# Astropianist/LumFuncMCMC

Hardware: AMD Instinct MI355X
Metric: walker-lnprob evals/sec (10^6 sources, 256 walkers) (higher is better)
Workload: dtype f64; 1 GPU; free completeness, single Schechter: 1000000 synthetic sources, 256 walkers in all (256 per GPU), 2 half-ensemble calls of 128 theta rows per step; walkers_per_gpu=256, walkers_total=256, variant=free, parallelism=1 GPU

## Files before the change

### lumfuncmcmc_amd/csrc/lf_free.h

```cpp
#pragma once
#include "lf_kernels.h"

namespace lf {

constexpr int PB = 512;
constexpr int PTW = 8;
constexpr int QSTRIDE = 9;
constexpr int VF = 32;
constexpr int DEAL_BINS = VF + 1, DEAL_LIST = 2 * (VF + 1), DEAL_MAX = 512;
constexpr unsigned long long PART_EMPTY = 0x7ff8dead7ff8deadull;
constexpr int PART_POLLS = 1 << 19;

template <bool THROUGH = false>
__device__ __forceinline__ void reduce_store512(const double* __restrict__ red, int wlo, int whi, double* __restrict__ out,
                                                size_t stride, int w0, int chunk, int tid) {
    const int w = tid >> 6, lane = tid & 63;
    if (w >= wlo && w < whi) {
        const double* row = red + w * PB + lane;
        double s0 = (row[0] + row[64]) + (row[128] + row[192]);
        double s1 = (row[256] + row[320]) + (row[384] + row[448]);
        const double s = wave_sum_dpp(s0 + s1);
        if (lane == 63) {
            if (THROUGH) __hip_atomic_store(out + (size_t)(w0 + w) * stride + chunk, s, __ATOMIC_RELAXED, __HIP_MEMORY_SCOPE_AGENT);
            else out[(size_t)(w0 + w) * stride + chunk] = s;
        }
    }
}

struct FreeArgs {
    int B, ntiles;
    int nchA, nchB;
    int nslot;
    int tile_stride;
    int skip_grid;
    int* queues;
    double* partA;
    double* partB;
    const double* cells;
    const double* nodes8;
    const int* deal;
    const int* cc_len;
    const int* cc_field;
    int nchC;
    double* partC;
    const int* wstat;
    const double* theta;
    double* out;
    double* wrec_w;
    int* wmode_w;
    int* wstat_w;
    double* wbase_w;
    const double* gq_rec;
    const double* gq_omega;
    const int* gq_rows;
    int nbq;
    int poll;
    int* err;
};

template <int ST, bool CENSUS, bool FUSED, bool STEP>
__device__ __forceinline__ void lf_free_body(const KConst& kc, const SrcArrays& sa, const NodeArrays& na, const double* __restrict__ wrec_arg,
                                             const int* __restrict__ wmode_arg, const FreeArgs& fa, const StepArgs& sp, const AcceptArgs& ap,
                                             unsigned long long t_pre = 0) {
    const double* wrec = FUSED ? fa.wrec_w : wrec_arg;
    const int* wmode = FUSED ? fa.wmode_w : wmode_arg;
    auto pstore = [](double* p, double v) {
        if (FUSED) __hip_atomic_store(p, v == v ? v : __builtin_nan(""), __ATOMIC_RELAXED, __HIP_MEMORY_SCOPE_AGENT);
        else *p = v;
    };
    __shared__ MathTables tab;
    __shared__ TermTables tt;
    __shared__ __attribute__((aligned(16))) double red[PTW * PB];
    __shared__ __attribute__((aligned(16))) double wfc[PTW * MAXF * 8];
    __shared__ __attribute__((aligned(16))) double wsc[PTW * 8];
    __shared__ int sitem[2];
    __shared__ int sdeal[DEAL_MAX];
    __shared__ int scell;
    __shared__ int snosrc;
    const int tid = threadIdx.x;
    __shared__ int sstat[PTW];
    __shared__ double sbase[PTW];
    __shared__ double wlf[PTW * MAXF];
    __shared__ double sprop[PTW * 16];
    __shared__ double szz[PTW];
    __shared__ double spre[PTW * 2];
    if (!FUSED) {
        for (int i = tid; i < 256; i += PB) {
            tab.logt[i] = *reinterpret_cast<const double2*>(LOG_TABLE + 2 * i);
            tab.expt[i] = EXP_TABLE[i];
        }
        load_term_tables<PB>(&tt);
        if (fa.deal && tid < DEAL_LIST + fa.nchC + fa.nbq) sdeal[tid] = fa.deal[tid];
    }
    bool tables_loaded = !FUSED;
    const int wave_base = __builtin_amdgcn_readfirstlane(tid & ~63);
    auto fresh_tid = [&]() -> int {
        int m = -1;
        asm volatile("" : "+s"(m));
        return wave_base + __builtin_amdgcn_mbcnt_hi(m, __builtin_amdgcn_mbcnt_lo(m, 0));
    };
    unsigned xcc;
    asm volatile("s_getreg_b32 %0, hwreg(HW_REG_XCC_ID)" : "=s"(xcc));
    const int myq = (int)(xcc & 7u);
#ifdef LF_STAMPS
    __shared__ unsigned long long s_targs;
    unsigned long long* stamp = kc.stamps ? kc.stamps + (size_t)blockIdx.x * 8 : nullptr;
    if (stamp && tid == 0) {
        stamp[0] = t_pre ? t_pre : __builtin_amdgcn_s_memtime();
        stamp[5] = __builtin_amdgcn_s_memrealtime();
        s_targs = __builtin_amdgcn_s_memtime();
    }
    int nitems_done = 0;
    unsigned long long t_first = 0, t_sw = 0, t_loop = 0, t_red = 0;
    unsigned long long t_prep = 0, t_cells = 0, t_grid = 0;
    __shared__ unsigned long long s_ttab;
    __shared__ unsigned long long s_tp0;
    __shared__ unsigned long long s_tprep[8];
#endif

#pragma unroll 1
    for (int tile = ((int)blockIdx.x >> 3) % fa.ntiles; tile < fa.ntiles; tile += fa.tile_stride) {
        const int w0 = tile * PTW;
        const int nw = min(PTW, fa.B - w0);
        __builtin_assume(nw >= 1 && nw <= PTW);
        int* __restrict__ q = fa.queues + tile * QSTRIDE;
        int fgroup = 8, frank = (int)blockIdx.x & 7;
        if (fa.ntiles <= fa.tile_stride) {
            const int k = (int)blockIdx.x >> 3;
            fgroup = 8 * ((fa.tile_stride - tile + fa.ntiles - 1) / fa.ntiles);
            frank += 8 * ((k - tile) / fa.ntiles);
        }
        bool no_src = false;
        auto grab = [&]() -> int {
            if (no_src) return -1;
            for (int d = 0; d < 8; ++d) {
                const int qq = (myq + d) & 7;
                const int lo = (int)(((long long)qq * fa.nchA) >> 3), hi = (int)(((long long)(qq + 1) * fa.nchA) >> 3);
                if (hi <= lo) continue;
                const int i = atomicAdd(q + 1 + qq, 1);
                if (i < hi - lo) return lo + i;
            }
            return -1;
        };
        int ticket = 0;
        auto take_ticket = [&]() {
            if (!no_src) ticket = atomicAdd(q + 1 + myq, 1);
        };
        auto redeem = [&]() -> int {
            if (no_src) return -1;
            const int lo = (int)(((long long)myq * fa.nchA) >> 3), hi = (int)(((long long)(myq + 1) * fa.nchA) >> 3);
            if (ticket < hi - lo) return lo + ticket;
            return grab();
        };
        if (tile != ((int)blockIdx.x >> 3) % fa.ntiles) __syncthreads();
        const int u = fresh_tid();
        if (FUSED) {
            const int pw = (int)(blockIdx.x >> 8) & 1;
            const int up = u - 64 * pw;
            if (up >= 0 && up < 64) {
                prepare_lane<false, true, STEP, LF_FREE>(kc, sp, fa.theta, fa.B, nullptr, nullptr, nullptr, nullptr, nullptr, 1,
                                          w0 + (up >> 3), up & 7, up >> 3, reinterpret_cast<double(*)[16]>(red), wfc, wsc, sstat, sbase, wlf,
#ifdef LF_STAMPS
                                          s_tprep,
#else
                                          nullptr,
#endif
                                          sprop, szz);
#ifdef LF_STAMPS
                if (up == 0) s_tp0 = __builtin_amdgcn_s_memtime();
#endif
            } else if (!tables_loaded) {
                const int t7 = u < 64 * pw ? u : u - 64;
                double2 lt = *reinterpret_cast<const double2*>(LOG_TABLE + 2 * min(t7, 255));
                double et = EXP_TABLE[min(t7, 255)];
                const int ndeal = fa.deal ? DEAL_LIST + fa.nchC + fa.nbq : 0;
                int d0 = ndeal ? fa.deal[min(t7, ndeal - 1)] : 0, d1 = ndeal ? fa.deal[min(t7 + 256, ndeal - 1)] : 0;
                asm volatile("" : "+v"(lt.x), "+v"(lt.y), "+v"(et), "+v"(d0), "+v"(d1));
                load_term_tables<PB - 64>(&tt, t7);
                if (t7 < 256) {
                    tab.logt[t7] = lt;
                    tab.expt[t7] = et;
                    if (t7 < ndeal) sdeal[t7] = d0;
                    if (t7 + 256 < ndeal) sdeal[t7 + 256] = d1;
                }
#ifdef LF_STAMPS
                if (t7 == 0) s_ttab = __builtin_amdgcn_s_memtime();
#endif
            }
            if (STEP && u >= PB - 64 && u < PB - 64 + nw) {
                const int wl = u - (PB - 64);
                unsigned int rr[4];
                sampler_draw(sp.step, sp.half, w0 + wl, 0, sp.seed, rr);
                accept_terms(ap, w0 + wl, stretch_z(sp.a, u53(rr[0], rr[1])), spre[2 * wl], spre[2 * wl + 1]);
            }
            tables_loaded = true;
            __syncthreads();
        }
        if (u < 64) {
            const int st = FUSED ? sstat[min(u, nw - 1)] : fa.wstat[w0 + min(u, nw - 1)];
            const bool on = fa.nchC > 0 && u < nw && (st & STAT_CELLS);
            const bool need = u < nw && !on && (st & STAT_PRIOR_OK) && !(st & STAT_NEGINF);
            const int m = (int)__ballot(on);
            const unsigned long long mneed = __ballot(need);
            if (u == 0) {
                scell = m;
                no_src = mneed == 0ull;
                snosrc = no_src ? 1 : 0;
                sitem[0] = grab();
            }
        }
        if (!FUSED && u < nw * MAXF) {
            const int w = u / MAXF, f = u - w * MAXF;
            double* d = wfc + u * 8;
            int* di = reinterpret_cast<int*>(d + 4);
            if (f < kc.nf) {
                const double* __restrict__ r = wrec + (size_t)(w0 + w) * REC;
                const int* __restrict__ km = wmode + ((size_t)(w0 + w) * MAXF + f) * WM;
                d[0] = r[R_ALPHAC];
                d[F_V] = r[RF(f, F_V)];
                d[F_CA] = r[RF(f, F_CA)];
                d[F_CY] = r[RF(f, F_CY)] - H_LO - 0.5 / H_INV;
                d[7] = r[RF(f, F_CY)] - H_LO;
#pragma unroll
                for (int i = 0; i < 5; ++i) di[i] = km[i];
            }
        }
        if (!FUSED && u >= PB - PTW * 8) {
            const int t = u - (PB - PTW * 8), w = t >> 3, j = t & 7;
            if (w < nw) wsc[t] = wrec[(size_t)(w0 + w) * REC + j];
        }
        __syncthreads();
#ifdef LF_STAMPS
        t_prep = __builtin_amdgcn_s_memtime();
#endif
        const int cellmask = __builtin_amdgcn_readfirstlane(scell);
        auto fetch = [&](int w, int fld) {
            const double2* __restrict__ p = reinterpret_cast<const double2*>(wfc + (w * MAXF + fld) * 8);
            const double2 a = p[0], b = p[1], c = p[3];
            if (FUSED) {
                const int* __restrict__ ki = reinterpret_cast<const int*>(wfc + (w * MAXF + fld) * 8 + 4);
                return WalkerK{a.x, b.x, b.y, c.y, uni(ki[M_MODE]), uni(ki[M_KLO]), uni(ki[M_KHI]), uni(ki[M_KNE]), uni(ki[M_KAC])};
            }
            const int* __restrict__ km = wmode + ((size_t)(w0 + w) * MAXF + fld) * WM;
            return WalkerK{a.x, b.x, b.y, c.y, km[M_MODE], km[M_KLO], km[M_KHI], km[M_KNE], km[M_KAC]};
        };

        {
            const int v = wave_base >> 6;
#pragma unroll 1
            for (int vr = frank; vr < VF; vr += fgroup) {
            double acc = 0.0;
            const bool dealt = fa.deal != nullptr;
            const int cfirst = (vr - VF / 2 + VF) % VF;
            const int cb = dealt ? DEAL_LIST + uni(sdeal[vr]) : cfirst;
            const int cn = dealt ? uni(sdeal[vr + 1]) - uni(sdeal[vr]) : (cfirst < fa.nchC ? (fa.nchC - cfirst + VF - 1) / VF : 0);
            auto chunk_at = [&](int i) { return dealt ? uni(sdeal[cb + i]) : cb + i * VF; };
            if (fa.nchC > 0 && v < nw && ((cellmask >> v) & 1) && cn > 0) {
                auto load_cells = [&](double (&d)[CELL_REC], int cc) {
                    const int lane = fresh_tid() & 63;
                    const double2* __restrict__ src = reinterpret_cast<const double2*>(fa.cells + ((size_t)cc * 64 + lane) * CELL_REC);
                    static_assert(CELL_REC % 2 == 0, "16-byte loads");
#pragma unroll
                    for (int k = 0; k < CELL_REC / 2; ++k) {
                        const double2 a = src[k];
                        d[2 * k] = a.x;
                        d[2 * k + 1] = a.y;
                    }
                };
                auto field_of = [&](int cc) {
                    int f = 0;
#pragma unroll
                    for (int k = 1; k < MAXF; ++k) f += cc >= kc.cc_fstart[k] ? 1 : 0;
                    return f;
                };
                double nx[CELL_REC];
                load_cells(nx, chunk_at(0));
#pragma unroll 1
                for (int ci = 0; ci < cn; ++ci) {
                    const int cc = chunk_at(ci);
                    double cd[CELL_REC];
#pragma unroll
                    for (int k = 0; k < CELL_REC; ++k) cd[k] = nx[k];
                    if (ci + 1 < cn) load_cells(nx, chunk_at(ci + 1));
                    const WalkerK p = fetch(v, field_of(cc));
                    asm volatile("; LF_BEGIN cell items=1");
                    acc += cell_sum(cd, p, &tt);
                    asm volatile("; LF_END cell");
                    if (CENSUS && kc.forms && (fresh_tid() & 63) == 0) atomicAdd(kc.forms + FORM_CELL, (unsigned long long)uni(fa.cc_len[cc]));
                }
            }
            if (fa.nchC > 0 && v < nw) {
                acc = wave_sum_dpp(acc);
                const int ln = fresh_tid() & 63;
                double* __restrict__ row = fa.partC + (size_t)(w0 + v) * fa.nslot;
                if (ln == 63) pstore(row + vr, acc);
            }
            }
        }
#ifdef LF_STAMPS
        t_cells = __builtin_amdgcn_s_memtime();
#endif
        if (fa.nbq > 0) {
            const int v = wave_base >> 6;
            const int nq = fa.nbq;
#pragma unroll 1
            for (int vr = frank; vr < VF; vr += fgroup) {
            double bsum = 0.0;
            const bool dealt = fa.deal != nullptr;
            const int qb = dealt ? DEAL_LIST + fa.nchC + uni(sdeal[DEAL_BINS + vr]) : vr;
            const int qn = dealt ? uni(sdeal[DEAL_BINS + vr + 1]) - uni(sdeal[DEAL_BINS + vr]) : (vr < nq ? (nq - vr + VF - 1) / VF : 0);
            auto bin_at = [&](int i) { return dealt ? uni(sdeal[qb + i]) : qb + i * VF; };
            if (v < nw && qn > 0) {
                const double* __restrict__ sc = wsc + v * 8;
                const int mode = __builtin_amdgcn_readfirstlane(*reinterpret_cast<const int*>(wfc + (v * MAXF) * 8 + 4));
                const double* __restrict__ r = wfc + v * MAXF * 8 - 8;
                double vmin = r[RF(0, F_V)];
                for (int f = 1; f < kc.nf; ++f) vmin = fmin(vmin, r[RF(f, F_V)]);
                vmin = uni(vmin);
                const double alphaC = uni(sc[R_ALPHAC]);
                auto mine = [&](int c) { return mode != MODE_SKIP && !(kc.grid_parts > 1 && c % kc.grid_parts != kc.grid_part); };
                struct QRec {
                    double x, a4, L, PGL;
                };
                auto load_rec = [&](int c) -> QRec {
                    const int lane = fresh_tid() & 63;
                    const double2* __restrict__ src = reinterpret_cast<const double2*>(fa.gq_rec + ((size_t)c * 64 + lane) * 4);
                    const double2 a = src[0], b = src[1];
                    return QRec{a.x, a.y, b.x, b.y};
                };
                double* __restrict__ Tl = red + v * 64;
                QRec nx = load_rec(bin_at(0));
#pragma unroll 1
                for (int qi = 0; qi < qn; ++qi) {
                    const int c = bin_at(qi);
                    const QRec nd = nx;
                    const int nr = uni(fa.gq_rows[4 * c + 1]), off = uni(fa.gq_rows[4 * c + 2]);
                    if (qi + 1 < qn) nx = load_rec(bin_at(qi + 1));
                    if (mine(c)) {
                        const int lane = fresh_tid() & 63;
                        const double* __restrict__ om = fa.gq_omega + off + lane;
                        double o[8];
#pragma unroll
                        for (int i = 0; i < 8; ++i) o[i] = i < nr ? om[i * 64] : 0.0;
                        asm volatile("; LF_BEGIN qT items=1");
                        Tl[lane] = fexp_c(fma(uni(sc[R_C1]), nd.L - uni(sc[R_LSTAR]), uni(sc[R_C0])) - nd.PGL * uni(sc[R_Q]), &tab);
                        asm volatile("; LF_END qT");
                        const double a4min = __hiloint2double(__builtin_amdgcn_readlane(__double2hiint(nd.a4), 63),
                                                              __builtin_amdgcn_readlane(__double2loint(nd.a4), 63));
                        const bool bright = kc.specialise && alphaC > 0.0 && a4min * vmin > 37.5;
                        if (CENSUS && kc.forms && lane == 0)
                            atomicAdd(kc.forms + (bright ? FORM_NODE_BRIGHT : FORM_NODE_GENERAL), (unsigned long long)(64 * kc.nf));
                        const double s = field_sum_nf(kc, r, alphaC, nd.x, nd.a4, &tab, bright);
                        __builtin_amdgcn_wave_barrier();
                        asm volatile("; LF_BEGIN qdot items=1");
                        double R = 0.0;
#pragma unroll 1
                        for (int k0 = 0; k0 < nr; k0 += 8) {
                            double on[8];
#pragma unroll
                            for (int i = 0; i < 8; ++i) on[i] = k0 + 8 + i < nr ? om[(k0 + 8 + i) * 64] : 0.0;
#pragma unroll
                            for (int i = 0; i < 8; ++i) R = fma(Tl[min(k0 + i, 63)], o[i], R);
#pragma unroll
                            for (int i = 0; i < 8; ++i) o[i] = on[i];
                        }
                        asm volatile("; LF_END qdot");
                        bsum = fma(R, s, bsum);
                        __builtin_amdgcn_wave_barrier();
                    }
                }
            }
            if (v < nw) {
                bsum = wave_sum_dpp(bsum);
                const int ln = fresh_tid() & 63;
                double* __restrict__ row = fa.partB + (size_t)(w0 + v) * fa.nslot;
                if (ln == 63) pstore(row + vr, bsum);
            }
            }
        } else
        {
            const int v = wave_base >> 6;
            const int nch64 = fa.nchB;
#pragma unroll 1
            for (int vr = frank; vr < VF; vr += fgroup) {
            double bsum = 0.0;
            if (v < nw && vr < nch64) {
                const double* __restrict__ sc = wsc + v * 8;
                const int mode = __builtin_amdgcn_readfirstlane(*reinterpret_cast<const int*>(wfc + (v * MAXF) * 8 + 4));
                const double* __restrict__ r = wfc + v * MAXF * 8 - 8;
                double vmin = r[RF(0, F_V)];
                for (int f = 1; f < kc.nf; ++f) vmin = fmin(vmin, r[RF(f, F_V)]);
                vmin = uni(vmin);
                const double alphaC = uni(sc[R_ALPHAC]);
                auto mine = [&](int c) { return mode != MODE_SKIP && !(kc.grid_parts > 1 && c % kc.grid_parts != kc.grid_part); };
                struct Node {
                    double G, PG, W, a3, a4, a4min;
                };
                auto load_nodes = [&](int c) -> Node {
                    const int lane = fresh_tid() & 63;
                    const double2* __restrict__ src = reinterpret_cast<const double2*>(fa.nodes8 + ((size_t)c * 64 + lane) * 8);
                    const double2 a = src[0], b = src[1], d = src[2];
                    return Node{a.x, a.y, b.x, b.y, d.x, d.y};
                };
                Node nx = load_nodes(vr);
#pragma unroll 1
                for (int c = vr; c < nch64; c += VF) {
                    const Node nd = nx;
                    if (c + VF < nch64) nx = load_nodes(c + VF);
                    if (mine(c)) {
                        const double a4min = uni(nd.a4min);
                        const double T = fexp_c(fma(uni(sc[R_C1]), nd.G - uni(sc[R_LSTAR]), uni(sc[R_C0])) - nd.PG * uni(sc[R_Q]), &tab);
                        const bool bright = kc.specialise && alphaC > 0.0 && a4min * vmin > 37.5;
                        if (CENSUS && kc.forms && (fresh_tid() & 63) == 0)
                            atomicAdd(kc.forms + (bright ? FORM_NODE_BRIGHT : FORM_NODE_GENERAL),
                                      (unsigned long long)(min(64, na.nnodes - c * 64) * kc.nf));
                        const double s = field_sum_nf(kc, r, alphaC, nd.a3, nd.a4, &tab, bright);
                        bsum = fma(nd.W * T, s, bsum);
                    }
                }
            }
            if (nch64 > 0 && v < nw) {
                bsum = wave_sum_dpp(bsum);
                const int ln = fresh_tid() & 63;
                double* __restrict__ row = fa.partB + (size_t)(w0 + v) * fa.nslot;
                if (ln == 63) pstore(row + vr, bsum);
            }
            }
        }
#ifdef LF_STAMPS
        t_grid = __builtin_amdgcn_s_memtime();
#endif
        int item = sitem[0];
#pragma unroll 1
        while (item >= 0) {
#ifdef LF_STAMPS
            const unsigned long long ta = __builtin_amdgcn_s_memtime();
            if (t_first == 0) t_first = ta;
            unsigned long long tb = ta, tc = ta;
#endif
            __syncthreads();
            int t = fresh_tid();
            {
                const int c = item;
                const int s0 = uni(sa.chunk_start[c]), n = uni(sa.chunk_len[c]), fld = uni(sa.chunk_field[c]);
                const int kfirst = uni(sa.chunk_keys[KEY_STRIDE * c]), klast = uni(sa.chunk_keys[KEY_STRIDE * c + 1]),
                          kamax = uni(sa.chunk_keys[KEY_STRIDE * c + 4 + (wave_base >> 6)]);
                double x[ST];
                if (t == 0) take_ticket();
                if (n == PB * ST) {
                    typedef double __attribute__((ext_vector_type(2), aligned(8))) double2_a8;
                    const double2_a8* __restrict__ src = reinterpret_cast<const double2_a8*>(sa.a1 + s0 + t * ST);
#pragma unroll
                    for (int k = 0; k < ST / 2; ++k) {
                        const double2_a8 a = src[k];
                        x[2 * k] = a.x;
                        x[2 * k + 1] = a.y;
                    }
                } else {
                    const double* __restrict__ src = sa.a1 + s0;
#pragma unroll
                    for (int k = 0; k < ST; ++k) x[k] = src[min(t * ST + k, n - 1)];
                }
                if (t == 0) {
                    asm volatile("" ::"v"(x[ST - 1]));
                    sitem[0] = redeem();
                }
#ifdef LF_STAMPS
                tb = __builtin_amdgcn_s_memtime();
#endif
                const int npad = ST - min(max(n - t * ST, 0), ST);
                const int nwave = min(max(n - wave_base * ST, 0), 64 * ST);
                int rest = 0;
                WalkerK pn = fetch(0, fld);
#pragma unroll 1
                for (int w = 0; w < nw; ++w) {
                    const WalkerK p = pn;
                    pn = fetch(min(w + 1, nw - 1), fld);
                    double acc = 0.0;
                    if ((cellmask >> w) & 1) {
                    } else if (p.mode < MODE_SKIP && p.mode != MODE_SLOW && kc.tables && kfirst >= p.klo && klast <= p.khi && p.kac <= kamax) {
                        TabCoef C;
                        if (kc.specialise && kfirst >= p.kne) {
                            asm volatile("; LF_BEGIN table_noexp items=%0" ::"n"(ST));
                            table_lookup<ST>(C, x, p, true, &tt);
                            acc = table_terms<ST, true>(C, x, npad);
                            asm volatile("; LF_END table_noexp");
                            if (CENSUS && kc.forms && (t & 63) == 0) atomicAdd(kc.forms + FORM_TABLE_NOEXP, (unsigned long long)nwave);
                        } else {
                            asm volatile("; LF_BEGIN table items=%0" ::"n"(ST));
                            table_lookup<ST>(C, x, p, false, &tt);
                            acc = table_terms<ST, false>(C, x, npad);
                            asm volatile("; LF_END table");
                            if (CENSUS && kc.forms && (t & 63) == 0) atomicAdd(kc.forms + FORM_TABLE, (unsigned long long)nwave);
                        }
                    } else if (p.mode < MODE_SKIP) {
                        rest |= 1 << w;
                    } else if (CENSUS && kc.forms && (t & 63) == 0) {
                        atomicAdd(kc.forms + FORM_SKIPPED, (unsigned long long)nwave);
                    }
                    red[w * PB + t] = acc;
                }
                if (rest) {
                    t = fresh_tid();
                    double u[ST];
                    {
                        const double* __restrict__ up = sa.U + s0;
#pragma unroll
                        for (int k = 0; k < ST; ++k) u[k] = up[min(t * ST + k, n - 1)];
                    }
                    const double a1_first = uni(x[0]), u_first = uni(u[0]);
                    const int nmine = ST - npad;
#pragma unroll 1
                    for (int w = 0; w < nw; ++w) {
                        if (!((rest >> w) & 1)) continue;
                        const double* __restrict__ r = FUSED ? wsc + w * 8 : wrec + (size_t)(w0 + w) * REC;
                        const double* __restrict__ rf = wfc + (w * MAXF + fld) * 8;
                        const int mode = FUSED ? uni(*reinterpret_cast<const int*>(rf + 4)) : wmode[((size_t)(w0 + w) * MAXF + fld) * WM];
                        const double r_lf = FUSED ? wlf[w * MAXF + fld] : r[RF(fld, F_LF)];
                        const double r_v = FUSED ? rf[F_V] : r[RF(fld, F_V)], r_ca = FUSED ? rf[F_CA] : r[RF(fld, F_CA)];
                        double acc = 0.0;
                        int form;
                        if (mode == MODE_SLOW) {
                            form = FORM_CAREFUL;
                            const WFree wf{r[R_LSTAR], r[R_C0] + kc.lnom0_src[fld], r[R_C1], r[R_Q], r[R_ALPHAC],
                                           r_lf, r_v, kc.lnom0_src[fld], 0.0};
#pragma unroll 1
                            for (int i = t; i < n; i += PB) {
                                const size_t g = (size_t)s0 + i;
                                acc += term_free_careful(wf, sa.lum[g], sa.a1[g], sa.P[g], sa.U[g]);
                            }
                        } else {
                            WFree wf{};
                            wf.alphaC = r[R_ALPHAC];
                            wf.cA = r_ca;
                            wf.V = r_v;
                            const bool upper = kc.specialise && wf.alphaC > 0.0 && fma(wf.alphaC, a1_first, wf.cA) >= 0.0;
                            if (upper && u_first * wf.V > 37.5) {
                                form = FORM_GENERAL_NOEXP;
#pragma unroll
                                for (int k = 0; k < ST; ++k) {
                                    asm volatile("; LF_BEGIN general_noexp items=1");
                                    const double term = term_free_noexp(wf, x[k], &tab);
                                    asm volatile("; LF_END general_noexp");
                                    acc += k < nmine ? term : 0.0;
                                    __builtin_amdgcn_sched_barrier(0);
                                }
                            } else {
                                form = FORM_GENERAL;
#pragma unroll
                                for (int k = 0; k < ST; ++k) {
                                    asm volatile("; LF_BEGIN general items=1");
                                    const double term = term_free_fast(wf, x[k], u[k], &tab);
                                    asm volatile("; LF_END general");
                                    acc += k < nmine ? term : 0.0;
                                    __builtin_amdgcn_sched_barrier(0);
                                }
                            }
                        }
                        if (CENSUS && kc.forms && (t & 63) == 0) atomicAdd(kc.forms + form, (unsigned long long)nwave);
                        red[w * PB + t] = acc;
                    }
                }
#ifdef LF_STAMPS
                tc = __builtin_amdgcn_s_memtime();
#endif
                __syncthreads();
                t = fresh_tid();
                reduce_store512<FUSED>(red, 0, nw, fa.partA, (size_t)fa.nchA, w0, c, t);
                item = sitem[0];
            }
#ifdef LF_STAMPS
            ++nitems_done;
            if (tb != ta) {
                t_sw += tb - ta;
                t_loop += tc - tb;
                t_red += __builtin_amdgcn_s_memtime() - tc;
            }
#endif
        }
        if (FUSED && fa.poll && uni(snosrc)) {
            if (frank == fgroup - 1) {
                const int t = fresh_tid(), v = t >> 6, ln = t & 63;
                const int nB = fa.nchB > 0 ? fa.nslot : 0, nC = fa.nchC > 0 ? fa.nslot : 0;
                if (v < nw) {
                    double* __restrict__ pb = fa.partB + (size_t)(w0 + v) * fa.nslot;
                    double* __restrict__ pc = fa.partC + (size_t)(w0 + v) * fa.nslot;
                    double pre[2] = {0.0, 0.0};
                    int tries = 0;
                    bool have;
                    do {
                        if (ln < nC) pre[0] = __hip_atomic_load(pc + ln, __ATOMIC_RELAXED, __HIP_MEMORY_SCOPE_AGENT);
                        if (ln < nB) pre[1] = __hip_atomic_load(pb + ln, __ATOMIC_RELAXED, __HIP_MEMORY_SCOPE_AGENT);
                        have = !((ln < nC && (unsigned long long)__double_as_longlong(pre[0]) == PART_EMPTY) ||
                                 (ln < nB && (unsigned long long)__double_as_longlong(pre[1]) == PART_EMPTY));
                    } while (!__all(have) && ++tries < PART_POLLS);
                    if (tries >= PART_POLLS) {
                        pre[0] = pre[1] = __builtin_nan("");
                        if (ln == 0) atomicExch(fa.err, 1);
                    }
                    if (ln < nC) __hip_atomic_store(pc + ln, __longlong_as_double((long long)PART_EMPTY), __ATOMIC_RELAXED, __HIP_MEMORY_SCOPE_AGENT);
                    if (ln < nB) __hip_atomic_store(pb + ln, __longlong_as_double((long long)PART_EMPTY), __ATOMIC_RELAXED, __HIP_MEMORY_SCOPE_AGENT);
                    finalize_wave<true>(fa.partA, 0, fa.nchA, fa.partB, nB, nB, nC > 0 ? fa.partC : nullptr, nC, (int)STAT_CELLS,
                                        sstat - w0, sbase - w0, w0 + v, ln, ap, fa.out, nullptr, nullptr, 0,
                                        STEP ? sprop + v * 16 : nullptr, STEP ? szz + v : nullptr, STEP ? spre + 2 * v : nullptr, pre);
                }
            }
        } else if (FUSED) {
            asm volatile("s_waitcnt vmcnt(0)" ::: "memory");
            __threadfence_block();
            __syncthreads();
            if (fresh_tid() == 0) sitem[1] = atomicAdd(q, 1);
            __syncthreads();
            if (sitem[1] == fgroup - 1) {
                __builtin_amdgcn_fence(__ATOMIC_ACQUIRE, "workgroup");
                const int t = fresh_tid(), v = t >> 6;
                const int nB = fa.nchB > 0 ? fa.nslot : 0, nC = fa.nchC > 0 ? fa.nslot : 0;
                if (v < nw) {
                    finalize_wave<true>(fa.partA, fa.nchA, fa.nchA, fa.partB, nB, nB, nC > 0 ? fa.partC : nullptr, nC, (int)STAT_CELLS,
                                        sstat - w0, sbase - w0, w0 + v, t & 63, ap, fa.out, nullptr, nullptr, 0,
                                        STEP ? sprop + v * 16 : nullptr, STEP ? szz + v : nullptr, STEP ? spre + 2 * v : nullptr);
                    if (fa.poll) {
                        const int ln = t & 63;
                        if (ln < nC) __hip_atomic_store(fa.partC + (size_t)(w0 + v) * fa.nslot + ln, __longlong_as_double((long long)PART_EMPTY), __ATOMIC_RELAXED, __HIP_MEMORY_SCOPE_AGENT);
                        if (ln < nB) __hip_atomic_store(fa.partB + (size_t)(w0 + v) * fa.nslot + ln, __longlong_as_double((long long)PART_EMPTY), __ATOMIC_RELAXED, __HIP_MEMORY_SCOPE_AGENT);
                    }
                }
                if (t < QSTRIDE) q[t] = 0;
            }
        }
    }
#ifdef LF_STAMPS
    if (stamp && tid == 0) {
        stamp[1] = __builtin_amdgcn_s_memtime();
        const bool noitems = nitems_done == 0;
        stamp[2] = (unsigned long long)nitems_done;
        if (noitems) {
            stamp[3] = t_prep - stamp[0];
            stamp[4] = t_cells - stamp[0];
            stamp[7] = t_grid - stamp[0];
            unsigned long long pk = 0;
            pk = ((s_targs - stamp[0]) >> 4) & 0xfffull;
            for (int i = 0; i < 4; ++i) pk |= (((s_tprep[i] - stamp[0]) >> 4) & 0xfffull) << (12 * (i + 1));
            stamp[2] = pk;
        } else {
            stamp[3] = t_first ? t_first - stamp[0] : 0;
            stamp[4] = t_sw;
            stamp[7] = t_loop;
        }
        stamp[6] = __builtin_amdgcn_s_memrealtime();
        kc.stamps[(size_t)gridDim.x * 8 + blockIdx.x] =
            !noitems ? t_red : (((s_ttab - stamp[0]) << 32) | ((s_tp0 - stamp[0]) & 0xffffffffull));
    }
#endif
}

template <int ST, bool CENSUS, bool FUSED = false>
__global__ __launch_bounds__(PB, 4) void lf_free(KConst kc, SrcArrays sa, NodeArrays na, const double* __restrict__ wrec_arg,
                                                 const int* __restrict__ wmode_arg, FreeArgs fa) {
#ifdef LF_STAMPS
    const unsigned long long t_pre = __builtin_amdgcn_s_memtime();
#else
    const unsigned long long t_pre = 0;
#endif
    warm_kernarg<sizeof(KConst) + sizeof(SrcArrays) + sizeof(NodeArrays) + 2 * 8 + sizeof(FreeArgs)>();
    lf_free_body<ST, CENSUS, FUSED, false>(kc, sa, na, wrec_arg, wmode_arg, fa, StepArgs{}, AcceptArgs{}, t_pre);
}

template <int ST>
__global__ __launch_bounds__(PB, 4) void lf_free_step(KConst kc, SrcArrays sa, NodeArrays na, FreeArgs fa, StepArgs sp, AcceptArgs ap) {
    warm_kernarg<sizeof(KConst) + sizeof(SrcArrays) + sizeof(NodeArrays) + sizeof(FreeArgs) + sizeof(StepArgs) + sizeof(AcceptArgs)>();
    lf_free_body<ST, false, true, true>(kc, sa, na, nullptr, nullptr, fa, sp, ap);
}

}
```

### lumfuncmcmc_amd/csrc/lf_math.h

```cpp
#pragma once
#include <hip/hip_runtime.h>

#include "lf_tables.h"

#define LF_LN10 2.302585092994045684
#define LF_LNLN10 0.834032445247955959
#define LF_LN2 0.693147180559945309
#define LF_UNDERFLOW 745.13321910194122
#define LF_LREF 42.0
#define LF_FREF (-17.0)
#define LF_SQARCSEC 42545170296.152206
#define LF_MPC_CM 3.086e24

namespace lf {

__device__ __forceinline__ double dexp(double x) { return exp(x); }
__device__ __forceinline__ double dlog(double x) { return log(x); }
__device__ __forceinline__ double drsqrt(double x) { return rsqrt(x); }
__device__ __forceinline__ double ddiv(double a, double b) { return a / b; }

struct MathTables {
    double2 logt[256];
    double expt[256];
};

__device__ __forceinline__ double fexp_t(double x, const MathTables* __restrict__ mt) {
    const double MAGIC = 6755399441055744.0;
    const double t = fma(x, 369.32993046757463, MAGIC);
    const double kd = t - MAGIC;
    double r = fma(kd, -0.00270760617331689, x);
    r = fma(kd, -7.453964567463233e-13, r);
    const int k = __double2loint(t);
    const double T = mt->expt[k & 255];
    double q = fma(r, 4.16666666666666666667e-02, 1.66666666666666666667e-01);
    q = fma(q, r, 0.5);
    const double p = fma(r * r, q, r);
    return ldexp(fma(T, p, T), k >> 8);
}

__device__ __forceinline__ double fexp_neg(double u, const MathTables* __restrict__ mt) {
    const double MAGIC = 6755399441055744.0;
    const double t = fma(u, -369.32993046757463, MAGIC);
    const double kd = t - MAGIC;
    const double r = fma(kd, -0.0027076061740622863, -u);
    const int k = __double2loint(t);
    const double T = mt->expt[k & 255];
    double q = fma(r, 4.16666666666666666667e-02, 1.66666666666666666667e-01);
    q = fma(q, r, 0.5);
    const double p = fma(r * r, q, r);
    return ldexp(fma(T, p, T), k >> 8);
}

__device__ __forceinline__ double fexp_c(double x, const MathTables* __restrict__ mt) {
    return fexp_t(fmin(fmax(x, -750.0), 709.0), mt);
}

__device__ __forceinline__ double flog_half(double w, const MathTables* __restrict__ mt) {
    const int hi = __double2hiint(w), lo = __double2loint(w);
    const int e = ((hi >> 20) & 0x7ff) - 1024;
    const int j = (hi >> 12) & 0xff;
    const double m = __hiloint2double((hi & 0x000fffff) | 0x3ff00000, lo);
    const double2 t = mt->logt[j];
    const double r = fma(m, t.x, -1.0);
    double p = fma(r, 0.2, -0.25);
    double third = 1.0 / 3.0;
    asm volatile("" : "+s"(third));
    p = fma(p, r, third);
    p = fma(p, r, -0.5);
    const double r2 = r * r;
    const double hi_part = fma((double)e, LF_LN2, t.y);
    return hi_part + fma(p, r2, r);
}

__device__ __forceinline__ double flog_half_upper(double w, const MathTables* __restrict__ mt) {
    const double m = fmin(w, 1.9999999999999998);
    const int j = (__double2hiint(m) >> 12) & 0xff;
    const double2 t = mt->logt[j];
    const double r = fma(m, t.x, -1.0);
    double p = fma(r, 0.2, -0.25);
    p = fma(p, r, 1.0 / 3.0);
    p = fma(p, r, -0.5);
    const double r2 = r * r;
    return (t.y - LF_LN2) + fma(p, r2, r);
}

__device__ __forceinline__ double frsqrt(double s) {
    const double z0 = __builtin_amdgcn_rsq(s);
    const double e = fma(-(s * z0), z0, 1.0);
    const double p = fma(0.375, e, 0.5);
    return fma(z0, p * e, z0);
}

__device__ __forceinline__ double frcp(double d) {
    const double y0 = __builtin_amdgcn_rcp(d);
    const double e = fma(-d, y0, 1.0);
    return fma(y0, fma(e, e, e), y0);
}

struct TermTables {
    double g[G_N * 8];
    double h[H_N * 8];
};
template <int NT>
__device__ __forceinline__ void load_term_tables(TermTables* tt, int t = -1) {
    double2* g2 = reinterpret_cast<double2*>(tt->g);
    double2* h2 = reinterpret_cast<double2*>(tt->h);
    const double2* G2 = reinterpret_cast<const double2*>(G_TABLE);
    const double2* H2 = reinterpret_cast<const double2*>(H_TABLE);
    constexpr int NG = (G_N * 4 + NT - 1) / NT, NH = (H_N * 4 + NT - 1) / NT;
    double2 vg[NG], vh[NH];
    if (t < 0) t = threadIdx.x;
#pragma unroll
    for (int q = 0; q < NG; ++q) vg[q] = G2[min(t + q * NT, G_N * 4 - 1)];
#pragma unroll
    for (int q = 0; q < NH; ++q) vh[q] = H2[min(t + q * NT, H_N * 4 - 1)];
#pragma unroll
    for (int q = 0; q < NG; ++q) asm volatile("" : "+v"(vg[q].x), "+v"(vg[q].y));
#pragma unroll
    for (int q = 0; q < NH; ++q) asm volatile("" : "+v"(vh[q].x), "+v"(vh[q].y));
#pragma unroll
    for (int q = 0; q < NG; ++q)
        if (t + q * NT < G_N * 4) g2[t + q * NT] = vg[q];
#pragma unroll
    for (int q = 0; q < NH; ++q)
        if (t + q * NT < H_N * 4) h2[t + q * NT] = vh[q];
}

__device__ __forceinline__ double horner7(const double (&c)[8], double t) {
    double p = fma(c[7], t, c[6]);
    p = fma(p, t, c[5]);
    p = fma(p, t, c[4]);
    p = fma(p, t, c[3]);
    p = fma(p, t, c[2]);
    p = fma(p, t, c[1]);
    return fma(p, t, c[0]);
}

__device__ __forceinline__ void load_tables(MathTables* mt) {
    for (int i = threadIdx.x; i < 256; i += blockDim.x) {
        mt->logt[i] = make_double2(LOG_TABLE[2 * i], LOG_TABLE[2 * i + 1]);
        mt->expt[i] = EXP_TABLE[i];
    }
}
__device__ __forceinline__ void load_tables_256(MathTables* mt) {
    const int i = threadIdx.x;
    const double2 l = *reinterpret_cast<const double2*>(LOG_TABLE + 2 * i);
    const double e = EXP_TABLE[i];
    mt->logt[i] = l;
    mt->expt[i] = e;
}

template <int CTRL, int ROW_MASK>
__device__ __forceinline__ double dpp_shift_add(double v) {
    const int lo = __builtin_amdgcn_update_dpp(0, __double2loint(v), CTRL, ROW_MASK, 0xf, false);
    const int hi = __builtin_amdgcn_update_dpp(0, __double2hiint(v), CTRL, ROW_MASK, 0xf, false);
    return v + __hiloint2double(hi, lo);
}
__device__ __forceinline__ double wave_sum_dpp(double v) {
    v = dpp_shift_add<0x111, 0xf>(v);
    v = dpp_shift_add<0x112, 0xf>(v);
    v = dpp_shift_add<0x114, 0xf>(v);
    v = dpp_shift_add<0x118, 0xf>(v);
    v = dpp_shift_add<0x142, 0xa>(v);
    v = dpp_shift_add<0x143, 0xc>(v);
    return v;
}

__device__ __forceinline__ double wave_sum(double v) {
#pragma unroll
    for (int off = 32; off > 0; off >>= 1) v += __shfl_down(v, off, 64);
    return v;
}

#define LF_KW1(o) "s_load_dword %0, %1, " #o "\n\t"
#define LF_KW4(b) LF_KW1(b + 0x00) LF_KW1(b + 0x40) LF_KW1(b + 0x80) LF_KW1(b + 0xc0)
template <int BYTES>
__device__ __forceinline__ void warm_kernarg() {
    constexpr int N4 = (BYTES + 255) / 256;
    static_assert(N4 >= 1 && N4 <= 10, "extend the ladder");
    auto p = __builtin_amdgcn_kernarg_segment_ptr();
    int t;
    if constexpr (N4 == 1) asm volatile(LF_KW4(0x000) "s_waitcnt lgkmcnt(0)" : "=&s"(t) : "s"(p) : "memory");
    if constexpr (N4 == 2) asm volatile(LF_KW4(0x000) LF_KW4(0x100) "s_waitcnt lgkmcnt(0)" : "=&s"(t) : "s"(p) : "memory");
    if constexpr (N4 == 3) asm volatile(LF_KW4(0x000) LF_KW4(0x100) LF_KW4(0x200) "s_waitcnt lgkmcnt(0)" : "=&s"(t) : "s"(p) : "memory");
    if constexpr (N4 == 4)
        asm volatile(LF_KW4(0x000) LF_KW4(0x100) LF_KW4(0x200) LF_KW4(0x300) "s_waitcnt lgkmcnt(0)" : "=&s"(t) : "s"(p) : "memory");
    if constexpr (N4 == 5)
        asm volatile(LF_KW4(0x000) LF_KW4(0x100) LF_KW4(0x200) LF_KW4(0x300) LF_KW4(0x400) "s_waitcnt lgkmcnt(0)" : "=&s"(t) : "s"(p) : "memory");
    if constexpr (N4 == 6)
        asm volatile(LF_KW4(0x000) LF_KW4(0x100) LF_KW4(0x200) LF_KW4(0x300) LF_KW4(0x400) LF_KW4(0x500) "s_waitcnt lgkmcnt(0)"
                     : "=&s"(t) : "s"(p) : "memory");
    if constexpr (N4 == 7)
        asm volatile(LF_KW4(0x000) LF_KW4(0x100) LF_KW4(0x200) LF_KW4(0x300) LF_KW4(0x400) LF_KW4(0x500) LF_KW4(0x600) "s_waitcnt lgkmcnt(0)"
                     : "=&s"(t) : "s"(p) : "memory");
    if constexpr (N4 == 8)
        asm volatile(LF_KW4(0x000) LF_KW4(0x100) LF_KW4(0x200) LF_KW4(0x300) LF_KW4(0x400) LF_KW4(0x500) LF_KW4(0x600) LF_KW4(0x700)
                     "s_waitcnt lgkmcnt(0)" : "=&s"(t) : "s"(p) : "memory");
    if constexpr (N4 == 9)
        asm volatile(LF_KW4(0x000) LF_KW4(0x100) LF_KW4(0x200) LF_KW4(0x300) LF_KW4(0x400) LF_KW4(0x500) LF_KW4(0x600) LF_KW4(0x700)
                     LF_KW4(0x800) "s_waitcnt lgkmcnt(0)" : "=&s"(t) : "s"(p) : "memory");
    if constexpr (N4 == 10)
        asm volatile(LF_KW4(0x000) LF_KW4(0x100) LF_KW4(0x200) LF_KW4(0x300) LF_KW4(0x400) LF_KW4(0x500) LF_KW4(0x600) LF_KW4(0x700)
                     LF_KW4(0x800) LF_KW4(0x900) "s_waitcnt lgkmcnt(0)" : "=&s"(t) : "s"(p) : "memory");
}

}
```

### lumfuncmcmc_amd/csrc/lf_pers.h

```cpp
#pragma once
#include "lf_free.h"

namespace lf {

constexpr int PERS_MAXS = 256;

struct PersArgs {
    int B, ntiles;
    int nchB;
    int nchC, ncell;
    int nslot;
    int tile_stride;
    int* queues;
    double* partA;
    double* partB;
    double* partC;
    const double* nodes4;
    const double* zcol;
    const double* cells;
    const double* lum;
    const double* a1;
    const double* P;
    const double* U;
    const double* theta;
    double* out;
    const double* wrec;
    const int* wmode;
    const int* wstat;
    int poll;
    int* err;
};

template <int VARIANT, bool FUSED, bool STEP>
__device__ __forceinline__ void lf_pers_body(const KConst& kc, const PersArgs& pa, const StepArgs& sp, const AcceptArgs& ap) {
    static_assert(VARIANT == LF_ZEVOL || VARIANT == LF_FIXCOMP, "the free variant has lf_free");
    auto pstore = [](double* p, double v) {
        if (FUSED) __hip_atomic_store(p, v == v ? v : __builtin_nan(""), __ATOMIC_RELAXED, __HIP_MEMORY_SCOPE_AGENT);
        else *p = v;
    };
    __shared__ MathTables tab;
    __shared__ __attribute__((aligned(16))) double wsc[PTW * 8];
    __shared__ __attribute__((aligned(16))) double wfc[PTW * MAXF * 8];
    __shared__ __attribute__((aligned(16))) double qe[VARIANT == LF_ZEVOL ? PTW * PERS_MAXS * 2 : 2];
    __shared__ __attribute__((aligned(16))) double red[PB];
    __shared__ __attribute__((aligned(16))) double zcl[VARIANT == LF_ZEVOL ? PERS_MAXS * 2 : 2];
    __shared__ int sstat[PTW];
    __shared__ double sbase[PTW];
    __shared__ double sprop[PTW * 16];
    __shared__ double szz[PTW];
    __shared__ double spre[PTW * 2];
    __shared__ int smask[4];
    __shared__ int sdone;
    const int tid = threadIdx.x;
    const int wave_base = __builtin_amdgcn_readfirstlane(tid & ~63);
    const int lane = tid & 63, v = wave_base >> 6;
    bool tables_loaded = false;
#ifdef LF_STAMPS
    unsigned long long* stamp = kc.stamps ? kc.stamps + (size_t)blockIdx.x * 8 : nullptr;
    unsigned long long t_prep = 0, t_cols = 0, t_cells = 0, t_grid = 0;
    if (stamp && tid == 0) {
        stamp[0] = __builtin_amdgcn_s_memtime();
        stamp[5] = __builtin_amdgcn_s_memrealtime();
    }
#endif

#pragma unroll 1
    for (int tile = ((int)blockIdx.x >> 3) % pa.ntiles; tile < pa.ntiles; tile += pa.tile_stride) {
        const int w0 = tile * PTW;
        const int nw = min(PTW, pa.B - w0);
        __builtin_assume(nw >= 1 && nw <= PTW);
        int* __restrict__ q = pa.queues + tile * QSTRIDE;
        int fgroup = 8, frank = (int)blockIdx.x & 7;
        if (pa.ntiles <= pa.tile_stride) {
            const int k = (int)blockIdx.x >> 3;
            fgroup = 8 * ((pa.tile_stride - tile + pa.ntiles - 1) / pa.ntiles);
            frank += 8 * ((k - tile) / pa.ntiles);
        }
        __syncthreads();
        if (FUSED) {
            const int pw = (int)(blockIdx.x >> 8) & 1;
            const int up = tid - 64 * pw;
            if (up >= 0 && up < 64) {
                prepare_lane<false, true, STEP, VARIANT>(kc, sp, pa.theta, pa.B, nullptr, nullptr, nullptr, nullptr, nullptr, 0, w0 + (up >> 3), up & 7,
                                                up >> 3, reinterpret_cast<double(*)[16]>(red), wfc, wsc, sstat, sbase, nullptr, nullptr, sprop, szz);
            } else if (!tables_loaded && tid >= 128 && tid < 128 + 256) {
                int fm = -1;
                asm volatile("" : "+s"(fm));
                const int t = wave_base + __builtin_amdgcn_mbcnt_hi(fm, __builtin_amdgcn_mbcnt_lo(fm, 0)) - 128;
                double2 lt = *reinterpret_cast<const double2*>(LOG_TABLE + 2 * t);
                double et = EXP_TABLE[t];
                double2 zz = VARIANT == LF_ZEVOL ? *reinterpret_cast<const double2*>(pa.zcol + 2 * min(t, kc.S - 1)) : double2{0.0, 0.0};
                asm volatile("" : "+v"(lt.x), "+v"(lt.y), "+v"(et), "+v"(zz.x), "+v"(zz.y));
                tab.logt[t] = lt;
                tab.expt[t] = et;
                if (VARIANT == LF_ZEVOL) *reinterpret_cast<double2*>(zcl + 2 * t) = zz;
            }
        } else {
            if (!tables_loaded && tid >= 256) {
                const int t = tid - 256;
                double2 lt = *reinterpret_cast<const double2*>(LOG_TABLE + 2 * t);
                double et = EXP_TABLE[t];
                double2 zz = VARIANT == LF_ZEVOL ? *reinterpret_cast<const double2*>(pa.zcol + 2 * min(t, kc.S - 1)) : double2{0.0, 0.0};
                asm volatile("" : "+v"(lt.x), "+v"(lt.y), "+v"(et), "+v"(zz.x), "+v"(zz.y));
                tab.logt[t] = lt;
                tab.expt[t] = et;
                if (VARIANT == LF_ZEVOL) *reinterpret_cast<double2*>(zcl + 2 * t) = zz;
            }
            if (tid < nw * MAXF) {
                const int w = tid / MAXF, f = tid - w * MAXF;
                wfc[tid * 8] = pa.wrec[(size_t)(w0 + w) * REC + RF(f, 0)];
                reinterpret_cast<int*>(wfc + tid * 8 + 4)[M_MODE] = pa.wmode[((size_t)(w0 + w) * MAXF + f) * WM + M_MODE];
            }
            if (tid >= 64 && tid < 128) {
                const int t = tid - 64, w = t >> 3, j = t & 7;
                if (w < nw) wsc[t] = pa.wrec[(size_t)(w0 + w) * REC + j];
            }
            if (tid >= 128 && tid < 128 + nw) sstat[tid - 128] = pa.wstat[w0 + tid - 128];
        }
        if (FUSED && STEP && tid >= PB - 64 && tid < PB - 64 + nw) {
            const int wl = tid - (PB - 64);
            unsigned int rr[4];
            sampler_draw(sp.step, sp.half, w0 + wl, 0, sp.seed, rr);
            accept_terms(ap, w0 + wl, stretch_z(sp.a, u53(rr[0], rr[1])), spre[2 * wl], spre[2 * wl + 1]);
        }
        tables_loaded = true;
        __syncthreads();
        if (tid < 64) {
            const int st = sstat[min(tid, nw - 1)];
            const bool in = tid < nw;
            const bool live = in && (st & STAT_PRIOR_OK) && !(st & STAT_NEGINF);
            const bool on = VARIANT == LF_ZEVOL && pa.nchC > 0 && in && (st & STAT_CELLS);
            const bool need = live && (VARIANT == LF_FIXCOMP ? (st & STAT_SLOW) != 0 : !on);
            const int mc = (int)__ballot(on), mn = (int)__ballot(need), mo = (int)__ballot(in && !(st & STAT_PRIOR_OK));
            if (tid == 0) {
                smask[0] = mc;
                smask[1] = mn;
                smask[2] = mo;
            }
        }
        __syncthreads();
#ifdef LF_STAMPS
        t_prep = __builtin_amdgcn_s_memtime();
#endif
        const int cellmask = uni(smask[0]), needmask = uni(smask[1]), outmask = uni(smask[2]);
        const bool mine_w = v < nw;
        const bool grid_w = mine_w && !((outmask >> v) & 1);
        const double* __restrict__ sc = wsc + v * 8;

#ifdef LF_STAMPS
        t_cols = __builtin_amdgcn_s_memtime();
#endif
        if (VARIANT == LF_ZEVOL && pa.nchC > 0 && mine_w) {
#pragma unroll 1
            for (int vr = frank; vr < VF; vr += fgroup) {
            double acc = 0.0;
            const int cfirst = (vr - VF / 2 + VF) % VF;
            if ((cellmask >> v) & 1) {
                const double aL = uni(sc[Z_AL]), bL = uni(sc[Z_BL]), cL = uni(sc[Z_CL]);
                auto load_cell = [&](double (&d)[8], int cc) {
                    const int i = cc * 64 + lane;
                    const double2* __restrict__ src = reinterpret_cast<const double2*>(pa.cells + (size_t)min(i, pa.ncell - 1) * 8);
#pragma unroll
                    for (int k = 0; k < 4; ++k) {
                        const double2 a = src[k];
                        d[2 * k] = i < pa.ncell || k == 0 ? a.x : 0.0;
                        d[2 * k + 1] = i < pa.ncell ? a.y : 0.0;
                    }
                };
                double nx[8];
                if (cfirst < pa.nchC) load_cell(nx, cfirst);
#pragma unroll 1
                for (int cc = cfirst; cc < pa.nchC; cc += VF) {
                    double cd[8];
#pragma unroll
                    for (int k = 0; k < 8; ++k) cd[k] = nx[k];
                    if (cc + VF < pa.nchC) load_cell(nx, cc + VF);
                    asm volatile("; LF_BEGIN pzcell items=1");
                    const double zc2 = cd[0] * cd[0];
                    const double Lc = quad_nofma(aL, bL, cL, cd[0], zc2);
                    const double Hc = fexp_c(LF_LN10 * (LF_LREF - Lc), &tab);
                    const double b2 = -2.0 * LF_LN10 * aL;
                    const double a = fma(b2, cd[0], -LF_LN10 * bL);
                    double cm2 = 1.0, cm1 = a, tail = 0.0;
                    const double head = fma(cm1, cd[2], cd[1]);
#pragma unroll
                    for (int j = 2; j <= ZCELL_M; ++j) {
                        const double cj = fma(a, cm1, b2 * cm2) * (1.0 / j);
                        tail = fma(cj, cd[1 + j], tail);
                        cm2 = cm1;
                        cm1 = cj;
                    }
                    acc = fma(-Hc, head + tail, acc);
                    asm volatile("; LF_END pzcell");
                }
            }
            acc = wave_sum_dpp(acc);
            double* __restrict__ row = pa.partC + (size_t)(w0 + v) * pa.nslot;
            if (lane == 63) pstore(row + vr, acc);
            }
        }
#ifdef LF_STAMPS
        t_cells = __builtin_amdgcn_s_memtime();
#endif
        if (mine_w) {
            const int cpr = (pa.nchB + VF - 1) / VF;
#pragma unroll 1
            for (int vr = frank; vr < VF; vr += fgroup) {
            double bsum = 0.0;
            const int clo = vr * cpr, chi = min(clo + cpr, pa.nchB);
            if (VARIANT == LF_ZEVOL && grid_w && clo < chi) {
                const double aL = uni(sc[Z_AL]), bL = uni(sc[Z_BL]), cL = uni(sc[Z_CL]);
                const double aP = uni(sc[Z_AP]), bP = uni(sc[Z_BP]), cP = uni(sc[Z_CP]), c1z = uni(sc[Z_C1]);
                const int k_lo = (clo * 64) / kc.S, k_hi = min((chi * 64 - 1) / kc.S, kc.S - 1);
                for (int k = k_lo + lane; k <= k_hi; k += 64) {
                    const double2 zz = *reinterpret_cast<const double2*>(zcl + 2 * k);
                    const double Lsz = quad_nofma(aL, bL, cL, zz.x, zz.y);
                    const double ph = quad_nofma(aP, bP, cP, zz.x, zz.y);
                    double2 o;
                    o.x = fexp_c(LF_LN10 * (LF_LREF - Lsz), &tab);
                    o.y = fma(-c1z, Lsz - LF_LREF, fma(LF_LN10, ph, LF_LNLN10));
                    *reinterpret_cast<double2*>(qe + (v * PERS_MAXS + k) * 2) = o;
                }
                __builtin_amdgcn_wave_barrier();
            }
            if (grid_w && clo < chi) {
                struct Node {
                    double G, PG, W, col;
                };
                auto load_nodes = [&](int c) -> Node {
                    const double2* __restrict__ src = reinterpret_cast<const double2*>(pa.nodes4 + ((size_t)c * 64 + lane) * 4);
                    const double2 a = src[0], b = src[1];
                    return Node{a.x, a.y, b.x, b.y};
                };
                auto mine = [&](int c) { return !(kc.grid_parts > 1 && c % kc.grid_parts != kc.grid_part); };
                const double c1 = uni(sc[VARIANT == LF_ZEVOL ? Z_C1 : R_C1]);
                const double Ls = uni(sc[R_LSTAR]), c0 = uni(sc[R_C0]), Qf = uni(sc[R_Q]);
                auto node = [&](const Node& nd, int c) {
                    if (!mine(c)) return;
                    asm volatile("; LF_BEGIN pznode items=1");
                    double e;
                    if (VARIANT == LF_ZEVOL) {
                        const int k = min((int)nd.col, PERS_MAXS - 1);
                        const double2 QE = *reinterpret_cast<const double2*>(qe + (v * PERS_MAXS + k) * 2);
                        e = fma(c1, nd.G - LF_LREF, QE.y) - nd.PG * QE.x;
                    } else {
                        e = fma(c1, nd.G - Ls, c0) - nd.PG * Qf;
                    }
                    if (__ballot(e > -750.0) != 0ull) bsum = fma(nd.W, fexp_c(e, &tab), bsum);
                    asm volatile("; LF_END pznode");
                };
                Node na = load_nodes(clo), nb;
#pragma unroll 1
                for (int c = clo; c < chi; c += 2) {
                    nb = load_nodes(min(c + 1, chi - 1));
                    node(na, c);
                    na = load_nodes(min(c + 2, chi - 1));
                    if (c + 1 < chi) node(nb, c + 1);
                }
            }
            bsum = wave_sum_dpp(bsum);
            double* __restrict__ row = pa.partB + (size_t)(w0 + v) * pa.nslot;
            if (lane == 63) pstore(row + vr, bsum);
            }
        }
#ifdef LF_STAMPS
        t_grid = __builtin_amdgcn_s_memtime();
#endif
        if (needmask) {
            const double NEG_INF = -__builtin_huge_val();
#pragma unroll 1
            for (int w = 0; w < nw; ++w) {
                if (!((needmask >> w) & 1)) continue;
                const double* __restrict__ r = wsc + w * 8;
#pragma unroll 1
                for (int vr = frank; vr < VF; vr += fgroup) {
                double acc = 0.0;
                long long start = 0;
#pragma unroll 1
                for (int f = 0; f < kc.nf; ++f) {
                    const int n = kc.nsrc[f];
                    const int mode = uni(reinterpret_cast<const int*>(wfc + (w * MAXF + f) * 8 + 4)[M_MODE]);
                    if (VARIANT == LF_FIXCOMP ? mode == MODE_SLOW : mode <= MODE_SLOW) {
#pragma unroll 1
                        for (int i = vr * PB + tid; i < n; i += VF * PB) {
                            const size_t g = (size_t)(start + i);
                            const double clum = pa.lum[g], ca1 = pa.a1[g], cpp = pa.P[g];
                            double term;
                            if (VARIANT == LF_FIXCOMP) {
                                const double vv = cpp * r[R_Q];
                                const double lnT = fma(r[R_C1], clum - r[R_LSTAR], r[R_C0]) - vv;
                                term = lnT + ca1;
                                const bool bad = (vv > LF_UNDERFLOW) | (lnT < -LF_UNDERFLOW) | (term < -LF_UNDERFLOW) | (term != term);
                                term = bad ? NEG_INF : 0.0;
                            } else {
                                const WZ wz{r[Z_AL], r[Z_BL], r[Z_CL], r[Z_AP], r[Z_BP], r[Z_CP], r[Z_C1], 0.0};
                                double vv;
                                if (mode == MODE_SLOW) {
                                    const double lnT = lnT_zevol<false>(wz, clum, ca1, pa.U[g], vv, &tab);
                                    term = lnT + cpp;
                                    const bool bad = (vv > LF_UNDERFLOW) | (lnT < -LF_UNDERFLOW) | (term < -LF_UNDERFLOW) | (term != term);
                                    term = bad ? NEG_INF : -vv;
                                } else {
                                    const double Lsz = quad_nofma(wz.aL, wz.bL, wz.cL, ca1, pa.U[g]);
                                    term = -fexp_t(LF_LN10 * (clum - Lsz), &tab);
                                }
                            }
                            acc += term;
                        }
                    }
                    start += n;
                }
                __syncthreads();
                red[tid] = acc;
                __syncthreads();
                if (tid < 64) {
                    double s = 0.0;
#pragma unroll
                    for (int k = 0; k < PB / 64; ++k) s += red[tid + 64 * k];
                    s = wave_sum_dpp(s);
                    double* __restrict__ row = pa.partA + (size_t)(w0 + w) * pa.nslot;
                    if (tid == 63) pstore(row + vr, s);
                }
                }
            }
        }
        if (FUSED && pa.poll && needmask == 0) {
            if (frank == fgroup - 1 && v < nw) {
                const int nB = pa.nchB > 0 ? pa.nslot : 0, nC = VARIANT == LF_ZEVOL && pa.nchC > 0 ? pa.nslot : 0;
                double* __restrict__ pb = pa.partB + (size_t)(w0 + v) * pa.nslot;
                double* __restrict__ pc = pa.partC + (size_t)(w0 + v) * pa.nslot;
                double pre[2] = {0.0, 0.0};
                int tries = 0;
                bool have;
                do {
                    if (lane < nC) pre[0] = __hip_atomic_load(pc + lane, __ATOMIC_RELAXED, __HIP_MEMORY_SCOPE_AGENT);
                    if (lane < nB) pre[1] = __hip_atomic_load(pb + lane, __ATOMIC_RELAXED, __HIP_MEMORY_SCOPE_AGENT);
                    have = !((lane < nC && (unsigned long long)__double_as_longlong(pre[0]) == PART_EMPTY) ||
                             (lane < nB && (unsigned long long)__double_as_longlong(pre[1]) == PART_EMPTY));
                } while (!__all(have) && ++tries < PART_POLLS);
                if (tries >= PART_POLLS) {
                    pre[0] = pre[1] = __builtin_nan("");
                    if (lane == 0) atomicExch(pa.err, 1);
                }
                if (lane < nC) __hip_atomic_store(pc + lane, __longlong_as_double((long long)PART_EMPTY), __ATOMIC_RELAXED, __HIP_MEMORY_SCOPE_AGENT);
                if (lane < nB) __hip_atomic_store(pb + lane, __longlong_as_double((long long)PART_EMPTY), __ATOMIC_RELAXED, __HIP_MEMORY_SCOPE_AGENT);
                finalize_wave<true>(pa.partA, 0, pa.nslot, pa.partB, nB, pa.nslot, nC > 0 ? pa.partC : nullptr, nC, (int)STAT_CELLS,
                                    sstat - w0, sbase - w0, w0 + v, lane, ap, pa.out, nullptr, nullptr,
                                    VARIANT == LF_FIXCOMP ? (int)STAT_SLOW : 0,
                                    STEP ? sprop + v * 16 : nullptr, STEP ? szz + v : nullptr, STEP ? spre + 2 * v : nullptr, pre);
            }
        } else if (FUSED) {
            asm volatile("s_waitcnt vmcnt(0)" ::: "memory");
            __threadfence_block();
            __syncthreads();
            if (tid == 0) sdone = atomicAdd(q, 1);
            __syncthreads();
            if (sdone == fgroup - 1) {
                __builtin_amdgcn_fence(__ATOMIC_ACQUIRE, "workgroup");
                const int nC = VARIANT == LF_ZEVOL && pa.nchC > 0 ? pa.nslot : 0;
                if (v < nw) {
                    finalize_wave<true>(pa.partA, pa.nslot, pa.nslot, pa.partB, pa.nslot, pa.nslot, nC > 0 ? pa.partC : nullptr, nC, (int)STAT_CELLS,
                                        sstat - w0, sbase - w0, w0 + v, lane, ap, pa.out, nullptr, nullptr,
                                        VARIANT == LF_FIXCOMP ? (int)STAT_SLOW : 0,
                                        STEP ? sprop + v * 16 : nullptr, STEP ? szz + v : nullptr, STEP ? spre + 2 * v : nullptr);
                    if (pa.poll) {
                        if (lane < nC) __hip_atomic_store(pa.partC + (size_t)(w0 + v) * pa.nslot + lane, __longlong_as_double((long long)PART_EMPTY), __ATOMIC_RELAXED, __HIP_MEMORY_SCOPE_AGENT);
                        if (lane < pa.nslot) __hip_atomic_store(pa.partB + (size_t)(w0 + v) * pa.nslot + lane, __longlong_as_double((long long)PART_EMPTY), __ATOMIC_RELAXED, __HIP_MEMORY_SCOPE_AGENT);
                    }
                }
                if (tid < QSTRIDE) q[tid] = 0;
            }
        }
    }
#ifdef LF_STAMPS
    if (stamp && tid == 0) {
        stamp[1] = __builtin_amdgcn_s_memtime();
        stamp[2] = 0;
        stamp[3] = t_prep - stamp[0];
        stamp[4] = t_cells - stamp[0];
        stamp[7] = t_grid - stamp[0];
        stamp[6] = __builtin_amdgcn_s_memrealtime();
        kc.stamps[(size_t)gridDim.x * 8 + blockIdx.x] = ((t_cols - stamp[0]) << 32) | ((t_prep - stamp[0]) & 0xffffffffull);
    }
#endif
}

template <int VARIANT, bool FUSED>
__global__ __launch_bounds__(PB, 4) void lf_pers(KConst kc, PersArgs pa) {
    warm_kernarg<sizeof(KConst) + sizeof(PersArgs)>();
    lf_pers_body<VARIANT, FUSED, false>(kc, pa, StepArgs{}, AcceptArgs{});
}

template <int VARIANT>
__global__ __launch_bounds__(PB, 4) void lf_pers_step(KConst kc, PersArgs pa, StepArgs sp, AcceptArgs ap) {
    warm_kernarg<sizeof(KConst) + sizeof(PersArgs) + sizeof(StepArgs) + sizeof(AcceptArgs)>();
    lf_pers_body<VARIANT, true, true>(kc, pa, sp, ap);
}

}
```

### lumfuncmcmc_amd/csrc/lfmcmc.hip

```cpp
#include "../../include/lfmcmc.h"

#include <hip/hip_runtime.h>

#include <algorithm>
#include <cmath>
#include <cstdio>
#include <cstdlib>
#include <cstring>
#include <map>
#include <string>
#include <vector>

#include "lf_bands.h"
#include "lf_compress.h"
#include "lf_gridbound.h"
#include "lf_kernels.h"
#include "lf_free.h"
#include "lf_pers.h"

namespace {

thread_local std::string g_create_error = "";

struct ChunkTable {
    int n = 0;
    int* d_start = nullptr;
    int* d_len = nullptr;
    int* d_field = nullptr;
    int* d_keys = nullptr;
};

struct EventPair {
    hipEvent_t a, b;
    int kind;
    int count = 1;
};

struct CompressedCat {
    bool built = false;
    int64_t n = 0;
    std::vector<int64_t> field_ind;
    double *d_lum = nullptr, *d_a1 = nullptr, *d_U = nullptr, *d_W = nullptr;
    std::map<int, ChunkTable> chunks;
    int nbins = 0;
    double bound = 0.0;
};

}

struct lf_ctx {
    lf::KConst kc{};
    int device = 0;
    int64_t N = 0;
    int nnodes = 0;
    std::vector<int64_t> field_ind;
    std::vector<double> h_x;
    unsigned long long* d_forms = nullptr;
    int last_launch[8] = {0, 0, 0, 0, 0, 0, 0, 0};
    int* d_queue = nullptr;
    double* d_cells = nullptr;
    int* d_cc_start = nullptr;
    int* d_deal = nullptr;
    int64_t deal_key = -1;
    int* d_cc_len = nullptr;
    int* d_cc_field = nullptr;
    int ncell = 0, ncchunk = 0;
    int64_t opt_cells = 1;
    int cap_queue = 0;
    int slots_free[3] = {0, 0, 0};
    int num_cu = 0;
    double *d_lum = nullptr, *d_a1 = nullptr, *d_P = nullptr, *d_U = nullptr;
    double *d_G = nullptr, *d_PG = nullptr, *d_W = nullptr, *d_a3 = nullptr, *d_a4 = nullptr, *d_a4min = nullptr, *d_nodes8 = nullptr;
    std::map<int, ChunkTable> chunks;
    std::map<int, ChunkTable> chunks_free;
    int64_t opt_persistent = 1;
    int64_t opt_fuse = 1;
    int64_t opt_fuse_step = 1;
    bool queue_zero = false;
    bool parts_empty = false;
    int* d_err = nullptr;
    int64_t opt_poll = 1;
    int64_t opt_free_st = 0;
    int64_t opt_geometry = -1;
    int64_t opt_walker_tile = 0;
    int64_t opt_taper = 0;
    int64_t opt_skip_grid = 0;
    int64_t opt_compress = 0;
    int64_t opt_compress_grid = 1;
    CompressedCat cmp;
    std::vector<double> h_L, h_wL, h_ck, h_Dk;
    struct {
        bool built = false;
        int nb = 0;
        double bound = 0.0;
        double *d_U = nullptr, *d_A4 = nullptr, *d_omega = nullptr, *d_L = nullptr, *d_PGL = nullptr;
        int *d_row0 = nullptr, *d_nrows = nullptr, *d_off = nullptr;
    } gridc;
    struct {
        bool built = false;
        int nb = 0;
        double margin = 0.0;
        double *d_rec = nullptr, *d_omega = nullptr;
        int* d_rows = nullptr;
    } gridq;
    int64_t opt_grid_shortcut = 1;
    double *d_nodes4 = nullptr, *d_zcol = nullptr;
    int nch4 = 0;
    int slots_pers = 0;
    double* d_partR = nullptr;
    int* d_slow = nullptr;
    int cap_slow = 0;
    size_t cap_partR = 0;
    int cap_B = 0;
    size_t cap_partA = 0, cap_partB = 0;
    double *d_theta = nullptr, *d_out = nullptr, *d_outA = nullptr, *d_outB = nullptr;
    double *d_wrec = nullptr, *d_partA = nullptr, *d_partB = nullptr;
    int *d_wstat = nullptr, *d_wmode = nullptr;
    double* d_wbase = nullptr;
    double *h_theta = nullptr, *h_out = nullptr;
    hipStream_t stream = nullptr;
    hipStream_t last_stream = nullptr;
    bool any_enqueued = false;
    int profiling = 0;
    lf::ZCells zcells{};
    int64_t opt_profile_every = 1;
    int64_t prof_tick = 0;
    int64_t opt_profile_span = 1;
    int64_t prof_pos = 0;
    bool prof_span_ok = false;
    bool span_open = false;
    EventPair span_ep{};
    bool prof_this = true;
    std::vector<EventPair> events;
    double acc_ms[4] = {0, 0, 0, 0};
    int64_t acc_n[4] = {0, 0, 0, 0};
    std::string err;
};

namespace {

#define LF_HIP(ctx, call)                                                                  \
    do {                                                                                   \
        hipError_t e_ = (call);                                                            \
        if (e_ != hipSuccess) {                                                            \
            (ctx)->err = std::string(#call) + ": " + hipGetErrorString(e_);                \
            return LF_ERR_HIP;                                                             \
        }                                                                                  \
    } while (0)

template <typename T>
int upload(lf_ctx* c, T** dst, const T* src, size_t n) {
    LF_HIP(c, hipMalloc((void**)dst, std::max<size_t>(n, 1) * sizeof(T)));
    if (n) LF_HIP(c, hipMemcpy(*dst, src, n * sizeof(T), hipMemcpyHostToDevice));
    return LF_OK;
}

double zcell_rho_for_box(const lf::KConst& kc, int nf) {
    using namespace lf;
    const double lo = kc.lims[LF_LIM_LSTAR][0], hi = kc.lims[LF_LIM_LSTAR][1];
    double zmin = HUGE_VAL, zmax = -HUGE_VAL;
    for (int f = 0; f < nf; ++f)
        if (kc.nsrc[f] > 0) {
            zmin = std::fmin(zmin, kc.z_lo[f]);
            zmax = std::fmax(zmax, kc.z_hi[f]);
        }
    if (!(std::isfinite(lo) && std::isfinite(hi) && std::isfinite(zmin) && std::isfinite(zmax))) return 0.0;
    const double z1 = kc.pivots[0], z2 = kc.pivots[1], z3 = kc.pivots[2];
    if (!(z1 != z2 && z2 != z3 && z1 != z3)) return 0.0;
    double smax = 0.0, amax = 0.0;
    for (int corner = 0; corner < 8; ++corner) {
        const double L1 = corner & 1 ? hi : lo, L2 = corner & 2 ? hi : lo, L3 = corner & 4 ? hi : lo;
        const double d12 = (L2 - L1) / (z2 - z1), d23 = (L3 - L2) / (z3 - z2);
        const double a = (d23 - d12) / (z3 - z1);
        for (double z : {zmin, zmax}) smax = std::fmax(smax, std::fabs(d12 + a * (2.0 * z - z1 - z2)));
        amax = std::fmax(amax, std::fabs(a));
    }
    double rho = ZCELL_RHO;
    if (smax > 0.0) rho = std::fmin(rho, 0.98 * ZCELL_X1 / (LF_LN10 * smax));
    if (amax > 0.0) rho = std::fmin(rho, std::sqrt(0.98 * ZCELL_X2 / (LF_LN10 * amax)));
    return std::isfinite(rho) ? rho : 0.0;
}

int build_cells(lf_ctx* c, lf::KConst& kc, const std::vector<double>& x, int nf, const double* wts = nullptr) {
    using namespace lf;
    const double ahi = kc.lims[LF_LIM_ALPHA][1];
    if (!wts && (!(ahi > 0.0) || !std::isfinite(ahi))) return LF_OK;
    const double rho = wts ? kc.zcell_rho : std::fmin(CELL_RHO_H, CELL_RHO_G / ahi);
    if (!(rho > 0.0)) return LF_OK;
    const size_t per_chunk = wts ? (size_t)BLOCK : 64;
    const int M = wts ? ZCELL_M : CELL_M;
    const size_t rec = (size_t)M + 2;
    std::vector<double> cd;
    std::vector<int> cst, cln, cfl;
    size_t nreal = 0;
    for (int f = 0; f < nf; ++f) {
        const int64_t lo = c->field_ind[f], hi = c->field_ind[f + 1];
        if (hi <= lo) continue;
        for (int64_t i = lo; i < hi; ++i)
            if (!std::isfinite(x[(size_t)i]) || (wts && !(std::isfinite(wts[(size_t)i]) && wts[(size_t)i] > 0.0))) return LF_OK;
        if (!wts) {
            const double k0 = std::floor((x[(size_t)lo] - kc.key_x0) * KEY_SCALE), k1 = std::ceil((x[(size_t)hi - 1] - kc.key_x0) * KEY_SCALE);
            if (!(k0 >= 0.0 && k1 < (double)KEY_MAX)) return LF_OK;
            kc.kf_first[f] = (int)k0;
            kc.kf_last[f] = (int)k1;
        }
        const size_t first_cell = cd.size() / rec;
        for (int64_t i = lo; i < hi;) {
            int64_t j = i + 1;
            while (j < hi && x[(size_t)j] - x[(size_t)i] <= 2.0 * rho) ++j;
            const double xc = 0.5 * (x[(size_t)i] + x[(size_t)j - 1]);
            long double S[CELL_M + 1] = {0};
            static_assert(ZCELL_M <= CELL_M, "S is sized for the larger");
            for (int64_t k = i; k < j; ++k) {
                const long double dlt = (long double)x[(size_t)k] - (long double)xc;
                long double pw = wts ? (long double)wts[(size_t)k] : 1.0L;
                for (int m = 0; m <= M; ++m) {
                    S[m] += pw;
                    pw *= dlt;
                }
            }
            cd.push_back(xc);
            for (int m = 0; m <= M; ++m) cd.push_back((double)S[m]);
            i = j;
        }
        size_t ncf = cd.size() / rec - first_cell;
        nreal += ncf;
        if (!wts) {
            kc.cc_fstart[f] = (int)cst.size();
            const double xlast = cd[cd.size() - rec];
            while (ncf % 64) {
                cd.push_back(xlast);
                for (int m = 0; m <= M; ++m) cd.push_back(0.0);
                ++ncf;
            }
        }
        for (size_t s0 = 0; s0 < ncf; s0 += per_chunk) {
            cst.push_back((int)(first_cell + s0));
            cln.push_back((int)std::min<size_t>(per_chunk, ncf - s0));
            cfl.push_back(f);
        }
    }
    const size_t ncell = cd.size() / rec;
    if (!wts) {
        for (int f = nf; f <= MAXF; ++f) kc.cc_fstart[f] = (int)cst.size();
        for (int f = nf - 1; f >= 0; --f)
            if (c->field_ind[f + 1] <= c->field_ind[f]) kc.cc_fstart[f] = kc.cc_fstart[f + 1];
    }
    if (nreal == 0 || ((size_t)c->N < 4 * nreal && c->N > 65536)) return LF_OK;
    int rc;
    if ((rc = upload(c, &c->d_cells, cd.data(), cd.size())) != LF_OK) return rc;
    if ((rc = upload(c, &c->d_cc_start, cst.data(), cst.size())) != LF_OK) return rc;
    if ((rc = upload(c, &c->d_cc_len, cln.data(), cln.size())) != LF_OK) return rc;
    if ((rc = upload(c, &c->d_cc_field, cfl.data(), cfl.size())) != LF_OK) return rc;
    c->ncell = (int)ncell;
    c->ncchunk = (int)cst.size();
    kc.cells = c->opt_cells ? 1 : 0;
    return LF_OK;
}

int get_chunks(lf_ctx* c, std::map<int, ChunkTable>& tables, const std::vector<int64_t>& field_ind, int ch,
               ChunkTable** out, const double* hx = nullptr, int lane_w = 0) {
    auto it = tables.find(ch);
    if (it != tables.end()) {
        *out = &it->second;
        return LF_OK;
    }
    std::vector<int> st, ln, fl;
    for (int f = 0; f < c->kc.nf; ++f) {
        for (int64_t s = field_ind[f]; s < field_ind[f + 1]; s += ch) {
            st.push_back((int)s);
            ln.push_back((int)std::min<int64_t>(ch, field_ind[f + 1] - s));
            fl.push_back(f);
        }
    }
    constexpr int KS = lf::KEY_STRIDE;
    std::vector<int> keys((size_t)KS * st.size(), 0);
// ... 171 lines not shown
            c->span_open = true;
        }
    }
    ~Prof() {
        if (on) {
            hipEventRecord(ep.b, s);
            c->events.push_back(ep);
        }
        if (span && c->span_open) {
            ++c->span_ep.count;
            if (c->span_ep.count >= std::min(c->opt_profile_span, c->opt_profile_every)) {
                hipEventRecord(c->span_ep.b, s);
                c->events.push_back(c->span_ep);
                c->span_open = false;
            }
        }
    }
};

template <int VARIANT, int GI, bool CMP = false>
void launch_geo(lf_ctx* c, dim3 grid, lf::Tiling tl, int ntilesB, int twb, int nblkB, hipStream_t s,
                const lf::SrcArrays& sa, const lf::NodeArrays& na, int B, int nchA, int nchB,
                const lf::Rescue& rs = lf::Rescue{}, const lf::GridC& gc = lf::GridC{}) {
    using namespace lf;
    if (std::getenv("LF_DEBUG_OCC")) {
        int nb = -1;
        hipFuncAttributes fa{};
        hipOccupancyMaxActiveBlocksPerMultiprocessor(&nb, lf_main<VARIANT, GEOS[GI].st, GEOS[GI].tw, GEOS[GI].twb, CMP>, BLOCK, 0);
        hipFuncGetAttributes(&fa, reinterpret_cast<const void*>(&lf_main<VARIANT, GEOS[GI].st, GEOS[GI].tw, GEOS[GI].twb, CMP>));
        std::fprintf(stderr, "lf_main<%d,%d,%d,%d,%d>: %d workgroups per CU (occupancy API), %d VGPRs, %zu B LDS, grid %u\n", VARIANT,
                     GEOS[GI].st, GEOS[GI].tw, GEOS[GI].twb, (int)CMP, nb, fa.numRegs, fa.sharedSizeBytes, grid.x);
    }
    ZCells zc{};
    if (!CMP && ((VARIANT == LF_ZEVOL && c->zcells.nchC > 0) || VARIANT == LF_FIXCOMP)) {
        zc = c->zcells;
        const int nsrc_wg = nchA * (tl.ntiles + tl.ntiles_s);
        zc.nwork = std::min(nsrc_wg, std::max(c->num_cu, 1));
        if (zc.nwork > 0) {
            grid.x = (unsigned)(nblkB + zc.nwork + zc.nchC * ((B + GEOS[GI].tw - 1) / GEOS[GI].tw));
            c->last_launch[4] = (int)grid.x;
        }
    }
    hipLaunchKernelGGL((lf_main<VARIANT, GEOS[GI].st, GEOS[GI].tw, GEOS[GI].twb, CMP>), grid, dim3(BLOCK), 0, s, c->kc, sa,
                       na, c->d_wrec, c->d_wmode, B, tl, nchA, ntilesB, twb, nblkB, c->d_partA, nchA, c->d_partB, nchB, rs, gc, zc);
}

constexpr int CMP_GEOS[] = {8, 1, 4, 2};
template <int VARIANT>
void launch_main_cmp(lf_ctx* c, int gi, dim3 grid, lf::Tiling tl, int ntilesB, int twb, int nblkB, hipStream_t s,
                     const lf::SrcArrays& sa, const lf::NodeArrays& na, int B, int nchA, int nchB, const lf::Rescue& rs,
                     const lf::GridC& gc) {
    switch (gi) {
        case 1: launch_geo<VARIANT, 1, true>(c, grid, tl, ntilesB, twb, nblkB, s, sa, na, B, nchA, nchB, rs, gc); break;
        case 4: launch_geo<VARIANT, 4, true>(c, grid, tl, ntilesB, twb, nblkB, s, sa, na, B, nchA, nchB, rs, gc); break;
        case 2: launch_geo<VARIANT, 2, true>(c, grid, tl, ntilesB, twb, nblkB, s, sa, na, B, nchA, nchB, rs, gc); break;
        default: launch_geo<VARIANT, 8, true>(c, grid, tl, ntilesB, twb, nblkB, s, sa, na, B, nchA, nchB, rs, gc);
    }
}

template <int VARIANT>
void launch_main(lf_ctx* c, int gi, dim3 grid, lf::Tiling tl, int ntilesB, int twb, int nblkB, hipStream_t s,
                 const lf::SrcArrays& sa, const lf::NodeArrays& na, int B, int nchA, int nchB, const lf::Rescue& rs) {
    switch (gi) {
        case 0: launch_geo<VARIANT, 0>(c, grid, tl, ntilesB, twb, nblkB, s, sa, na, B, nchA, nchB, rs); break;
        case 1: launch_geo<VARIANT, 1>(c, grid, tl, ntilesB, twb, nblkB, s, sa, na, B, nchA, nchB, rs); break;
        case 2: launch_geo<VARIANT, 2>(c, grid, tl, ntilesB, twb, nblkB, s, sa, na, B, nchA, nchB, rs); break;
        case 3: launch_geo<VARIANT, 3>(c, grid, tl, ntilesB, twb, nblkB, s, sa, na, B, nchA, nchB, rs); break;
        case 4: launch_geo<VARIANT, 4>(c, grid, tl, ntilesB, twb, nblkB, s, sa, na, B, nchA, nchB, rs); break;
        case 5: launch_geo<VARIANT, 5>(c, grid, tl, ntilesB, twb, nblkB, s, sa, na, B, nchA, nchB, rs); break;
        case 6: launch_geo<VARIANT, 6>(c, grid, tl, ntilesB, twb, nblkB, s, sa, na, B, nchA, nchB, rs); break;
        case 7: launch_geo<VARIANT, 7>(c, grid, tl, ntilesB, twb, nblkB, s, sa, na, B, nchA, nchB, rs); break;
        default: launch_geo<VARIANT, 8>(c, grid, tl, ntilesB, twb, nblkB, s, sa, na, B, nchA, nchB, rs);
    }
}

struct FreeShape {
    int st;
    int64_t items_per_tile;
};
FreeShape free_shape(const lf_ctx* c) {
    using namespace lf;
    FreeShape fs;
    const int64_t chunks8 = (c->N + 8 * (int64_t)PB - 1) / (8 * (int64_t)PB);
    fs.st = c->opt_free_st ? (int)c->opt_free_st : (chunks8 >= 74 ? 8 : 4);
    const int64_t nchB = c->opt_skip_grid ? 0 : (c->nnodes + PB - 1) / PB;
    fs.items_per_tile = (c->N + (int64_t)PB * fs.st - 1) / ((int64_t)PB * fs.st) + nchB * 2;
    return fs;
}

template <int ST>
int free_groups(lf_ctx* c, int slot, int ntiles, int nchA, int nchB, int nchC) {
    using namespace lf;
    if (c->slots_free[slot] == 0) {
        int nb = 0;
        if (hipOccupancyMaxActiveBlocksPerMultiprocessor(&nb, lf_free<ST, false>, PB, 0) != hipSuccess || nb < 1) nb = 1;
        c->slots_free[slot] = nb * std::max(c->num_cu, 1);
        if (std::getenv("LF_DEBUG_OCC")) {
            hipFuncAttributes at{};
            hipFuncGetAttributes(&at, reinterpret_cast<const void*>(&lf_free<ST, false>));
            std::fprintf(stderr, "lf_free<%d>: %d workgroups per CU (occupancy API), %d VGPRs, %zu B LDS\n", ST, nb, at.numRegs, at.sharedSizeBytes);
        }
    }
    const int64_t per_tile = std::min<int64_t>(VF / 8, ((int64_t)nchA + nchB + nchC + 7) / 8);
    return (int)std::max<int64_t>(1, std::min<int64_t>(c->slots_free[slot] / 8, (int64_t)ntiles * std::max<int64_t>(per_tile, 1)));
}

static std::vector<int> make_deal(int nchC, int nbq, int grid_part, int grid_parts) {
    using namespace lf;
    std::vector<int> load(VF), cnt_c(VF, 0), cnt_b(VF, 0), own_c(nchC), own_b(nbq);
    const int cost_h = std::getenv("LF_DEAL_H") ? std::atoi(std::getenv("LF_DEAL_H")) : 8;
    const int cost_b = std::getenv("LF_DEAL_B") ? std::atoi(std::getenv("LF_DEAL_B")) : 8;
    for (int v = 0; v < VF; ++v) load[v] = v >= VF / 2 ? cost_h : 0;
    auto next = [&]() { return (int)(std::min_element(load.begin(), load.end()) - load.begin()); };
    for (int b = 0; b < nbq; ++b) {
        const int v = next();
        own_b[b] = v;
        ++cnt_b[v];
        load[v] += grid_parts > 1 && b % grid_parts != grid_part ? 0 : cost_b;
    }
    for (int i = 0; i < nchC; ++i) {
        const int v = next();
        own_c[i] = v;
        ++cnt_c[v];
        load[v] += 3;
    }
    std::vector<int> t(DEAL_LIST + nchC + nbq);
    t[0] = 0;
    t[DEAL_BINS] = 0;
    for (int v = 0; v < VF; ++v) {
        t[v + 1] = t[v] + cnt_c[v];
        t[DEAL_BINS + v + 1] = t[DEAL_BINS + v] + cnt_b[v];
    }
    std::vector<int> at_c(t.begin(), t.begin() + VF), at_b(t.begin() + DEAL_BINS, t.begin() + DEAL_BINS + VF);
    for (int i = 0; i < nchC; ++i) t[DEAL_LIST + at_c[own_c[i]]++] = i;
    for (int b = 0; b < nbq; ++b) t[DEAL_LIST + nchC + at_b[own_b[b]]++] = b;
    return t;
}

int ensure_deal(lf_ctx* c, int nchC, int nbq, hipStream_t s) {
    using namespace lf;
    const int64_t key = nbq <= 0 || DEAL_LIST + nchC + nbq > DEAL_MAX || std::getenv("LF_NO_DEAL")
                            ? 0 : 1 + nchC + 4096ll * nbq + (4096ll * 4096) * (c->kc.grid_part + 4096ll * c->kc.grid_parts);
    if (key == c->deal_key) return LF_OK;
    if (key > 0) {
        const std::vector<int> t = make_deal(nchC, nbq, c->kc.grid_part, c->kc.grid_parts);
        if (!c->d_deal) LF_HIP(c, hipMalloc((void**)&c->d_deal, (size_t)DEAL_MAX * sizeof(int)));
        if (c->any_enqueued) LF_HIP(c, hipStreamSynchronize(c->last_stream));
        LF_HIP(c, hipMemcpy(c->d_deal, t.data(), t.size() * sizeof(int), hipMemcpyHostToDevice));
    }
    c->deal_key = key;
    return LF_OK;
}

template <int ST>
void launch_free(lf_ctx* c, int slot, int B, int ntiles, const lf::SrcArrays& sa, const lf::NodeArrays& na, lf::FreeArgs fa, hipStream_t s,
                 bool fused, const lf::StepArgs* sp = nullptr, const lf::AcceptArgs* ap = nullptr) {
    using namespace lf;
    const dim3 grid((unsigned)(8 * fa.tile_stride));
    const int info[8] = {ST, PTW, PTW, fused ? 3 : 2, (int)grid.x, fa.nchA, fa.nchB, B};
    std::memcpy(c->last_launch, info, sizeof(info));
    if (fused && sp) hipLaunchKernelGGL((lf_free_step<ST>), grid, dim3(PB), 0, s, c->kc, sa, na, fa, *sp, *ap);
    else if (fused) hipLaunchKernelGGL((lf_free<ST, false, true>), grid, dim3(PB), 0, s, c->kc, sa, na, c->d_wrec, c->d_wmode, fa);
    else if (c->kc.forms) hipLaunchKernelGGL((lf_free<ST, true>), grid, dim3(PB), 0, s, c->kc, sa, na, c->d_wrec, c->d_wmode, fa);
    else hipLaunchKernelGGL((lf_free<ST, false>), grid, dim3(PB), 0, s, c->kc, sa, na, c->d_wrec, c->d_wmode, fa);
}

int enqueue_free(lf_ctx* c, const double* d_theta, int B, double* d_out, double* d_outA, double* d_outB, hipStream_t s,
                 const lf::StepArgs& sp, const lf::AcceptArgs& ap) {
    using namespace lf;
    const int ntiles = (B + PTW - 1) / PTW;
    const FreeShape fs = free_shape(c);
    const int st = fs.st, slot = fs.st == 8 ? 2 : (fs.st == 4 ? 1 : 0);
    ChunkTable* ct = nullptr;
    int rc = get_chunks(c, c->chunks_free, c->field_ind, PB * st, &ct, c->h_x.data(), st);
    if (rc != LF_OK) return rc;
    const int nchA = ct->n;
    const bool gq = c->gridq.built && c->opt_grid_shortcut && !c->opt_skip_grid;
    const int nchB = c->opt_skip_grid ? 0 : (gq ? c->gridq.nb : (c->nnodes + 63) / 64);
    const int nchC = c->kc.cells ? c->ncchunk : 0;
    const int g8 = st == 8 ? free_groups<8>(c, slot, ntiles, nchA, nchB, nchC)
                 : st == 4 ? free_groups<4>(c, slot, ntiles, nchA, nchB, nchC) : free_groups<2>(c, slot, ntiles, nchA, nchB, nchC);
    const int nslot = VF;
    rc = ensure_workspace(c, B, (size_t)B * std::max(nchA, 1), (size_t)B * nslot, (size_t)B * nslot);
    if (rc != LF_OK) return rc;
    if ((rc = ensure_deal(c, nchC, gq ? c->gridq.nb : 0, s)) != LF_OK) return rc;
    if (ntiles * QSTRIDE > c->cap_queue) {
        LF_HIP(c, hipDeviceSynchronize());
        release(c->d_queue);
        c->cap_queue = 0;
        const int cap = std::max(2 * ntiles * QSTRIDE, 1024);
        LF_HIP(c, hipMalloc((void**)&c->d_queue, (size_t)cap * sizeof(int)));
        c->cap_queue = cap;
        c->queue_zero = false;
    }
    const bool stepf = sp.enabled && ap.enabled && c->opt_fuse_step;
    const bool fused = c->opt_fuse && (stepf || (!sp.enabled && !ap.enabled)) && !d_outA && !d_outB && d_out && !c->kc.forms && c->profiling < 2 &&
                       nchA + nchB > 0;
    if (c->any_enqueued && c->last_stream != s) LF_HIP(c, hipStreamSynchronize(c->last_stream));
    c->last_stream = s;
    c->any_enqueued = true;
    c->prof_pos = c->prof_tick++ % c->opt_profile_every;
    c->prof_this = c->profiling > 0 && c->prof_pos == 0;
    c->prof_span_ok = fused;
    if (fused && !c->queue_zero) {
        LF_HIP(c, hipMemsetAsync(c->d_queue, 0, (size_t)c->cap_queue * sizeof(int), s));
        c->queue_zero = true;
    }
    const bool poll = fused && c->opt_poll && nslot <= 64;
    if (poll && !c->parts_empty) {
        static_assert((PART_EMPTY >> 32) == (PART_EMPTY & 0xffffffffull), "filled by 32-bit words");
        LF_HIP(c, hipMemsetD32Async((hipDeviceptr_t)c->d_partB, (int)(PART_EMPTY & 0xffffffffull), c->cap_partB * 2, s));
        LF_HIP(c, hipMemsetD32Async((hipDeviceptr_t)c->d_partR, (int)(PART_EMPTY & 0xffffffffull), c->cap_partR * 2, s));
        if (!c->d_err) {
            LF_HIP(c, hipMalloc((void**)&c->d_err, sizeof(int)));
            LF_HIP(c, hipMemsetAsync(c->d_err, 0, sizeof(int), s));
        }
        c->parts_empty = true;
    }
    if (!poll) c->parts_empty = false;
    if (!fused) {
        c->queue_zero = false;
        Prof p(c, s, 0);
        hipLaunchKernelGGL(lf_prepare, dim3((B + 7) / 8), dim3(64), 0, s, c->kc, sp, d_theta, B, c->d_wrec,
                           c->d_wstat, c->d_wmode, c->d_wbase, (int*)nullptr, c->d_queue, ntiles * QSTRIDE);
    }
    const SrcArrays sa{c->d_lum, c->d_a1, c->d_P, c->d_U, nullptr, ct->d_start, ct->d_len, ct->d_field, ct->d_keys, nullptr};
    const NodeArrays na{c->d_G, c->d_PG, c->d_W, c->d_a3, c->d_a4, c->d_a4min, c->nnodes};
    FreeArgs fa{B, ntiles, nchA, nchB, nslot, g8, (int)c->opt_skip_grid, c->d_queue, c->d_partA, c->d_partB,
                c->d_cells, c->d_nodes8, c->deal_key > 0 ? c->d_deal : nullptr, c->d_cc_len, c->d_cc_field, nchC, c->d_partR, c->d_wstat,
                d_theta, d_out, c->d_wrec, c->d_wmode, c->d_wstat, c->d_wbase,
                gq ? c->gridq.d_rec : nullptr, gq ? c->gridq.d_omega : nullptr, gq ? c->gridq.d_rows : nullptr, gq ? c->gridq.nb : 0,
                poll ? 1 : 0, c->d_err};
    {
        Prof p(c, s, 1);
        if (nchA + nchB > 0) {
            const StepArgs* psp = fused && stepf ? &sp : nullptr;
            if (st == 8) launch_free<8>(c, slot, B, ntiles, sa, na, fa, s, fused, psp, &ap);
            else if (st == 4) launch_free<4>(c, slot, B, ntiles, sa, na, fa, s, fused, psp, &ap);
            else launch_free<2>(c, slot, B, ntiles, sa, na, fa, s, fused, psp, &ap);
        }
    }
    if (!fused) {
        Prof p(c, s, 3);
        const int nB = nchB > 0 ? nslot : 0, nC = nchC > 0 ? nslot : 0;
        hipLaunchKernelGGL(lf_finalize, dim3(B), dim3(64), 0, s, c->d_partA, nchA, nchA, c->d_partB, nB, nB,
                           nC > 0 ? (const double*)c->d_partR : (const double*)nullptr, nC, (int)STAT_CELLS, c->d_wstat, c->d_wbase, B, ap,
                           d_out, d_outA, d_outB, (int*)nullptr, 0);
    }
    LF_HIP(c, hipGetLastError());
    return LF_OK;
}

template <int VARIANT>
int enqueue_pers_v(lf_ctx* c, const double* d_theta, int B, double* d_out, double* d_outA, double* d_outB, hipStream_t s,
                   const lf::StepArgs& sp, const lf::AcceptArgs& ap) {
    using namespace lf;
    const int ntiles = (B + PTW - 1) / PTW;
    if (c->slots_pers == 0) {
        int nb = 0;
        if (hipOccupancyMaxActiveBlocksPerMultiprocessor(&nb, lf_pers<VARIANT, true>, PB, 0) != hipSuccess || nb < 1) nb = 1;
        c->slots_pers = std::min(nb, 2) * std::max(c->num_cu, 1);
    }
    const int nchB = c->opt_skip_grid ? 0 : c->nch4;
    const int nchC = VARIANT == LF_ZEVOL && c->kc.cells ? (c->ncell + 63) / 64 : 0;
    const int64_t per_tile = std::max<int64_t>(1, std::min<int64_t>(VF / 8, ((int64_t)nchB + nchC + 7) / 8));
    const int g8 = (int)std::max<int64_t>(1, std::min<int64_t>(c->slots_pers / 8, (int64_t)ntiles * per_tile));
    const int nslot = VF;
    int rc = ensure_workspace(c, B, (size_t)B * nslot, (size_t)B * nslot, (size_t)B * nslot);
    if (rc != LF_OK) return rc;
    if (ntiles * QSTRIDE > c->cap_queue) {
        LF_HIP(c, hipDeviceSynchronize());
        release(c->d_queue);
        c->cap_queue = 0;
        const int cap = std::max(2 * ntiles * QSTRIDE, 1024);
        LF_HIP(c, hipMalloc((void**)&c->d_queue, (size_t)cap * sizeof(int)));
        c->cap_queue = cap;
        c->queue_zero = false;
    }
    const bool stepf = sp.enabled && ap.enabled && c->opt_fuse_step;
    const bool fused = c->opt_fuse && (stepf || (!sp.enabled && !ap.enabled)) && !d_outA && !d_outB && d_out && c->profiling < 2;
    if (c->any_enqueued && c->last_stream != s) LF_HIP(c, hipStreamSynchronize(c->last_stream));
    c->last_stream = s;
    c->any_enqueued = true;
    c->prof_pos = c->prof_tick++ % c->opt_profile_every;
    c->prof_this = c->profiling > 0 && c->prof_pos == 0;
    c->prof_span_ok = fused;
    if (fused && !c->queue_zero) {
        LF_HIP(c, hipMemsetAsync(c->d_queue, 0, (size_t)c->cap_queue * sizeof(int), s));
        c->queue_zero = true;
    }
    const bool poll = fused && c->opt_poll;
    if (poll && !c->parts_empty) {
        LF_HIP(c, hipMemsetD32Async((hipDeviceptr_t)c->d_partB, (int)(PART_EMPTY & 0xffffffffull), c->cap_partB * 2, s));
        LF_HIP(c, hipMemsetD32Async((hipDeviceptr_t)c->d_partR, (int)(PART_EMPTY & 0xffffffffull), c->cap_partR * 2, s));
        if (!c->d_err) {
            LF_HIP(c, hipMalloc((void**)&c->d_err, sizeof(int)));
            LF_HIP(c, hipMemsetAsync(c->d_err, 0, sizeof(int), s));
        }
        c->parts_empty = true;
    }
    if (!poll) c->parts_empty = false;
    if (!fused) {
        Prof p(c, s, 0);
        hipLaunchKernelGGL(lf_prepare, dim3((B + 7) / 8), dim3(64), 0, s, c->kc, sp, d_theta, B, c->d_wrec,
                           c->d_wstat, c->d_wmode, c->d_wbase, (int*)nullptr, c->d_queue, 0);
    }
    const PersArgs pa{B, ntiles, nchB, nchC, c->ncell, nslot, g8, c->d_queue, c->d_partA, c->d_partB, c->d_partR, c->d_nodes4, c->d_zcol,
                      c->d_cells, c->d_lum, c->d_a1, c->d_P, c->d_U, d_theta, d_out, c->d_wrec, c->d_wmode, c->d_wstat, poll ? 1 : 0, c->d_err};
    {
        Prof p(c, s, 1);
        const dim3 grid((unsigned)(8 * g8));
        const int info[8] = {0, PTW, PTW, fused ? 5 : 4, (int)grid.x, nchC, nchB, B};
        std::memcpy(c->last_launch, info, sizeof(info));
        if (fused && stepf) hipLaunchKernelGGL((lf_pers_step<VARIANT>), grid, dim3(PB), 0, s, c->kc, pa, sp, ap);
        else if (fused) hipLaunchKernelGGL((lf_pers<VARIANT, true>), grid, dim3(PB), 0, s, c->kc, pa);
        else hipLaunchKernelGGL((lf_pers<VARIANT, false>), grid, dim3(PB), 0, s, c->kc, pa);
    }
    if (!fused) {
        Prof p(c, s, 3);
        hipLaunchKernelGGL(lf_finalize, dim3(B), dim3(64), 0, s, c->d_partA, nslot, nslot, c->d_partB, nchB > 0 ? nslot : 0, nslot,
                           nchC > 0 ? (const double*)c->d_partR : (const double*)nullptr, nchC > 0 ? nslot : 0, (int)STAT_CELLS, c->d_wstat,
                           c->d_wbase, B, ap, d_out, d_outA, d_outB, (int*)nullptr, VARIANT == LF_FIXCOMP ? (int)STAT_SLOW : 0);
    }
    LF_HIP(c, hipGetLastError());
    return LF_OK;
}

int enqueue(lf_ctx* c, const double* d_theta, int B, double* d_out, double* d_outA, double* d_outB,
            hipStream_t s, const lf::StepArgs* step = nullptr, const lf::AcceptArgs* accept = nullptr) {
    using namespace lf;
    StepArgs sp{};
    AcceptArgs ap{};
    if (step) sp = *step;
    if (accept) ap = *accept;
    const bool shared_bins = c->kc.variant == LF_FREE && c->kc.grid_parts > 1 && c->gridq.built && c->opt_grid_shortcut && !c->opt_skip_grid;
    if (c->kc.variant == LF_FREE && c->opt_persistent && c->opt_geometry < 0 && c->opt_walker_tile == 0 && !c->opt_taper &&
        !(c->opt_compress && c->cmp.built) && (c->N >= 8192 || c->kc.cells || c->opt_persistent == 2 || shared_bins)) {
        const int64_t ntiles = (B + PTW - 1) / PTW;
        const int64_t items = free_shape(c).items_per_tile * ntiles;
        const bool plain = !sp.enabled && !ap.enabled && !d_outA && !d_outB && c->opt_fuse;
        const bool wins = c->kc.cells ? true : items >= 4 * 2 * (int64_t)std::max(c->num_cu, 1);
        (void)plain;
        if (wins || shared_bins || c->opt_persistent == 2 || c->opt_free_st)
            return enqueue_free(c, d_theta, B, d_out, d_outA, d_outB, s, sp, ap);
    }
    if (c->kc.variant != LF_FREE && c->opt_persistent && c->opt_geometry < 0 && c->opt_walker_tile == 0 && !c->opt_taper &&
        !(c->opt_compress && c->cmp.built) && !c->kc.forms && c->d_nodes4 &&
        (c->kc.variant == LF_FIXCOMP || (c->kc.cells && c->kc.zgrid_cols && c->kc.S <= PERS_MAXS))) {
        return c->kc.variant == LF_FIXCOMP ? enqueue_pers_v<LF_FIXCOMP>(c, d_theta, B, d_out, d_outA, d_outB, s, sp, ap)
                                           : enqueue_pers_v<LF_ZEVOL>(c, d_theta, B, d_out, d_outA, d_outB, s, sp, ap);
    }
    c->parts_empty = false;
    const bool cmp = c->opt_compress && c->cmp.built && c->kc.variant != LF_FIXCOMP;
    int gi = pick_geometry(c, B);
    if (cmp) {
        bool ok = false;
        for (int g : CMP_GEOS) ok = ok || g == gi;
        if (!ok || c->opt_geometry < 0) gi = CMP_GEOS[0];
    }
    const Geo geo = GEOS[gi];
    ChunkTable *ct = nullptr, *ctd = nullptr;
    const double* hz = c->kc.variant == LF_ZEVOL && !c->h_x.empty() ? c->h_x.data() : nullptr;
    int rc = cmp ? get_chunks(c, c->cmp.chunks, c->cmp.field_ind, geo.st * BLOCK, &ct)
                 : get_chunks(c, c->chunks, c->field_ind, geo.st * BLOCK, &ct, hz, hz ? geo.st : 0);
    if (rc != LF_OK) return rc;
    if (cmp && (rc = get_chunks(c, c->chunks, c->field_ind, geo.st * BLOCK, &ctd, hz, hz ? geo.st : 0)) != LF_OK) return rc;
    const int nchA = ct->n;
    const int nchD = cmp ? ctd->n : 0;
    const int nresc = cmp ? std::min(nchD, std::min(1024, std::max(128, 2 * B))) : 0;
    const bool cgrid = cmp && c->gridc.built && c->opt_compress_grid && !c->opt_skip_grid && c->kc.grid_parts <= 1;
    const int nchB = c->opt_skip_grid ? 0 : (cgrid ? (c->gridc.nb + 15) / 16 : (c->nnodes + BLOCK - 1) / BLOCK);
    const int nchC = !cmp && c->kc.variant == LF_ZEVOL && c->kc.cells ? c->ncchunk : 0;
    rc = ensure_workspace(c, B, (size_t)B * std::max(nchA, 1), (size_t)B * std::max(nchB, 1), (size_t)B * std::max(nchD, nchC));
    if (rc != LF_OK) return rc;
    c->zcells = ZCells{c->d_cells, c->d_cc_start, c->d_cc_len, c->d_cc_field, nchC, c->d_partR, c->d_wstat, 0};
    if (c->any_enqueued && c->last_stream != s) LF_HIP(c, hipStreamSynchronize(c->last_stream));
    c->last_stream = s;
    c->any_enqueued = true;
    c->prof_pos = c->prof_tick++ % c->opt_profile_every;
    c->prof_this = c->profiling > 0 && c->prof_pos == 0;
    c->prof_span_ok = false;

    {
        Prof p(c, s, 0);
        hipLaunchKernelGGL(lf_prepare, dim3((B + 7) / 8), dim3(64), 0, s, c->kc, sp, d_theta, B, c->d_wrec,
                           c->d_wstat, c->d_wmode, c->d_wbase, cmp ? c->d_slow : nullptr, c->d_queue, 0);
    }
    const SrcArrays sd{c->d_lum, c->d_a1, c->d_P, c->d_U, nullptr, ct->d_start, ct->d_len, ct->d_field, ct->d_keys, c->d_queue};
    SrcArrays sa = sd;
    Rescue rs{};
    GridC gc{};
    if (cgrid) {
        const auto& g = c->gridc;
        gc = GridC{g.d_U, g.d_A4, g.d_row0, g.d_nrows, g.d_off, g.d_omega, g.d_L, g.d_PGL, g.nb, c->kc.S};
    }
    if (cmp) {
        sa = SrcArrays{c->cmp.d_lum, c->cmp.d_a1, c->cmp.d_lum, c->cmp.d_U, c->cmp.d_W, ct->d_start, ct->d_len, ct->d_field, ct->d_keys, nullptr};
        rs.sd = sd;
        rs.sd.chunk_start = ctd->d_start;
        rs.sd.chunk_len = ctd->d_len;
        rs.sd.chunk_field = ctd->d_field;
        rs.sd.chunk_keys = ctd->d_keys;
        rs.slow_count = c->d_slow;
        rs.slow_list = c->d_slow + 1;
        rs.partR = c->d_partR;
        rs.nchD = nchD;
        rs.nresc = nresc;
    }
    NodeArrays na{c->d_G, c->d_PG, c->d_W, c->d_a3, c->d_a4, c->d_a4min, c->nnodes};
    {
        Prof p(c, s, 1);
        int tw = geo.tw, twb = geo.twb;
        if (cmp && nchB > 0) {
            const int64_t want = cgrid ? 768 : 2048;
            int t = 1;
            while (t < geo.twb && (int64_t)nchB * ((B + 2 * t - 1) / (2 * t)) >= want) t *= 2;
            twb = t;
        }
        if (cmp && nchA > 0) {
            int t = 1;
            while (t < geo.tw && (int64_t)nchA * ((B + 2 * t - 1) / (2 * t)) >= 1024) t *= 2;
            tw = t;
        }
        if (c->opt_walker_tile > 0) {
            tw = (int)std::min<int64_t>(c->opt_walker_tile, geo.tw);
            twb = (int)std::min<int64_t>(c->opt_walker_tile, geo.twb);
        }
        Tiling tl{tw, 0, B, std::max(1, tw / 4), 0};
        if (c->opt_taper && !cmp && B >= 2 * tw && tw >= 4) {
            const int tail = std::max(tw, ((B / 8 + tw - 1) / tw) * tw);
            tl.B1 = ((B - tail) / tw) * tw;
        }
        tl.ntiles = (tl.B1 + tw - 1) / tw;
        tl.ntiles_s = (B - tl.B1 + tl.tws - 1) / tl.tws;
        const int ntilesB = (B + twb - 1) / twb;
        const int nblkB = nchB * ntilesB;
        dim3 grid((unsigned)(nblkB + nchA * (tl.ntiles + tl.ntiles_s) + nresc));
        const int info[8] = {geo.st, geo.tw, geo.twb, cmp ? 1 : 0, (int)grid.x, nchA, nchB, B};
        std::memcpy(c->last_launch, info, sizeof(info));
        if (grid.x > 0) {
            if (cmp) {
                if (c->kc.variant == LF_FREE) launch_main_cmp<LF_FREE>(c, gi, grid, tl, ntilesB, twb, nblkB, s, sa, na, B, nchA, nchB, rs, gc);
                else launch_main_cmp<LF_ZEVOL>(c, gi, grid, tl, ntilesB, twb, nblkB, s, sa, na, B, nchA, nchB, rs, gc);
            } else switch (c->kc.variant) {
                case LF_FREE: launch_main<LF_FREE>(c, gi, grid, tl, ntilesB, twb, nblkB, s, sa, na, B, nchA, nchB, rs); break;
                case LF_FIXCOMP: launch_main<LF_FIXCOMP>(c, gi, grid, tl, ntilesB, twb, nblkB, s, sa, na, B, nchA, nchB, rs); break;
                default: launch_main<LF_ZEVOL>(c, gi, grid, tl, ntilesB, twb, nblkB, s, sa, na, B, nchA, nchB, rs);
            }
        }
    }
    {
        Prof p(c, s, 3);
        hipLaunchKernelGGL(lf_finalize, dim3(B), dim3(64), 0, s, c->d_partA, nchA, nchA, c->d_partB, nchB, nchB,
                           cmp || nchC > 0 ? c->d_partR : nullptr, cmp ? nchD : nchC, (int)(cmp ? STAT_SLOW : STAT_CELLS), c->d_wstat,
                           c->d_wbase, B, ap, d_out, d_outA, d_outB, cmp ? c->d_slow : nullptr,
                           !cmp && c->kc.variant == LF_FIXCOMP && nchA > 0 ? (int)STAT_SLOW : 0);
    }
    LF_HIP(c, hipGetLastError());
    return LF_OK;
}

void free_cmp(CompressedCat& cc) {
    for (auto& kv : cc.chunks) {
        hipFree(kv.second.d_start);
        hipFree(kv.second.d_len);
        hipFree(kv.second.d_field);
        hipFree(kv.second.d_keys);
    }
    cc.chunks.clear();
// ... 38 lines not shown
    const lfc::Bins bins = lfc::shared_bins(m, klo, khi);
    for (int f = 0; f < c->kc.nf; ++f) {
        const int64_t lo = c->field_ind[f], hi = c->field_ind[f + 1];
        if (!lfc::compress_field(m, key.data() + lo, wt.empty() ? nullptr : wt.data() + lo, hi - lo, out, &bins)) {
            c->err = "compress: the catalogue of field " + std::to_string(f) + " cannot be compressed to the error bound "
                     "(non-finite coordinate, or a prior box the bins cannot resolve)";
            return LF_ERR_ARG;
        }
        {
            const size_t a = (size_t)cc.field_ind.back(), b = out.node.size();
            std::vector<size_t> idx(b - a);
            for (size_t i = 0; i < idx.size(); ++i) idx[i] = a + i;
            std::stable_sort(idx.begin(), idx.end(), [&](size_t x, size_t y) { return out.node[x] < out.node[y]; });
            std::vector<double> nn(idx.size()), ww(idx.size());
            for (size_t i = 0; i < idx.size(); ++i) {
                nn[i] = out.node[idx[i]];
                ww[i] = out.weight[idx[i]];
            }
            std::copy(nn.begin(), nn.end(), out.node.begin() + (std::ptrdiff_t)a);
            std::copy(ww.begin(), ww.end(), out.weight.begin() + (std::ptrdiff_t)a);
        }
        cc.field_ind.push_back((int64_t)out.node.size());
    }
    cc.n = (int64_t)out.node.size();
    cc.nbins = out.nbins;
    cc.bound = out.bound;
    std::vector<double> lumc((size_t)cc.n, c->kc.variant == LF_ZEVOL ? LF_LREF : 0.0), U((size_t)cc.n);
    for (int64_t i = 0; i < cc.n; ++i)
        U[(size_t)i] = c->kc.variant == LF_FREE ? std::pow(10.0, out.node[(size_t)i] - LF_FREF) : out.node[(size_t)i] * out.node[(size_t)i];
    int rc;
    if ((rc = upload(c, &cc.d_lum, lumc.data(), (size_t)cc.n)) != LF_OK || (rc = upload(c, &cc.d_a1, out.node.data(), (size_t)cc.n)) != LF_OK ||
        (rc = upload(c, &cc.d_U, U.data(), (size_t)cc.n)) != LF_OK || (rc = upload(c, &cc.d_W, out.weight.data(), (size_t)cc.n)) != LF_OK) {
        free_cmp(cc);
        return rc;
    }
    cc.built = true;
    c->cmp = cc;
    if (c->kc.variant == LF_FREE && !c->h_L.empty() && !c->gridc.built) {
        lfc::Model mg = m;
        mg.kind = 2;
        lfc::GridOut go;
        const int S = c->kc.S;
        if (lfc::compress_grid(mg, S, c->h_L.data(), c->h_wL.data(), c->h_ck.data(), c->h_Dk.data(), go)) {
            std::vector<double> A4(go.u.size()), PGL((size_t)S);
            for (size_t i = 0; i < go.u.size(); ++i) A4[i] = std::pow(10.0, go.u[i] - LF_FREF);
            for (int j = 0; j < S; ++j) PGL[(size_t)j] = std::pow(10.0, c->h_L[(size_t)j] - LF_LREF);
            auto& g = c->gridc;
            if ((rc = upload(c, &g.d_U, go.u.data(), go.u.size())) != LF_OK) return rc;
            if ((rc = upload(c, &g.d_A4, A4.data(), A4.size())) != LF_OK) return rc;
            if ((rc = upload(c, &g.d_omega, go.omega.data(), go.omega.size())) != LF_OK) return rc;
            if ((rc = upload(c, &g.d_L, c->h_L.data(), (size_t)S)) != LF_OK) return rc;
            if ((rc = upload(c, &g.d_PGL, PGL.data(), (size_t)S)) != LF_OK) return rc;
            if ((rc = upload(c, &g.d_row0, go.row0.data(), go.row0.size())) != LF_OK) return rc;
            if ((rc = upload(c, &g.d_nrows, go.nrows.data(), go.nrows.size())) != LF_OK) return rc;
            if ((rc = upload(c, &g.d_off, go.off.data(), go.off.size())) != LF_OK) return rc;
            g.nb = go.nb;
            g.bound = go.bound;
            g.built = true;
        }
    }
    return LF_OK;
}

int compress_selfcheck(lf_ctx* c) {
    using namespace lf;
    const int B = 64, nd = c->kc.ndim, nf = c->kc.nf;
    std::vector<double> th((size_t)B * nd), direct(B), comp(B);
    uint64_t st = 0x9e3779b97f4a7c15ull;
    auto uni = [&]() {
        uint64_t z = (st += 0x9e3779b97f4a7c15ull);
        z = (z ^ (z >> 30)) * 0xbf58476d1ce4e5b9ull;
        z = (z ^ (z >> 27)) * 0x94d049bb133111ebull;
        return (double)((z ^ (z >> 31)) >> 11) * 1.1102230246251565e-16;
    };
    auto in = [&](int lim, double lo_frac) {
        const double lo = c->kc.lims[lim][0], hi = c->kc.lims[lim][1];
        return lo + (hi - lo) * (lo_frac + (1.0 - lo_frac) * uni());
    };
    for (int b = 0; b < B; ++b) {
        double* t = th.data() + (size_t)b * nd;
        int k = 0;
        if (c->kc.variant == LF_ZEVOL) {
            for (int i = 0; i < 3; ++i) t[k++] = in(LF_LIM_LSTAR, 0.3);
            for (int i = 0; i < 3; ++i) t[k++] = in(LF_LIM_PHISTAR, 0.0);
            if (!c->kc.fix_sch_al) t[k++] = in(LF_LIM_SCH_AL, 0.0);
        } else {
            t[k++] = in(LF_LIM_LSTAR, 0.3);
            t[k++] = in(LF_LIM_PHISTAR, 0.0);
            if (!c->kc.fix_sch_al) t[k++] = in(LF_LIM_SCH_AL, 0.0);
            if (c->kc.variant == LF_FREE) {
                for (int f = 0; f < nf; ++f) t[k++] = in(LF_LIM_FLIM, 0.0);
                t[k++] = in(LF_LIM_ALPHA, 0.0);
            }
        }
    }
    const int64_t was = c->opt_compress;
    int rc = ensure_workspace(c, B, 0, 0);
    for (int pass = 0; pass < 2 && rc == LF_OK; ++pass) {
        c->opt_compress = pass;
        LF_HIP(c, hipMemcpy(c->d_theta, th.data(), th.size() * sizeof(double), hipMemcpyHostToDevice));
        rc = enqueue(c, c->d_theta, B, c->d_out, nullptr, nullptr, c->stream);
        if (rc != LF_OK) break;
        LF_HIP(c, hipStreamSynchronize(c->stream));
        LF_HIP(c, hipMemcpy(pass ? comp.data() : direct.data(), c->d_out, B * sizeof(double), hipMemcpyDeviceToHost));
    }
    c->opt_compress = was;
    if (rc != LF_OK) return rc;
    double worst = 0.0;
    int nfin = 0;
    for (int b = 0; b < B; ++b) {
        if (std::isinf(direct[b]) || std::isinf(comp[b])) {
            if (direct[b] != comp[b]) worst = HUGE_VAL;
            continue;
        }
        ++nfin;
        worst = std::fmax(worst, std::fabs(comp[b] - direct[b]) / std::fmax(std::fabs(direct[b]), 1e-300));
    }
    if (!(worst <= 1.0e-12)) {
        char msg[200];
        std::snprintf(msg, sizeof(msg), "compress: the compressed catalogue differs from the direct path by %.3g (relative) on "
                      "%d of 64 self-check walkers of this prior box: option refused", worst, nfin);
        c->err = msg;
        return LF_ERR_ARG;
    }
    return LF_OK;
}

void free_ctx(lf_ctx* c) {
    if (!c) return;
    hipSetDevice(c->device);
    if (c->stream) hipStreamSynchronize(c->stream);
    for (auto& e : c->events) {
        hipEventDestroy(e.a);
        hipEventDestroy(e.b);
    }
    for (auto& kv : c->chunks) {
        hipFree(kv.second.d_start);
        hipFree(kv.second.d_len);
        hipFree(kv.second.d_field);
        hipFree(kv.second.d_keys);
    }
    for (auto& kv : c->chunks_free) {
        hipFree(kv.second.d_start);
        hipFree(kv.second.d_len);
        hipFree(kv.second.d_field);
        hipFree(kv.second.d_keys);
    }
    free_cmp(c->cmp);
    if (c->d_partR) hipFree(c->d_partR);
    if (c->d_cells) hipFree(c->d_cells);
    if (c->d_cc_start) hipFree(c->d_cc_start);
    if (c->d_deal) hipFree(c->d_deal);
    if (c->d_err) hipFree(c->d_err);
    if (c->d_cc_len) hipFree(c->d_cc_len);
    if (c->d_cc_field) hipFree(c->d_cc_field);
    {
        auto& g = c->gridc;
        double* gb[] = {g.d_U, g.d_A4, g.d_omega, g.d_L, g.d_PGL};
        for (double* b : gb)
            if (b) hipFree(b);
        int* gi_[] = {g.d_row0, g.d_nrows, g.d_off};
        for (int* b : gi_)
            if (b) hipFree(b);
        if (c->d_nodes4) hipFree(c->d_nodes4);
        if (c->d_zcol) hipFree(c->d_zcol);
        if (c->gridq.d_rec) hipFree(c->gridq.d_rec);
        if (c->gridq.d_omega) hipFree(c->gridq.d_omega);
        if (c->gridq.d_rows) hipFree(c->gridq.d_rows);
    }
    double* bufs[] = {c->d_lum, c->d_a1, c->d_P, c->d_U, c->d_G, c->d_PG, c->d_W, c->d_a3, c->d_a4, c->d_a4min, c->d_nodes8,
                      c->d_theta, c->d_out, c->d_outA, c->d_outB, c->d_wrec, c->d_partA, c->d_partB};
    for (double* b : bufs)
        if (b) hipFree(b);
    if (c->d_wstat) hipFree(c->d_wstat);
    if (c->d_wmode) hipFree(c->d_wmode);
    if (c->d_wbase) hipFree(c->d_wbase);
    if (c->d_slow) hipFree(c->d_slow);
    if (c->d_forms) hipFree(c->d_forms);
    if (c->d_queue) hipFree(c->d_queue);
    if (c->h_theta) hipHostFree(c->h_theta);
    if (c->h_out) hipHostFree(c->h_out);
    if (c->stream) hipStreamDestroy(c->stream);
    delete c;
}

int build(lf_ctx* c, const lf_desc* d) {
    using namespace lf;
    const int nf = d->nf, S = d->S;
    const int64_t N = d->N;
    KConst& kc = c->kc;
    kc.variant = d->variant;
    kc.fix_sch_al = d->fix_sch_al ? 1 : 0;
    kc.specialise = 1;
    kc.grid_part = 0;
    kc.grid_parts = 1;
    kc.tables = 1;
    kc.key_x0 = 0.0;
    kc.forms = nullptr;
#ifdef LF_STAMPS
    kc.stamps = nullptr;
#endif
    kc.nf = nf;
    kc.S = S;
    if (d->variant == LF_FREE) kc.ndim = 2 + (kc.fix_sch_al ? 0 : 1) + nf + 1;
    else if (d->variant == LF_FIXCOMP) kc.ndim = 2 + (kc.fix_sch_al ? 0 : 1);
    else kc.ndim = 6 + (kc.fix_sch_al ? 0 : 1);
    for (int f = 0; f < MAXF; ++f) {
        kc.lnom0_src[f] = 0.0;
        kc.om0_grid[f] = 0.0;
        kc.flim0[f] = 0.0;
    }
    for (int f = 0; f < nf; ++f) {
        kc.lnom0_src[f] = std::log(std::trunc(d->omega0[f]) / LF_SQARCSEC);
        kc.om0_grid[f] = d->omega0[f] / LF_SQARCSEC;
        if (d->flim0) kc.flim0[f] = d->flim0[f];
    }
    {
        const double a = (2.0 * d->fcmin - 1.0) * (2.0 * d->fcmin - 1.0);
        kc.fc_ratio = std::fabs(a / (1.0 - a));
    }
    std::memcpy(kc.lims, d->lims, sizeof(kc.lims));
    std::memcpy(kc.pivots, d->pivots, sizeof(kc.pivots));
    kc.sch_al0 = d->sch_al0;
    kc.alpha0 = d->alpha0;
    c->N = N;
    c->nnodes = S * S;
    c->field_ind.assign(d->field_ind, d->field_ind + nf + 1);

    std::vector<int64_t> perm((size_t)N);
    for (int64_t i = 0; i < N; ++i) perm[(size_t)i] = i;
    if (d->variant == LF_FREE || d->variant == LF_ZEVOL) {
        const double* key = d->variant == LF_FREE ? d->logf : d->z;
        for (int f = 0; f < nf; ++f)
            std::stable_sort(perm.begin() + d->field_ind[f], perm.begin() + d->field_ind[f + 1], [&](int64_t a, int64_t b) {
                const double x = key[a], y = key[b];
                return std::isnan(y) ? !std::isnan(x) : x < y;
            });
    }
    std::vector<double> lumv(N), a1(N), P(N), U(N);
    for (int64_t i = 0; i < N; ++i) lumv[(size_t)i] = d->lum[perm[(size_t)i]];
    for (int64_t i = 0; i < N; ++i) {
        const double lum = lumv[(size_t)i];
        if (d->variant == LF_FREE) {
            a1[i] = d->logf[perm[(size_t)i]];
            P[i] = std::pow(10.0, lum - LF_LREF);
            U[i] = std::pow(10.0, d->logf[perm[(size_t)i]] - LF_FREF);
        } else if (d->variant == LF_FIXCOMP) {
            a1[i] = std::log(d->om_arr[perm[(size_t)i]]);
            P[i] = std::pow(10.0, lum - LF_LREF);
            U[i] = 0.0;
        } else {
            a1[i] = d->z[perm[(size_t)i]];
            P[i] = std::log(d->om_arr[perm[(size_t)i]]);
            U[i] = d->z[perm[(size_t)i]] * d->z[perm[(size_t)i]];
        }
    }
    for (int f = 0; f < MAXF; ++f) {
        kc.nsrc[f] = 0;
        kc.pmax[f] = kc.lum_min[f] = kc.lum_max[f] = kc.a_min[f] = kc.u_min[f] = kc.u_max[f] = kc.z_lo[f] = kc.z_hi[f] = kc.slc[f] = kc.sp[f] = kc.som[f] = kc.sz[f] = kc.sz2[f] = 0.0;
    }
    for (int f = 0; f < nf; ++f) {
        const int64_t lo = d->field_ind[f], hi = d->field_ind[f + 1];
        kc.nsrc[f] = (int)(hi - lo);
        if (hi <= lo) continue;
        double pmax = -HUGE_VAL, lmin = HUGE_VAL, lmax = -HUGE_VAL, amin = HUGE_VAL, amax = -HUGE_VAL, zlo = HUGE_VAL, zhi = -HUGE_VAL;
        bool nan = false;
        long double slc = 0.0L, sp = 0.0L, som = 0.0L, sz = 0.0L, sz2 = 0.0L;
        for (int64_t i = lo; i < hi; ++i) {
            const double lum = lumv[(size_t)i];
            slc += (long double)(lum - LF_LREF);
            if (d->variant != LF_ZEVOL) sp += (long double)P[i];
            if (d->variant == LF_FIXCOMP) som += (long double)a1[i];
            if (d->variant == LF_ZEVOL) {
                som += (long double)P[i];
                sz += (long double)d->z[perm[(size_t)i]];
                sz2 += (long double)U[i];
            }
            lmin = std::fmin(lmin, lum);
            lmax = std::fmax(lmax, lum);
            nan = nan || std::isnan(lum);
            if (d->variant != LF_ZEVOL) pmax = std::fmax(pmax, P[i]);
            const double a = d->variant == LF_FREE ? a1[i] : (d->variant == LF_FIXCOMP ? a1[i] : P[i]);
            amin = std::fmin(amin, a);
            amax = std::fmax(amax, a);
            nan = nan || std::isnan(a);
            if (d->variant == LF_ZEVOL) {
                zlo = std::fmin(zlo, d->z[perm[(size_t)i]]);
                zhi = std::fmax(zhi, d->z[perm[(size_t)i]]);
                nan = nan || std::isnan(d->z[perm[(size_t)i]]);
            }
        }
        if (nan) amin = -HUGE_VAL;
        kc.pmax[f] = pmax;
        kc.lum_min[f] = lmin;
        kc.lum_max[f] = lmax;
        kc.a_min[f] = amin;
        kc.u_min[f] = d->variant == LF_FREE ? std::pow(10.0, amin - LF_FREF) : 0.0;
        kc.u_max[f] = d->variant == LF_FREE ? (nan ? HUGE_VAL : std::pow(10.0, amax - LF_FREF)) : 0.0;
        kc.z_lo[f] = zlo;
        kc.z_hi[f] = zhi;
        kc.slc[f] = (double)slc;
        kc.sp[f] = (double)sp;
        kc.som[f] = (double)som;
        kc.sz[f] = (double)sz;
        kc.sz2[f] = (double)sz2;
    }
// ... 109 lines not shown
    }
    if (d->variant == LF_FIXCOMP && !std::getenv("LF_NO_COLLAPSE_GRID")) {
        bool sep = true;
        for (int j = 0; j < S && sep; ++j)
            for (int k = 1; k < S; ++k)
                if (d->logL[(size_t)j * S + k] != d->logL[(size_t)j * S]) {
                    sep = false;
                    break;
                }
        if (sep) {
            for (int j = 0; j < S; ++j) {
                long double rs = 0.0L;
                for (int k = 0; k < S; ++k) rs += (long double)W[(size_t)j * S + k];
                G[(size_t)j] = G[(size_t)j * S];
                PG[(size_t)j] = PG[(size_t)j * S];
                W[(size_t)j] = (double)rs;
                a3[(size_t)j] = a4[(size_t)j] = 0.0;
            }
            nn = (size_t)S;
            c->nnodes = S;
        }
    }
    if ((rc = upload(c, &c->d_G, G.data(), nn)) != LF_OK) return rc;
    if ((rc = upload(c, &c->d_PG, PG.data(), nn)) != LF_OK) return rc;
    if ((rc = upload(c, &c->d_W, W.data(), nn)) != LF_OK) return rc;
    if ((rc = upload(c, &c->d_a3, a3.data(), nn)) != LF_OK) return rc;
    if ((rc = upload(c, &c->d_a4, a4.data(), nn)) != LF_OK) return rc;
    if (d->variant != LF_FREE) {
        const size_t nch = (nn + 63) / 64;
        std::vector<double> n4(nch * 64 * 4, 0.0);
        for (size_t g = 0; g < nch * 64; ++g) {
            const size_t gg = std::min(g, nn - 1);
            double* r = &n4[g * 4];
            r[0] = G[gg];
            r[1] = PG[gg];
            r[2] = g < nn ? W[gg] : 0.0;
            r[3] = kc.zgrid_cols ? (double)(gg / (size_t)S) : 0.0;
        }
        if ((rc = upload(c, &c->d_nodes4, n4.data(), n4.size())) != LF_OK) return rc;
        c->nch4 = (int)nch;
        std::vector<double> zc((size_t)S * 2);
        for (int k = 0; k < S; ++k) {
            zc[(size_t)2 * k] = d->zarr[k];
            zc[(size_t)2 * k + 1] = d->zarr[k] * d->zarr[k];
        }
        if ((rc = upload(c, &c->d_zcol, zc.data(), zc.size())) != LF_OK) return rc;
    }
    {
        std::vector<double> a4min((nn + lf::BLOCK - 1) / lf::BLOCK, 0.0);
        for (size_t ch = 0; ch < a4min.size(); ++ch) {
            double m = HUGE_VAL;
            for (size_t g = ch * lf::BLOCK; g < std::min(nn, (ch + 1) * lf::BLOCK); ++g) m = std::isnan(a4[g]) ? 0.0 : std::fmin(m, a4[g]);
            a4min[ch] = d->variant == LF_FREE ? m : 0.0;
        }
        if ((rc = upload(c, &c->d_a4min, a4min.data(), a4min.size())) != LF_OK) return rc;
        if (d->variant == LF_FREE) {
            const size_t nch64 = (nn + 63) / 64;
            std::vector<double> n8(nch64 * 64 * 8, 0.0);
            for (size_t ch = 0; ch < nch64; ++ch) {
                double m = HUGE_VAL;
                for (size_t g = ch * 64; g < std::min(nn, (ch + 1) * 64); ++g) m = std::isnan(a4[g]) ? 0.0 : std::fmin(m, a4[g]);
                for (size_t l = 0; l < 64; ++l) {
                    const size_t g = std::min(ch * 64 + l, nn - 1);
                    double* r = &n8[(ch * 64 + l) * 8];
                    r[0] = G[g];
                    r[1] = PG[g];
                    r[2] = ch * 64 + l < nn ? W[g] : 0.0;
                    r[3] = a3[g];
                    r[4] = a4[g];
                    r[5] = m;
                }
            }
            if ((rc = upload(c, &c->d_nodes8, n8.data(), n8.size())) != LF_OK) return rc;
        }
    }
    {
        hipDeviceProp_t prop;
        LF_HIP(c, hipGetDeviceProperties(&prop, c->device));
        c->num_cu = prop.multiProcessorCount;
        LF_HIP(c, hipMalloc((void**)&c->d_queue, 1024 * sizeof(int)));
        LF_HIP(c, hipMemset(c->d_queue, 0, 1024 * sizeof(int)));
        c->cap_queue = 1024;
    }
    LF_HIP(c, hipStreamCreateWithFlags(&c->stream, hipStreamNonBlocking));
    const int mb = d->max_batch > 0 ? d->max_batch : 1024;
    return ensure_workspace(c, mb, 0, 0);
}

}

extern "C" {

int lf_deal_table(int n_cell_chunks, int n_bins, int grid_part, int grid_parts, int32_t* table, int64_t cap) {
    using namespace lf;
    if (n_cell_chunks < 0 || n_bins < 0 || grid_parts < 0 || grid_part < 0 || (grid_parts > 0 && grid_part >= grid_parts)) return LF_ERR_ARG;
    const int64_t n = (int64_t)DEAL_LIST + n_cell_chunks + n_bins;
    if (!table) return (int)n;
    if (cap < n) return LF_ERR_ARG;
    const std::vector<int> t = make_deal(n_cell_chunks, n_bins, grid_part, grid_parts);
    for (int64_t i = 0; i < n; ++i) table[i] = t[(size_t)i];
    return (int)n;
}

int lf_abi_version(void) { return LF_ABI_VERSION; }

const char* lf_last_error(const lf_ctx* ctx) { return ctx ? ctx->err.c_str() : g_create_error.c_str(); }

lf_ctx* lf_create(const lf_desc* d) {
    g_create_error.clear();
    if (!d) {
        g_create_error = "lf_create: NULL descriptor";
        return nullptr;
    }
    auto bad = [&](const char* m) {
        g_create_error = std::string("lf_create: ") + m;
        return (lf_ctx*)nullptr;
    };
    if (d->variant < LF_FREE || d->variant > LF_ZEVOL) return bad("unknown variant");
    if (d->nf < 1 || d->nf > LF_MAX_FIELDS) return bad("nf out of range (1..LF_MAX_FIELDS)");
    if (d->S < 2 || d->S > 4096) return bad("S out of range");
    if (d->N < 0 || d->N > 2000000000LL) return bad("N out of range");
    if (!d->field_ind || !d->omega0 || !d->logL || !d->zarr) return bad("NULL field_ind/omega0/logL/zarr");
    if (d->N > 0 && !d->lum) return bad("NULL lum");
    if (d->field_ind[0] != 0 || d->field_ind[d->nf] != d->N) return bad("field_ind must span [0, N]");
    for (int f = 0; f < d->nf; ++f)
        if (d->field_ind[f + 1] < d->field_ind[f]) return bad("field_ind must be non-decreasing");
    if (!(d->fcmin > 0.0 && d->fcmin < 1.0) || d->fcmin == 0.5) return bad("fcmin must be in (0,1), != 0.5");
    if (d->variant == LF_FREE) {
        if ((d->N > 0 && !d->logf) || !d->volume_part || !d->dl_zarr) return bad("FREE needs logf, volume_part, dl_zarr");
    } else {
        if ((d->N > 0 && !d->om_arr) || !d->integ_part) return bad("FIXCOMP/ZEVOL need om_arr, integ_part");
        if (d->variant == LF_FIXCOMP && !d->flim0) return bad("FIXCOMP needs flim0");
        if (d->variant == LF_ZEVOL && d->N > 0 && !d->z) return bad("ZEVOL needs z");
        if (d->variant == LF_ZEVOL && (d->pivots[0] == d->pivots[1] || d->pivots[0] == d->pivots[2] ||
                                       d->pivots[1] == d->pivots[2]))
            return bad("ZEVOL pivots must be distinct");
    }
    int ndev = 0;
    if (hipGetDeviceCount(&ndev) != hipSuccess || ndev <= 0) return bad("no HIP device visible");
    if (d->device < 0 || d->device >= ndev) return bad("device ordinal out of range");
    hipDeviceProp_t prop;
    if (hipGetDeviceProperties(&prop, d->device) != hipSuccess) return bad("hipGetDeviceProperties failed");
    if (std::strncmp(prop.gcnArchName, "gfx950", 6) != 0) {
        g_create_error = std::string("lf_create: device is ") + prop.gcnArchName + ", this library is built for gfx950 only";
        return nullptr;
    }
    if (hipSetDevice(d->device) != hipSuccess) return bad("hipSetDevice failed");
    lf_ctx* c = new (std::nothrow) lf_ctx();
    if (!c) return bad("out of host memory");
    c->device = d->device;
    int rc = LF_OK;
    try {
        rc = build(c, d);
    } catch (const std::bad_alloc&) {
        c->err = "out of host memory";
        rc = LF_ERR_NOMEM;
    }
    if (rc != LF_OK) {
        g_create_error = "lf_create: " + c->err;
        free_ctx(c);
        return nullptr;
    }
    return c;
}

void lf_destroy(lf_ctx* ctx) { free_ctx(ctx); }

int lf_ndim(const lf_ctx* ctx) { return ctx ? ctx->kc.ndim : LF_ERR_ARG; }

int lf_lnprob_batch_device(lf_ctx* c, const double* d_theta, int B, double* d_out, void* hip_stream) {
    if (!c) return LF_ERR_ARG;
    if (!d_theta || !d_out || B <= 0) {
        c->err = "lf_lnprob_batch_device: NULL pointer or B <= 0";
        return LF_ERR_ARG;
    }
    LF_HIP(c, hipSetDevice(c->device));
    return enqueue(c, d_theta, B, d_out, nullptr, nullptr, (hipStream_t)hip_stream);
}

int lf_lnprob_batch_device_n(lf_ctx* c, const double* d_theta, int B, int K, double* d_out, void* hip_stream) {
    if (!c) return LF_ERR_ARG;
    if (!d_theta || !d_out || B <= 0 || K <= 0) {
        c->err = "lf_lnprob_batch_device_n: NULL pointer, B <= 0 or K <= 0";
        return LF_ERR_ARG;
    }
    LF_HIP(c, hipSetDevice(c->device));
    const size_t nd = (size_t)c->kc.ndim;
    for (int k = 0; k < K; ++k) {
        const int rc = enqueue(c, d_theta + (size_t)k * B * nd, B, d_out + (size_t)k * B, nullptr, nullptr, (hipStream_t)hip_stream);
        if (rc != LF_OK) return rc;
    }
    return LF_OK;
}

static int host_eval(lf_ctx* c, const double* theta, int B, double* out, double* outA, double* outB) {
    using namespace lf;
    if (!c) return LF_ERR_ARG;
    if (!theta || B <= 0 || (!out && !(outA && outB))) {
        c->err = "lf_lnprob_batch: NULL pointer or B <= 0";
        return LF_ERR_ARG;
    }
    LF_HIP(c, hipSetDevice(c->device));
    int rc = ensure_workspace(c, B, 0, 0);
    if (rc != LF_OK) return rc;
    const size_t tb = (size_t)B * c->kc.ndim * sizeof(double);
    std::memcpy(c->h_theta, theta, tb);
    LF_HIP(c, hipMemcpyAsync(c->d_theta, c->h_theta, tb, hipMemcpyHostToDevice, c->stream));
    rc = enqueue(c, c->d_theta, B, c->d_out, outA ? c->d_outA : nullptr, outB ? c->d_outB : nullptr, c->stream);
    if (rc != LF_OK) return rc;
    const size_t ob = (size_t)B * sizeof(double);
    LF_HIP(c, hipMemcpyAsync(c->h_out, c->d_out, ob, hipMemcpyDeviceToHost, c->stream));
    if (outA) {
        LF_HIP(c, hipMemcpyAsync(c->h_out + B, c->d_outA, ob, hipMemcpyDeviceToHost, c->stream));
        LF_HIP(c, hipMemcpyAsync(c->h_out + 2 * (size_t)B, c->d_outB, ob, hipMemcpyDeviceToHost, c->stream));
    }
    LF_HIP(c, hipStreamSynchronize(c->stream));
    if (out && c->d_err) {
        bool nan = false;
        for (int i = 0; i < B; ++i) nan = nan || c->h_out[i] != c->h_out[i];
        if (nan) {
            int e = 0;
            LF_HIP(c, hipMemcpy(&e, c->d_err, sizeof(int), hipMemcpyDeviceToHost));
            if (e) {
                c->err = "lf_lnprob_batch: a tile's finishing workgroup waited in vain for the tile's partial sums (device stalled?)";
                return LF_ERR_HIP;
            }
        }
    }
    if (out) std::memcpy(out, c->h_out, ob);
    if (outA) {
        std::memcpy(outA, c->h_out + B, ob);
        std::memcpy(outB, c->h_out + 2 * (size_t)B, ob);
    }
    return LF_OK;
}

int lf_lnprob_batch(lf_ctx* c, const double* theta, int B, double* out) {
    if (c && !out) {
        c->err = "lf_lnprob_batch: NULL out";
        return LF_ERR_ARG;
    }
    return host_eval(c, theta, B, out, nullptr, nullptr);
}

int lf_lnprob_pieces(lf_ctx* c, const double* theta, int B, double* outA, double* outB) {
    if (c && (!outA || !outB)) {
        c->err = "lf_lnprob_pieces: NULL output";
        return LF_ERR_ARG;
    }
    return host_eval(c, theta, B, nullptr, outA, outB);
}

int lf_set_profiling(lf_ctx* c, int enabled) {
    if (!c) return LF_ERR_ARG;
    c->profiling = enabled < 0 ? 0 : (enabled > 2 ? 2 : enabled);
    return LF_OK;
}

int lf_kernel_times(lf_ctx* c, double ms[4], int64_t launches[4]) {
    if (!c || !ms || !launches) return LF_ERR_ARG;
    LF_HIP(c, hipSetDevice(c->device));
    if (c->span_open) {
        if (c->span_ep.count > 0) {
            hipEventRecord(c->span_ep.b, c->last_stream);
            c->events.push_back(c->span_ep);
        } else {
            hipEventDestroy(c->span_ep.a);
            hipEventDestroy(c->span_ep.b);
        }
        c->span_open = false;
    }
    for (auto& e : c->events) {
        LF_HIP(c, hipEventSynchronize(e.b));
        float t = 0.f;
        LF_HIP(c, hipEventElapsedTime(&t, e.a, e.b));
        c->acc_ms[e.kind] += t;
        c->acc_n[e.kind] += e.count;
        hipEventDestroy(e.a);
        hipEventDestroy(e.b);
    }
    c->events.clear();
    for (int i = 0; i < 4; ++i) {
        ms[i] = c->acc_ms[i];
        launches[i] = c->acc_n[i];
        c->acc_ms[i] = 0;
        c->acc_n[i] = 0;
    }
    return LF_OK;
}

#ifdef LF_STAMPS
int lf_debug_stamps(lf_ctx* c, uint64_t* out, int64_t nblocks) {
    if (!c) return LF_ERR_ARG;
    LF_HIP(c, hipSetDevice(c->device));
    LF_HIP(c, hipDeviceSynchronize());
    if (!out) {
        if (c->kc.stamps) hipFree(c->kc.stamps);
        c->kc.stamps = nullptr;
        if (nblocks > 0) {
            LF_HIP(c, hipMalloc((void**)&c->kc.stamps, (size_t)nblocks * 8 * sizeof(uint64_t)));
            LF_HIP(c, hipMemset(c->kc.stamps, 0, (size_t)nblocks * 8 * sizeof(uint64_t)));
        }
        return LF_OK;
    }
    if (!c->kc.stamps) return LF_ERR_ARG;
    LF_HIP(c, hipMemcpy(out, c->kc.stamps, (size_t)nblocks * 8 * sizeof(uint64_t), hipMemcpyDeviceToHost));
// ... 533 lines not shown
```

Before: 9.515 million walker-lnprob evals/s.

## Move invariant kernel arguments into a cached device-resident constant block

Splits the large by-value kernel argument structs into a per-launch LaunchArgs (theta, out, sizes) and a FreeCtx/PersCtx block holding the invariant pointers and constants. The block is uploaded once to a device buffer and re-copied only when its bytes change. Kernels receive a pointer to it instead of copying everything into the kernarg segment. This shrinks per-launch argument size and setup cost, at the price of an extra indirection (global/scalar loads) inside the kernel and a device synchronize whenever the block changes.

```diff
diff --git a/lumfuncmcmc_amd/csrc/lf_free.h b/lumfuncmcmc_amd/csrc/lf_free.h
--- a/lumfuncmcmc_amd/csrc/lf_free.h
+++ b/lumfuncmcmc_amd/csrc/lf_free.h
@@ -27,11 +27,17 @@
     }
 }
 
+struct LaunchArgs {
+    const double* theta;
+    double* out;
+    int B, ntiles;
+    int tile_stride;
+    int nslot;
+    int poll;
+};
+
 struct FreeArgs {
-    int B, ntiles;
     int nchA, nchB;
-    int nslot;
-    int tile_stride;
     int skip_grid;
     int* queues;
     double* partA;
@@ -44,8 +50,6 @@
     int nchC;
     double* partC;
     const int* wstat;
-    const double* theta;
-    double* out;
     double* wrec_w;
     int* wmode_w;
     int* wstat_w;
@@ -54,16 +58,22 @@
     const double* gq_omega;
     const int* gq_rows;
     int nbq;
-    int poll;
     int* err;
 };
 
+struct FreeCtx {
+    KConst kc;
+    SrcArrays sa;
+    NodeArrays na;
+    FreeArgs fa;
+};
+
 template <int ST, bool CENSUS, bool FUSED, bool STEP>
 __device__ __forceinline__ void lf_free_body(const KConst& kc, const SrcArrays& sa, const NodeArrays& na, const double* __restrict__ wrec_arg,
-                                             const int* __restrict__ wmode_arg, const FreeArgs& fa, const StepArgs& sp, const AcceptArgs& ap,
-                                             unsigned long long t_pre = 0) {
-    const double* wrec = FUSED ? fa.wrec_w : wrec_arg;
-    const int* wmode = FUSED ? fa.wmode_w : wmode_arg;
+                                             const int* __restrict__ wmode_arg, const FreeArgs& fa, const LaunchArgs& la, const StepArgs& sp,
+                                             const AcceptArgs& ap, unsigned long long t_pre = 0) {
+    const double* wrec = FUSED ? glb(fa.wrec_w) : wrec_arg;
+    const int* wmode = FUSED ? glb(fa.wmode_w) : wmode_arg;
     auto pstore = [](double* p, double v) {
         if (FUSED) __hip_atomic_store(p, v == v ? v : __builtin_nan(""), __ATOMIC_RELAXED, __HIP_MEMORY_SCOPE_AGENT);
         else *p = v;
@@ -90,7 +100,7 @@
             tab.expt[i] = EXP_TABLE[i];
         }
         load_term_tables<PB>(&tt);
-        if (fa.deal && tid < DEAL_LIST + fa.nchC + fa.nbq) sdeal[tid] = fa.deal[tid];
+        if (fa.deal && tid < DEAL_LIST + fa.nchC + fa.nbq) sdeal[tid] = glb(fa.deal)[tid];
     }
     bool tables_loaded = !FUSED;
     const int wave_base = __builtin_amdgcn_readfirstlane(tid & ~63);
@@ -104,7 +114,7 @@
     const int myq = (int)(xcc & 7u);
 #ifdef LF_STAMPS
     __shared__ unsigned long long s_targs;
-    unsigned long long* stamp = kc.stamps ? kc.stamps + (size_t)blockIdx.x * 8 : nullptr;
+    unsigned long long* stamp = kc.stamps ? glb(kc.stamps) + (size_t)blockIdx.x * 8 : nullptr;
     if (stamp && tid == 0) {
         stamp[0] = t_pre ? t_pre : __builtin_amdgcn_s_memtime();
         stamp[5] = __builtin_amdgcn_s_memrealtime();
@@ -119,16 +129,16 @@
 #endif
 
 #pragma unroll 1
-    for (int tile = ((int)blockIdx.x >> 3) % fa.ntiles; tile < fa.ntiles; tile += fa.tile_stride) {
+    for (int tile = ((int)blockIdx.x >> 3) % la.ntiles; tile < la.ntiles; tile += la.tile_stride) {
         const int w0 = tile * PTW;
-        const int nw = min(PTW, fa.B - w0);
+        const int nw = min(PTW, la.B - w0);
         __builtin_assume(nw >= 1 && nw <= PTW);
-        int* __restrict__ q = fa.queues + tile * QSTRIDE;
+        int* __restrict__ q = glb(fa.queues) + tile * QSTRIDE;
         int fgroup = 8, frank = (int)blockIdx.x & 7;
-        if (fa.ntiles <= fa.tile_stride) {
+        if (la.ntiles <= la.tile_stride) {
             const int k = (int)blockIdx.x >> 3;
-            fgroup = 8 * ((fa.tile_stride - tile + fa.ntiles - 1) / fa.ntiles);
-            frank += 8 * ((k - tile) / fa.ntiles);
+            fgroup = 8 * ((la.tile_stride - tile + la.ntiles - 1) / la.ntiles);
+            frank += 8 * ((k - tile) / la.ntiles);
         }
         bool no_src = false;
         auto grab = [&]() -> int {
@@ -152,13 +162,13 @@
             if (ticket < hi - lo) return lo + ticket;
             return grab();
         };
-        if (tile != ((int)blockIdx.x >> 3) % fa.ntiles) __syncthreads();
+        if (tile != ((int)blockIdx.x >> 3) % la.ntiles) __syncthreads();
         const int u = fresh_tid();
         if (FUSED) {
             const int pw = (int)(blockIdx.x >> 8) & 1;
             const int up = u - 64 * pw;
             if (up >= 0 && up < 64) {
-                prepare_lane<false, true, STEP, LF_FREE>(kc, sp, fa.theta, fa.B, nullptr, nullptr, nullptr, nullptr, nullptr, 1,
+                prepare_lane<false, true, STEP, LF_FREE>(kc, sp, la.theta, la.B, nullptr, nullptr, nullptr, nullptr, nullptr, 1,
                                           w0 + (up >> 3), up & 7, up >> 3, reinterpret_cast<double(*)[16]>(red), wfc, wsc, sstat, sbase, wlf,
 #ifdef LF_STAMPS
                                           s_tprep,
@@ -174,7 +184,7 @@
                 double2 lt = *reinterpret_cast<const double2*>(LOG_TABLE + 2 * min(t7, 255));
                 double et = EXP_TABLE[min(t7, 255)];
                 const int ndeal = fa.deal ? DEAL_LIST + fa.nchC + fa.nbq : 0;
-                int d0 = ndeal ? fa.deal[min(t7, ndeal - 1)] : 0, d1 = ndeal ? fa.deal[min(t7 + 256, ndeal - 1)] : 0;
+                int d0 = ndeal ? glb(fa.deal)[min(t7, ndeal - 1)] : 0, d1 = ndeal ? glb(fa.deal)[min(t7 + 256, ndeal - 1)] : 0;
                 asm volatile("" : "+v"(lt.x), "+v"(lt.y), "+v"(et), "+v"(d0), "+v"(d1));
                 load_term_tables<PB - 64>(&tt, t7);
                 if (t7 < 256) {
@@ -197,7 +207,7 @@
             __syncthreads();
         }
         if (u < 64) {
-            const int st = FUSED ? sstat[min(u, nw - 1)] : fa.wstat[w0 + min(u, nw - 1)];
+            const int st = FUSED ? sstat[min(u, nw - 1)] : glb(fa.wstat)[w0 + min(u, nw - 1)];
             const bool on = fa.nchC > 0 && u < nw && (st & STAT_CELLS);
             const bool need = u < nw && !on && (st & STAT_PRIOR_OK) && !(st & STAT_NEGINF);
             const int m = (int)__ballot(on);
@@ -258,7 +268,7 @@
             if (fa.nchC > 0 && v < nw && ((cellmask >> v) & 1) && cn > 0) {
                 auto load_cells = [&](double (&d)[CELL_REC], int cc) {
                     const int lane = fresh_tid() & 63;
-                    const double2* __restrict__ src = reinterpret_cast<const double2*>(fa.cells + ((size_t)cc * 64 + lane) * CELL_REC);
+                    const double2* __restrict__ src = reinterpret_cast<const double2*>(glb(fa.cells) + ((size_t)cc * 64 + lane) * CELL_REC);
                     static_assert(CELL_REC % 2 == 0, "16-byte loads");
 #pragma unroll
                     for (int k = 0; k < CELL_REC / 2; ++k) {
@@ -286,13 +296,13 @@
                     asm volatile("; LF_BEGIN cell items=1");
                     acc += cell_sum(cd, p, &tt);
                     asm volatile("; LF_END cell");
-                    if (CENSUS && kc.forms && (fresh_tid() & 63) == 0) atomicAdd(kc.forms + FORM_CELL, (unsigned long long)uni(fa.cc_len[cc]));
+                    if (CENSUS && kc.forms && (fresh_tid() & 63) == 0) atomicAdd(glb(kc.forms) + FORM_CELL, (unsigned long long)uni(glb(fa.cc_len)[cc]));
                 }
             }
             if (fa.nchC > 0 && v < nw) {
                 acc = wave_sum_dpp(acc);
                 const int ln = fresh_tid() & 63;
-                double* __restrict__ row = fa.partC + (size_t)(w0 + v) * fa.nslot;
+                double* __restrict__ row = glb(fa.partC) + (size_t)(w0 + v) * la.nslot;
                 if (ln == 63) pstore(row + vr, acc);
             }
             }
@@ -324,7 +334,7 @@
                 };
                 auto load_rec = [&](int c) -> QRec {
                     const int lane = fresh_tid() & 63;
-                    const double2* __restrict__ src = reinterpret_cast<const double2*>(fa.gq_rec + ((size_t)c * 64 + lane) * 4);
+                    const double2* __restrict__ src = reinterpret_cast<const double2*>(glb(fa.gq_rec) + ((size_t)c * 64 + lane) * 4);
                     const double2 a = src[0], b = src[1];
                     return QRec{a.x, a.y, b.x, b.y};
                 };
@@ -334,11 +344,11 @@
                 for (int qi = 0; qi < qn; ++qi) {
                     const int c = bin_at(qi);
                     const QRec nd = nx;
-                    const int nr = uni(fa.gq_rows[4 * c + 1]), off = uni(fa.gq_rows[4 * c + 2]);
+                    const int nr = uni(glb(fa.gq_rows)[4 * c + 1]), off = uni(glb(fa.gq_rows)[4 * c + 2]);
                     if (qi + 1 < qn) nx = load_rec(bin_at(qi + 1));
                     if (mine(c)) {
                         const int lane = fresh_tid() & 63;
-                        const double* __restrict__ om = fa.gq_omega + off + lane;
+                        const double* __restrict__ om = glb(fa.gq_omega) + off + lane;
                         double o[8];
 #pragma unroll
                         for (int i = 0; i < 8; ++i) o[i] = i < nr ? om[i * 64] : 0.0;
@@ -349,7 +359,7 @@
                                                               __builtin_amdgcn_readlane(__double2loint(nd.a4), 63));
                         const bool bright = kc.specialise && alphaC > 0.0 && a4min * vmin > 37.5;
                         if (CENSUS && kc.forms && lane == 0)
-                            atomicAdd(kc.forms + (bright ? FORM_NODE_BRIGHT : FORM_NODE_GENERAL), (unsigned long long)(64 * kc.nf));
+                            atomicAdd(glb(kc.forms) + (bright ? FORM_NODE_BRIGHT : FORM_NODE_GENERAL), (unsigned long long)(64 * kc.nf));
                         const double s = field_sum_nf(kc, r, alphaC, nd.x, nd.a4, &tab, bright);
                         __builtin_amdgcn_wave_barrier();
                         asm volatile("; LF_BEGIN qdot items=1");
@@ -373,7 +383,7 @@
             if (v < nw) {
                 bsum = wave_sum_dpp(bsum);
                 const int ln = fresh_tid() & 63;
-                double* __restrict__ row = fa.partB + (size_t)(w0 + v) * fa.nslot;
+                double* __restrict__ row = glb(fa.partB) + (size_t)(w0 + v) * la.nslot;
                 if (ln == 63) pstore(row + vr, bsum);
             }
             }
@@ -398,7 +408,7 @@
                 };
                 auto load_nodes = [&](int c) -> Node {
                     const int lane = fresh_tid() & 63;
-                    const double2* __restrict__ src = reinterpret_cast<const double2*>(fa.nodes8 + ((size_t)c * 64 + lane) * 8);
+                    const double2* __restrict__ src = reinterpret_cast<const double2*>(glb(fa.nodes8) + ((size_t)c * 64 + lane) * 8);
                     const double2 a = src[0], b = src[1], d = src[2];
                     return Node{a.x, a.y, b.x, b.y, d.x, d.y};
                 };
@@ -412,7 +422,7 @@
                         const double T = fexp_c(fma(uni(sc[R_C1]), nd.G - uni(sc[R_LSTAR]), uni(sc[R_C0])) - nd.PG * uni(sc[R_Q]), &tab);
                         const bool bright = kc.specialise && alphaC > 0.0 && a4min * vmin > 37.5;
                         if (CENSUS && kc.forms && (fresh_tid() & 63) == 0)
-                            atomicAdd(kc.forms + (bright ? FORM_NODE_BRIGHT : FORM_NODE_GENERAL),
+                            atomicAdd(glb(kc.forms) + (bright ? FORM_NODE_BRIGHT : FORM_NODE_GENERAL),
                                       (unsigned long long)(min(64, na.nnodes - c * 64) * kc.nf));
                         const double s = field_sum_nf(kc, r, alphaC, nd.a3, nd.a4, &tab, bright);
                         bsum = fma(nd.W * T, s, bsum);
@@ -422,7 +432,7 @@
             if (nch64 > 0 && v < nw) {
                 bsum = wave_sum_dpp(bsum);
                 const int ln = fresh_tid() & 63;
-                double* __restrict__ row = fa.partB + (size_t)(w0 + v) * fa.nslot;
+                double* __restrict__ row = glb(fa.partB) + (size_t)(w0 + v) * la.nslot;
                 if (ln == 63) pstore(row + vr, bsum);
             }
             }
@@ -442,14 +452,14 @@
             int t = fresh_tid();
             {
                 const int c = item;
-                const int s0 = uni(sa.chunk_start[c]), n = uni(sa.chunk_len[c]), fld = uni(sa.chunk_field[c]);
-                const int kfirst = uni(sa.chunk_keys[KEY_STRIDE * c]), klast = uni(sa.chunk_keys[KEY_STRIDE * c + 1]),
-                          kamax = uni(sa.chunk_keys[KEY_STRIDE * c + 4 + (wave_base >> 6)]);
+                const int s0 = uni(glb(sa.chunk_start)[c]), n = uni(glb(sa.chunk_len)[c]), fld = uni(glb(sa.chunk_field)[c]);
+                const int kfirst = uni(glb(sa.chunk_keys)[KEY_STRIDE * c]), klast = uni(glb(sa.chunk_keys)[KEY_STRIDE * c + 1]),
+                          kamax = uni(glb(sa.chunk_keys)[KEY_STRIDE * c + 4 + (wave_base >> 6)]);
                 double x[ST];
                 if (t == 0) take_ticket();
                 if (n == PB * ST) {
                     typedef double __attribute__((ext_vector_type(2), aligned(8))) double2_a8;
-                    const double2_a8* __restrict__ src = reinterpret_cast<const double2_a8*>(sa.a1 + s0 + t * ST);
+                    const double2_a8* __restrict__ src = reinterpret_cast<const double2_a8*>(glb(sa.a1) + s0 + t * ST);
 #pragma unroll
                     for (int k = 0; k < ST / 2; ++k) {
                         const double2_a8 a = src[k];
@@ -457,7 +467,7 @@
                         x[2 * k + 1] = a.y;
                     }
                 } else {
-                    const double* __restrict__ src = sa.a1 + s0;
+                    const double* __restrict__ src = glb(sa.a1) + s0;
 #pragma unroll
                     for (int k = 0; k < ST; ++k) x[k] = src[min(t * ST + k, n - 1)];
                 }
@@ -485,18 +495,18 @@
                             table_lookup<ST>(C, x, p, true, &tt);
                             acc = table_terms<ST, true>(C, x, npad);
                             asm volatile("; LF_END table_noexp");
-                            if (CENSUS && kc.forms && (t & 63) == 0) atomicAdd(kc.forms + FORM_TABLE_NOEXP, (unsigned long long)nwave);
+                            if (CENSUS && kc.forms && (t & 63) == 0) atomicAdd(glb(kc.forms) + FORM_TABLE_NOEXP, (unsigned long long)nwave);
                         } else {
                             asm volatile("; LF_BEGIN table items=%0" ::"n"(ST));
                             table_lookup<ST>(C, x, p, false, &tt);
                             acc = table_terms<ST, false>(C, x, npad);
                             asm volatile("; LF_END table");
-                            if (CENSUS && kc.forms && (t & 63) == 0) atomicAdd(kc.forms + FORM_TABLE, (unsigned long long)nwave);
+                            if (CENSUS && kc.forms && (t & 63) == 0) atomicAdd(glb(kc.forms) + FORM_TABLE, (unsigned long long)nwave);
                         }
                     } else if (p.mode < MODE_SKIP) {
                         rest |= 1 << w;
                     } else if (CENSUS && kc.forms && (t & 63) == 0) {
-                        atomicAdd(kc.forms + FORM_SKIPPED, (unsigned long long)nwave);
+                        atomicAdd(glb(kc.forms) + FORM_SKIPPED, (unsigned long long)nwave);
                     }
                     red[w * PB + t] = acc;
                 }
@@ -504,7 +514,7 @@
                     t = fresh_tid();
                     double u[ST];
                     {
-                        const double* __restrict__ up = sa.U + s0;
+                        const double* __restrict__ up = glb(sa.U) + s0;
 #pragma unroll
                         for (int k = 0; k < ST; ++k) u[k] = up[min(t * ST + k, n - 1)];
                     }
@@ -527,7 +537,7 @@
 #pragma unroll 1
                             for (int i = t; i < n; i += PB) {
                                 const size_t g = (size_t)s0 + i;
-                                acc += term_free_careful(wf, sa.lum[g], sa.a1[g], sa.P[g], sa.U[g]);
+                                acc += term_free_careful(wf, glb(sa.lum)[g], glb(sa.a1)[g], glb(sa.P)[g], glb(sa.U)[g]);
                             }
                         } else {
                             WFree wf{};
@@ -557,7 +567,7 @@
                                 }
                             }
                         }
-                        if (CENSUS && kc.forms && (t & 63) == 0) atomicAdd(kc.forms + form, (unsigned long long)nwave);
+                        if (CENSUS && kc.forms && (t & 63) == 0) atomicAdd(glb(kc.forms) + form, (unsigned long long)nwave);
                         red[w * PB + t] = acc;
                     }
                 }
@@ -566,7 +576,7 @@
 #endif
                 __syncthreads();
                 t = fresh_tid();
-                reduce_store512<FUSED>(red, 0, nw, fa.partA, (size_t)fa.nchA, w0, c, t);
+                reduce_store512<FUSED>(red, 0, nw, glb(fa.partA), (size_t)fa.nchA, w0, c, t);
                 item = sitem[0];
             }
 #ifdef LF_STAMPS
@@ -578,13 +588,13 @@
             }
 #endif
         }
-        if (FUSED && fa.poll && uni(snosrc)) {
+        if (FUSED && la.poll && uni(snosrc)) {
             if (frank == fgroup - 1) {
                 const int t = fresh_tid(), v = t >> 6, ln = t & 63;
-                const int nB = fa.nchB > 0 ? fa.nslot : 0, nC = fa.nchC > 0 ? fa.nslot : 0;
+                const int nB = fa.nchB > 0 ? la.nslot : 0, nC = fa.nchC > 0 ? la.nslot : 0;
                 if (v < nw) {
-                    double* __restrict__ pb = fa.partB + (size_t)(w0 + v) * fa.nslot;
-                    double* __restrict__ pc = fa.partC + (size_t)(w0 + v) * fa.nslot;
+                    double* __restrict__ pb = glb(fa.partB) + (size_t)(w0 + v) * la.nslot;
+                    double* __restrict__ pc = glb(fa.partC) + (size_t)(w0 + v) * la.nslot;
                     double pre[2] = {0.0, 0.0};
                     int tries = 0;
                     bool have;
@@ -596,12 +606,12 @@
                     } while (!__all(have) && ++tries < PART_POLLS);
                     if (tries >= PART_POLLS) {
                         pre[0] = pre[1] = __builtin_nan("");
-                        if (ln == 0) atomicExch(fa.err, 1);
+                        if (ln == 0) atomicExch(glb(fa.err), 1);
                     }
                     if (ln < nC) __hip_atomic_store(pc + ln, __longlong_as_double((long long)PART_EMPTY), __ATOMIC_RELAXED, __HIP_MEMORY_SCOPE_AGENT);
                     if (ln < nB) __hip_atomic_store(pb + ln, __longlong_as_double((long long)PART_EMPTY), __ATOMIC_RELAXED, __HIP_MEMORY_SCOPE_AGENT);
-                    finalize_wave<true>(fa.partA, 0, fa.nchA, fa.partB, nB, nB, nC > 0 ? fa.partC : nullptr, nC, (int)STAT_CELLS,
-                                        sstat - w0, sbase - w0, w0 + v, ln, ap, fa.out, nullptr, nullptr, 0,
+                    finalize_wave<true>(glb(fa.partA), 0, fa.nchA, glb(fa.partB), nB, nB, nC > 0 ? glb(fa.partC) : nullptr, nC, (int)STAT_CELLS,
+                                        sstat - w0, sbase - w0, w0 + v, ln, ap, la.out, nullptr, nullptr, 0,
                                         STEP ? sprop + v * 16 : nullptr, STEP ? szz + v : nullptr, STEP ? spre + 2 * v : nullptr, pre);
                 }
             }
@@ -614,15 +624,15 @@
             if (sitem[1] == fgroup - 1) {
                 __builtin_amdgcn_fence(__ATOMIC_ACQUIRE, "workgroup");
                 const int t = fresh_tid(), v = t >> 6;
-                const int nB = fa.nchB > 0 ? fa.nslot : 0, nC = fa.nchC > 0 ? fa.nslot : 0;
+                const int nB = fa.nchB > 0 ? la.nslot : 0, nC = fa.nchC > 0 ? la.nslot : 0;
                 if (v < nw) {
-                    finalize_wave<true>(fa.partA, fa.nchA, fa.nchA, fa.partB, nB, nB, nC > 0 ? fa.partC : nullptr, nC, (int)STAT_CELLS,
-                                        sstat - w0, sbase - w0, w0 + v, t & 63, ap, fa.out, nullptr, nullptr, 0,
+                    finalize_wave<true>(glb(fa.partA), fa.nchA, fa.nchA, glb(fa.partB), nB, nB, nC > 0 ? glb(fa.partC) : nullptr, nC, (int)STAT_CELLS,
+                                        sstat - w0, sbase - w0, w0 + v, t & 63, ap, la.out, nullptr, nullptr, 0,
                                         STEP ? sprop + v * 16 : nullptr, STEP ? szz + v : nullptr, STEP ? spre + 2 * v : nullptr);
-                    if (fa.poll) {
+                    if (la.poll) {
                         const int ln = t & 63;
-                        if (ln < nC) __hip_atomic_store(fa.partC + (size_t)(w0 + v) * fa.nslot + ln, __longlong_as_double((long long)PART_EMPTY), __ATOMIC_RELAXED, __HIP_MEMORY_SCOPE_AGENT);
-                        if (ln < nB) __hip_atomic_store(fa.partB + (size_t)(w0 + v) * fa.nslot + ln, __longlong_as_double((long long)PART_EMPTY), __ATOMIC_RELAXED, __HIP_MEMORY_SCOPE_AGENT);
+                        if (ln < nC) __hip_atomic_store(glb(fa.partC) + (size_t)(w0 + v) * la.nslot + ln, __longlong_as_double((long long)PART_EMPTY), __ATOMIC_RELAXED, __HIP_MEMORY_SCOPE_AGENT);
+                        if (ln < nB) __hip_atomic_store(glb(fa.partB) + (size_t)(w0 + v) * la.nslot + ln, __longlong_as_double((long long)PART_EMPTY), __ATOMIC_RELAXED, __HIP_MEMORY_SCOPE_AGENT);
                     }
                 }
                 if (t < QSTRIDE) q[t] = 0;
@@ -648,28 +658,30 @@
             stamp[7] = t_loop;
         }
         stamp[6] = __builtin_amdgcn_s_memrealtime();
-        kc.stamps[(size_t)gridDim.x * 8 + blockIdx.x] =
+        glb(kc.stamps)[(size_t)gridDim.x * 8 + blockIdx.x] =
             !noitems ? t_red : (((s_ttab - stamp[0]) << 32) | ((s_tp0 - stamp[0]) & 0xffffffffull));
     }
 #endif
 }
 
 template <int ST, bool CENSUS, bool FUSED = false>
-__global__ __launch_bounds__(PB, 4) void lf_free(KConst kc, SrcArrays sa, NodeArrays na, const double* __restrict__ wrec_arg,
-                                                 const int* __restrict__ wmode_arg, FreeArgs fa) {
+__global__ __launch_bounds__(PB, 4) void lf_free(const FreeCtx* __restrict__ cb, const double* __restrict__ wrec_arg,
+                                                 const int* __restrict__ wmode_arg, LaunchArgs la) {
 #ifdef LF_STAMPS
     const unsigned long long t_pre = __builtin_amdgcn_s_memtime();
 #else
     const unsigned long long t_pre = 0;
 #endif
-    warm_kernarg<sizeof(KConst) + sizeof(SrcArrays) + sizeof(NodeArrays) + 2 * 8 + sizeof(FreeArgs)>();
-    lf_free_body<ST, CENSUS, FUSED, false>(kc, sa, na, wrec_arg, wmode_arg, fa, StepArgs{}, AcceptArgs{}, t_pre);
+    static_assert(sizeof(FreeCtx*) + 2 * 8 + sizeof(LaunchArgs) <= 64, "the kernel arguments fit one line");
+    const FreeCtx& k = const_block(cb);
+    lf_free_body<ST, CENSUS, FUSED, false>(k.kc, k.sa, k.na, wrec_arg, wmode_arg, k.fa, la, StepArgs{}, AcceptArgs{}, t_pre);
 }
 
 template <int ST>
-__global__ __launch_bounds__(PB, 4) void lf_free_step(KConst kc, SrcArrays sa, NodeArrays na, FreeArgs fa, StepArgs sp, AcceptArgs ap) {
-    warm_kernarg<sizeof(KConst) + sizeof(SrcArrays) + sizeof(NodeArrays) + sizeof(FreeArgs) + sizeof(StepArgs) + sizeof(AcceptArgs)>();
-    lf_free_body<ST, false, true, true>(kc, sa, na, nullptr, nullptr, fa, sp, ap);
+__global__ __launch_bounds__(PB, 4) void lf_free_step(const FreeCtx* __restrict__ cb, LaunchArgs la, StepArgs sp, AcceptArgs ap) {
+    warm_kernarg<sizeof(FreeCtx*) + sizeof(LaunchArgs) + sizeof(StepArgs) + sizeof(AcceptArgs)>();
+    const FreeCtx& k = const_block(cb);
+    lf_free_body<ST, false, true, true>(k.kc, k.sa, k.na, nullptr, nullptr, k.fa, la, sp, ap);
 }
 
 }
diff --git a/lumfuncmcmc_amd/csrc/lf_math.h b/lumfuncmcmc_amd/csrc/lf_math.h
--- a/lumfuncmcmc_amd/csrc/lf_math.h
+++ b/lumfuncmcmc_amd/csrc/lf_math.h
@@ -172,36 +172,39 @@
     return v;
 }
 
-#define LF_KW1(o) "s_load_dword %0, %1, " #o "\n\t"
-#define LF_KW4(b) LF_KW1(b + 0x00) LF_KW1(b + 0x40) LF_KW1(b + 0x80) LF_KW1(b + 0xc0)
+template <int OFF, int BYTES, typename P>
+__device__ __forceinline__ void warm_line(P p, int& t) {
+    if constexpr (OFF < BYTES) {
+        constexpr int at = OFF + 4 <= BYTES ? OFF : BYTES - 4;
+        static_assert(at >= 0 && at + 4 <= BYTES, "a load past the end of the range");
+        asm volatile("s_load_dword %0, %1, %2" : "+s"(t) : "s"(p), "n"(at));
+        warm_line<OFF + 64, BYTES>(p, t);
+    }
+}
+template <int BYTES, typename P>
+__device__ __forceinline__ void warm_lines(P p) {
+    static_assert(BYTES >= 4 && BYTES <= 4096, "range");
+    int t = 0;
+    warm_line<0, BYTES>(p, t);
+    asm volatile("s_waitcnt lgkmcnt(0)" : "+s"(t) : : "memory");
+}
 template <int BYTES>
 __device__ __forceinline__ void warm_kernarg() {
-    constexpr int N4 = (BYTES + 255) / 256;
-    static_assert(N4 >= 1 && N4 <= 10, "extend the ladder");
-    auto p = __builtin_amdgcn_kernarg_segment_ptr();
-    int t;
-    if constexpr (N4 == 1) asm volatile(LF_KW4(0x000) "s_waitcnt lgkmcnt(0)" : "=&s"(t) : "s"(p) : "memory");
-    if constexpr (N4 == 2) asm volatile(LF_KW4(0x000) LF_KW4(0x100) "s_waitcnt lgkmcnt(0)" : "=&s"(t) : "s"(p) : "memory");
-    if constexpr (N4 == 3) asm volatile(LF_KW4(0x000) LF_KW4(0x100) LF_KW4(0x200) "s_waitcnt lgkmcnt(0)" : "=&s"(t) : "s"(p) : "memory");
-    if constexpr (N4 == 4)
-        asm volatile(LF_KW4(0x000) LF_KW4(0x100) LF_KW4(0x200) LF_KW4(0x300) "s_waitcnt lgkmcnt(0)" : "=&s"(t) : "s"(p) : "memory");
-    if constexpr (N4 == 5)
-        asm volatile(LF_KW4(0x000) LF_KW4(0x100) LF_KW4(0x200) LF_KW4(0x300) LF_KW4(0x400) "s_waitcnt lgkmcnt(0)" : "=&s"(t) : "s"(p) : "memory");
-    if constexpr (N4 == 6)
-        asm volatile(LF_KW4(0x000) LF_KW4(0x100) LF_KW4(0x200) LF_KW4(0x300) LF_KW4(0x400) LF_KW4(0x500) "s_waitcnt lgkmcnt(0)"
-                     : "=&s"(t) : "s"(p) : "memory");
-    if constexpr (N4 == 7)
-        asm volatile(LF_KW4(0x000) LF_KW4(0x100) LF_KW4(0x200) LF_KW4(0x300) LF_KW4(0x400) LF_KW4(0x500) LF_KW4(0x600) "s_waitcnt lgkmcnt(0)"
-                     : "=&s"(t) : "s"(p) : "memory");
-    if constexpr (N4 == 8)
-        asm volatile(LF_KW4(0x000) LF_KW4(0x100) LF_KW4(0x200) LF_KW4(0x300) LF_KW4(0x400) LF_KW4(0x500) LF_KW4(0x600) LF_KW4(0x700)
-                     "s_waitcnt lgkmcnt(0)" : "=&s"(t) : "s"(p) : "memory");
-    if constexpr (N4 == 9)
-        asm volatile(LF_KW4(0x000) LF_KW4(0x100) LF_KW4(0x200) LF_KW4(0x300) LF_KW4(0x400) LF_KW4(0x500) LF_KW4(0x600) LF_KW4(0x700)
-                     LF_KW4(0x800) "s_waitcnt lgkmcnt(0)" : "=&s"(t) : "s"(p) : "memory");
-    if constexpr (N4 == 10)
-        asm volatile(LF_KW4(0x000) LF_KW4(0x100) LF_KW4(0x200) LF_KW4(0x300) LF_KW4(0x400) LF_KW4(0x500) LF_KW4(0x600) LF_KW4(0x700)
-                     LF_KW4(0x800) LF_KW4(0x900) "s_waitcnt lgkmcnt(0)" : "=&s"(t) : "s"(p) : "memory");
-}
-
-}
+    warm_lines<BYTES>(__builtin_amdgcn_kernarg_segment_ptr());
+}
+
+template <typename T>
+__device__ __forceinline__ T* glb(T* const& field) {
+    typedef __attribute__((address_space(1))) T GT;
+    return (T*)*static_cast<GT* const*>(static_cast<const void*>(&field));
+}
+
+template <typename T>
+__device__ __forceinline__ const T& const_block(const T* p) {
+    static_assert(alignof(T) <= 64, "64-byte aligned block");
+    warm_lines<(int)sizeof(T)>(p);
+    typedef const __attribute__((address_space(4))) T CT;
+    return *(const T*)(CT*)(unsigned long long)p;
+}
+
+}
diff --git a/lumfuncmcmc_amd/csrc/lf_pers.h b/lumfuncmcmc_amd/csrc/lf_pers.h
--- a/lumfuncmcmc_amd/csrc/lf_pers.h
+++ b/lumfuncmcmc_amd/csrc/lf_pers.h
@@ -6,11 +6,8 @@
 constexpr int PERS_MAXS = 256;
 
 struct PersArgs {
-    int B, ntiles;
     int nchB;
     int nchC, ncell;
-    int nslot;
-    int tile_stride;
     int* queues;
     double* partA;
     double* partB;
@@ -22,17 +19,19 @@
     const double* a1;
     const double* P;
     const double* U;
-    const double* theta;
-    double* out;
     const double* wrec;
     const int* wmode;
     const int* wstat;
-    int poll;
     int* err;
 };
 
+struct PersCtx {
+    KConst kc;
+    PersArgs pa;
+};
+
 template <int VARIANT, bool FUSED, bool STEP>
-__device__ __forceinline__ void lf_pers_body(const KConst& kc, const PersArgs& pa, const StepArgs& sp, const AcceptArgs& ap) {
+__device__ __forceinline__ void lf_pers_body(const KConst& kc, const PersArgs& pa, const LaunchArgs& la, const StepArgs& sp, const AcceptArgs& ap) {
     static_assert(VARIANT == LF_ZEVOL || VARIANT == LF_FIXCOMP, "the free variant has lf_free");
     auto pstore = [](double* p, double v) {
         if (FUSED) __hip_atomic_store(p, v == v ? v : __builtin_nan(""), __ATOMIC_RELAXED, __HIP_MEMORY_SCOPE_AGENT);
@@ -56,7 +55,7 @@
     const int lane = tid & 63, v = wave_base >> 6;
     bool tables_loaded = false;
 #ifdef LF_STAMPS
-    unsigned long long* stamp = kc.stamps ? kc.stamps + (size_t)blockIdx.x * 8 : nullptr;
+    unsigned long long* stamp = kc.stamps ? glb(kc.stamps) + (size_t)blockIdx.x * 8 : nullptr;
     unsigned long long t_prep = 0, t_cols = 0, t_cells = 0, t_grid = 0;
     if (stamp && tid == 0) {
         stamp[0] = __builtin_amdgcn_s_memtime();
@@ -65,23 +64,23 @@
 #endif
 
 #pragma unroll 1
-    for (int tile = ((int)blockIdx.x >> 3) % pa.ntiles; tile < pa.ntiles; tile += pa.tile_stride) {
+    for (int tile = ((int)blockIdx.x >> 3) % la.ntiles; tile < la.ntiles; tile += la.tile_stride) {
         const int w0 = tile * PTW;
-        const int nw = min(PTW, pa.B - w0);
+        const int nw = min(PTW, la.B - w0);
         __builtin_assume(nw >= 1 && nw <= PTW);
-        int* __restrict__ q = pa.queues + tile * QSTRIDE;
+        int* __restrict__ q = glb(pa.queues) + tile * QSTRIDE;
         int fgroup = 8, frank = (int)blockIdx.x & 7;
-        if (pa.ntiles <= pa.tile_stride) {
+        if (la.ntiles <= la.tile_stride) {
             const int k = (int)blockIdx.x >> 3;
-            fgroup = 8 * ((pa.tile_stride - tile + pa.ntiles - 1) / pa.ntiles);
-            frank += 8 * ((k - tile) / pa.ntiles);
+            fgroup = 8 * ((la.tile_stride - tile + la.ntiles - 1) / la.ntiles);
+            frank += 8 * ((k - tile) / la.ntiles);
         }
         __syncthreads();
         if (FUSED) {
             const int pw = (int)(blockIdx.x >> 8) & 1;
             const int up = tid - 64 * pw;
             if (up >= 0 && up < 64) {
-                prepare_lane<false, true, STEP, VARIANT>(kc, sp, pa.theta, pa.B, nullptr, nullptr, nullptr, nullptr, nullptr, 0, w0 + (up >> 3), up & 7,
+                prepare_lane<false, true, STEP, VARIANT>(kc, sp, la.theta, la.B, nullptr, nullptr, nullptr, nullptr, nullptr, 0, w0 + (up >> 3), up & 7,
                                                 up >> 3, reinterpret_cast<double(*)[16]>(red), wfc, wsc, sstat, sbase, nullptr, nullptr, sprop, szz);
             } else if (!tables_loaded && tid >= 128 && tid < 128 + 256) {
                 int fm = -1;
@@ -89,7 +88,7 @@
                 const int t = wave_base + __builtin_amdgcn_mbcnt_hi(fm, __builtin_amdgcn_mbcnt_lo(fm, 0)) - 128;
                 double2 lt = *reinterpret_cast<const double2*>(LOG_TABLE + 2 * t);
                 double et = EXP_TABLE[t];
-                double2 zz = VARIANT == LF_ZEVOL ? *reinterpret_cast<const double2*>(pa.zcol + 2 * min(t, kc.S - 1)) : double2{0.0, 0.0};
+                double2 zz = VARIANT == LF_ZEVOL ? *reinterpret_cast<const double2*>(glb(pa.zcol) + 2 * min(t, kc.S - 1)) : double2{0.0, 0.0};
                 asm volatile("" : "+v"(lt.x), "+v"(lt.y), "+v"(et), "+v"(zz.x), "+v"(zz.y));
                 tab.logt[t] = lt;
                 tab.expt[t] = et;
@@ -100,7 +99,7 @@
                 const int t = tid - 256;
                 double2 lt = *reinterpret_cast<const double2*>(LOG_TABLE + 2 * t);
                 double et = EXP_TABLE[t];
-                double2 zz = VARIANT == LF_ZEVOL ? *reinterpret_cast<const double2*>(pa.zcol + 2 * min(t, kc.S - 1)) : double2{0.0, 0.0};
+                double2 zz = VARIANT == LF_ZEVOL ? *reinterpret_cast<const double2*>(glb(pa.zcol) + 2 * min(t, kc.S - 1)) : double2{0.0, 0.0};
                 asm volatile("" : "+v"(lt.x), "+v"(lt.y), "+v"(et), "+v"(zz.x), "+v"(zz.y));
                 tab.logt[t] = lt;
                 tab.expt[t] = et;
@@ -108,14 +107,14 @@
             }
             if (tid < nw * MAXF) {
                 const int w = tid / MAXF, f = tid - w * MAXF;
-                wfc[tid * 8] = pa.wrec[(size_t)(w0 + w) * REC + RF(f, 0)];
-                reinterpret_cast<int*>(wfc + tid * 8 + 4)[M_MODE] = pa.wmode[((size_t)(w0 + w) * MAXF + f) * WM + M_MODE];
+                wfc[tid * 8] = glb(pa.wrec)[(size_t)(w0 + w) * REC + RF(f, 0)];
+                reinterpret_cast<int*>(wfc + tid * 8 + 4)[M_MODE] = glb(pa.wmode)[((size_t)(w0 + w) * MAXF + f) * WM + M_MODE];
             }
             if (tid >= 64 && tid < 128) {
                 const int t = tid - 64, w = t >> 3, j = t & 7;
-                if (w < nw) wsc[t] = pa.wrec[(size_t)(w0 + w) * REC + j];
-            }
-            if (tid >= 128 && tid < 128 + nw) sstat[tid - 128] = pa.wstat[w0 + tid - 128];
+                if (w < nw) wsc[t] = glb(pa.wrec)[(size_t)(w0 + w) * REC + j];
+            }
+            if (tid >= 128 && tid < 128 + nw) sstat[tid - 128] = glb(pa.wstat)[w0 + tid - 128];
         }
         if (FUSED && STEP && tid >= PB - 64 && tid < PB - 64 + nw) {
             const int wl = tid - (PB - 64);
@@ -159,7 +158,7 @@
                 const double aL = uni(sc[Z_AL]), bL = uni(sc[Z_BL]), cL = uni(sc[Z_CL]);
                 auto load_cell = [&](double (&d)[8], int cc) {
                     const int i = cc * 64 + lane;
-                    const double2* __restrict__ src = reinterpret_cast<const double2*>(pa.cells + (size_t)min(i, pa.ncell - 1) * 8);
+                    const double2* __restrict__ src = reinterpret_cast<const double2*>(glb(pa.cells) + (size_t)min(i, pa.ncell - 1) * 8);
 #pragma unroll
                     for (int k = 0; k < 4; ++k) {
                         const double2 a = src[k];
@@ -195,7 +194,7 @@
                 }
             }
             acc = wave_sum_dpp(acc);
-            double* __restrict__ row = pa.partC + (size_t)(w0 + v) * pa.nslot;
+            double* __restrict__ row = glb(pa.partC) + (size_t)(w0 + v) * la.nslot;
             if (lane == 63) pstore(row + vr, acc);
             }
         }
@@ -228,7 +227,7 @@
                     double G, PG, W, col;
                 };
                 auto load_nodes = [&](int c) -> Node {
-                    const double2* __restrict__ src = reinterpret_cast<const double2*>(pa.nodes4 + ((size_t)c * 64 + lane) * 4);
+                    const double2* __restrict__ src = reinterpret_cast<const double2*>(glb(pa.nodes4) + ((size_t)c * 64 + lane) * 4);
                     const double2 a = src[0], b = src[1];
                     return Node{a.x, a.y, b.x, b.y};
                 };
@@ -259,7 +258,7 @@
                 }
             }
             bsum = wave_sum_dpp(bsum);
-            double* __restrict__ row = pa.partB + (size_t)(w0 + v) * pa.nslot;
+            double* __restrict__ row = glb(pa.partB) + (size_t)(w0 + v) * la.nslot;
             if (lane == 63) pstore(row + vr, bsum);
             }
         }
@@ -284,7 +283,7 @@
 #pragma unroll 1
                         for (int i = vr * PB + tid; i < n; i += VF * PB) {
                             const size_t g = (size_t)(start + i);
-                            const double clum = pa.lum[g], ca1 = pa.a1[g], cpp = pa.P[g];
+                            const double clum = glb(pa.lum)[g], ca1 = glb(pa.a1)[g], cpp = glb(pa.P)[g];
                             double term;
                             if (VARIANT == LF_FIXCOMP) {
                                 const double vv = cpp * r[R_Q];
@@ -296,12 +295,12 @@
                                 const WZ wz{r[Z_AL], r[Z_BL], r[Z_CL], r[Z_AP], r[Z_BP], r[Z_CP], r[Z_C1], 0.0};
                                 double vv;
                                 if (mode == MODE_SLOW) {
-                                    const double lnT = lnT_zevol<false>(wz, clum, ca1, pa.U[g], vv, &tab);
+                                    const double lnT = lnT_zevol<false>(wz, clum, ca1, glb(pa.U)[g], vv, &tab);
                                     term = lnT + cpp;
                                     const bool bad = (vv > LF_UNDERFLOW) | (lnT < -LF_UNDERFLOW) | (term < -LF_UNDERFLOW) | (term != term);
                                     term = bad ? NEG_INF : -vv;
                                 } else {
-                                    const double Lsz = quad_nofma(wz.aL, wz.bL, wz.cL, ca1, pa.U[g]);
+                                    const double Lsz = quad_nofma(wz.aL, wz.bL, wz.cL, ca1, glb(pa.U)[g]);
                                     term = -fexp_t(LF_LN10 * (clum - Lsz), &tab);
                                 }
                             }
@@ -318,17 +317,17 @@
 #pragma unroll
                     for (int k = 0; k < PB / 64; ++k) s += red[tid + 64 * k];
                     s = wave_sum_dpp(s);
-                    double* __restrict__ row = pa.partA + (size_t)(w0 + w) * pa.nslot;
+                    double* __restrict__ row = glb(pa.partA) + (size_t)(w0 + w) * la.nslot;
                     if (tid == 63) pstore(row + vr, s);
                 }
                 }
             }
         }
-        if (FUSED && pa.poll && needmask == 0) {
+        if (FUSED && la.poll && needmask == 0) {
             if (frank == fgroup - 1 && v < nw) {
-                const int nB = pa.nchB > 0 ? pa.nslot : 0, nC = VARIANT == LF_ZEVOL && pa.nchC > 0 ? pa.nslot : 0;
-                double* __restrict__ pb = pa.partB + (size_t)(w0 + v) * pa.nslot;
-                double* __restrict__ pc = pa.partC + (size_t)(w0 + v) * pa.nslot;
+                const int nB = pa.nchB > 0 ? la.nslot : 0, nC = VARIANT == LF_ZEVOL && pa.nchC > 0 ? la.nslot : 0;
+                double* __restrict__ pb = glb(pa.partB) + (size_t)(w0 + v) * la.nslot;
+                double* __restrict__ pc = glb(pa.partC) + (size_t)(w0 + v) * la.nslot;
                 double pre[2] = {0.0, 0.0};
                 int tries = 0;
                 bool have;
@@ -340,12 +339,12 @@
                 } while (!__all(have) && ++tries < PART_POLLS);
                 if (tries >= PART_POLLS) {
                     pre[0] = pre[1] = __builtin_nan("");
-                    if (lane == 0) atomicExch(pa.err, 1);
+                    if (lane == 0) atomicExch(glb(pa.err), 1);
                 }
                 if (lane < nC) __hip_atomic_store(pc + lane, __longlong_as_double((long long)PART_EMPTY), __ATOMIC_RELAXED, __HIP_MEMORY_SCOPE_AGENT);
                 if (lane < nB) __hip_atomic_store(pb + lane, __longlong_as_double((long long)PART_EMPTY), __ATOMIC_RELAXED, __HIP_MEMORY_SCOPE_AGENT);
-                finalize_wave<true>(pa.partA, 0, pa.nslot, pa.partB, nB, pa.nslot, nC > 0 ? pa.partC : nullptr, nC, (int)STAT_CELLS,
-                                    sstat - w0, sbase - w0, w0 + v, lane, ap, pa.out, nullptr, nullptr,
+                finalize_wave<true>(glb(pa.partA), 0, la.nslot, glb(pa.partB), nB, la.nslot, nC > 0 ? glb(pa.partC) : nullptr, nC, (int)STAT_CELLS,
+                                    sstat - w0, sbase - w0, w0 + v, lane, ap, la.out, nullptr, nullptr,
                                     VARIANT == LF_FIXCOMP ? (int)STAT_SLOW : 0,
                                     STEP ? sprop + v * 16 : nullptr, STEP ? szz + v : nullptr, STEP ? spre + 2 * v : nullptr, pre);
             }
@@ -357,15 +356,15 @@
             __syncthreads();
             if (sdone == fgroup - 1) {
                 __builtin_amdgcn_fence(__ATOMIC_ACQUIRE, "workgroup");
-                const int nC = VARIANT == LF_ZEVOL && pa.nchC > 0 ? pa.nslot : 0;
+                const int nC = VARIANT == LF_ZEVOL && pa.nchC > 0 ? la.nslot : 0;
                 if (v < nw) {
-                    finalize_wave<true>(pa.partA, pa.nslot, pa.nslot, pa.partB, pa.nslot, pa.nslot, nC > 0 ? pa.partC : nullptr, nC, (int)STAT_CELLS,
-                                        sstat - w0, sbase - w0, w0 + v, lane, ap, pa.out, nullptr, nullptr,
+                    finalize_wave<true>(glb(pa.partA), la.nslot, la.nslot, glb(pa.partB), la.nslot, la.nslot, nC > 0 ? glb(pa.partC) : nullptr, nC, (int)STAT_CELLS,
+                                        sstat - w0, sbase - w0, w0 + v, lane, ap, la.out, nullptr, nullptr,
                                         VARIANT == LF_FIXCOMP ? (int)STAT_SLOW : 0,
                                         STEP ? sprop + v * 16 : nullptr, STEP ? szz + v : nullptr, STEP ? spre + 2 * v : nullptr);
-                    if (pa.poll) {
-                        if (lane < nC) __hip_atomic_store(pa.partC + (size_t)(w0 + v) * pa.nslot + lane, __longlong_as_double((long long)PART_EMPTY), __ATOMIC_RELAXED, __HIP_MEMORY_SCOPE_AGENT);
-                        if (lane < pa.nslot) __hip_atomic_store(pa.partB + (size_t)(w0 + v) * pa.nslot + lane, __longlong_as_double((long long)PART_EMPTY), __ATOMIC_RELAXED, __HIP_MEMORY_SCOPE_AGENT);
+                    if (la.poll) {
+                        if (lane < nC) __hip_atomic_store(glb(pa.partC) + (size_t)(w0 + v) * la.nslot + lane, __longlong_as_double((long long)PART_EMPTY), __ATOMIC_RELAXED, __HIP_MEMORY_SCOPE_AGENT);
+                        if (lane < la.nslot) __hip_atomic_store(glb(pa.partB) + (size_t)(w0 + v) * la.nslot + lane, __longlong_as_double((long long)PART_EMPTY), __ATOMIC_RELAXED, __HIP_MEMORY_SCOPE_AGENT);
                     }
                 }
                 if (tid < QSTRIDE) q[tid] = 0;
@@ -380,21 +379,22 @@
         stamp[4] = t_cells - stamp[0];
         stamp[7] = t_grid - stamp[0];
         stamp[6] = __builtin_amdgcn_s_memrealtime();
-        kc.stamps[(size_t)gridDim.x * 8 + blockIdx.x] = ((t_cols - stamp[0]) << 32) | ((t_prep - stamp[0]) & 0xffffffffull);
+        glb(kc.stamps)[(size_t)gridDim.x * 8 + blockIdx.x] = ((t_cols - stamp[0]) << 32) | ((t_prep - stamp[0]) & 0xffffffffull);
     }
 #endif
 }
 
 template <int VARIANT, bool FUSED>
-__global__ __launch_bounds__(PB, 4) void lf_pers(KConst kc, PersArgs pa) {
-    warm_kernarg<sizeof(KConst) + sizeof(PersArgs)>();
-    lf_pers_body<VARIANT, FUSED, false>(kc, pa, StepArgs{}, AcceptArgs{});
+__global__ __launch_bounds__(PB, 4) void lf_pers(const PersCtx* __restrict__ cb, LaunchArgs la) {
+    static_assert(sizeof(PersCtx*) + sizeof(LaunchArgs) <= 64, "the kernel arguments fit one line");
+    const PersCtx& k = const_block(cb);
+    lf_pers_body<VARIANT, FUSED, false>(k.kc, k.pa, la, StepArgs{}, AcceptArgs{});
 }
 
 template <int VARIANT>
-__global__ __launch_bounds__(PB, 4) void lf_pers_step(KConst kc, PersArgs pa, StepArgs sp, AcceptArgs ap) {
-    warm_kernarg<sizeof(KConst) + sizeof(PersArgs) + sizeof(StepArgs) + sizeof(AcceptArgs)>();
-    lf_pers_body<VARIANT, true, true>(kc, pa, sp, ap);
+__global__ __launch_bounds__(PB, 4) void lf_pers_step(KConst kc, PersArgs pa, LaunchArgs la, StepArgs sp, AcceptArgs ap) {
+    warm_kernarg<sizeof(KConst) + sizeof(PersArgs) + sizeof(LaunchArgs) + sizeof(StepArgs) + sizeof(AcceptArgs)>();
+    lf_pers_body<VARIANT, true, true>(kc, pa, la, sp, ap);
 }
 
 }
diff --git a/lumfuncmcmc_amd/csrc/lfmcmc.hip b/lumfuncmcmc_amd/csrc/lfmcmc.hip
--- a/lumfuncmcmc_amd/csrc/lfmcmc.hip
+++ b/lumfuncmcmc_amd/csrc/lfmcmc.hip
@@ -47,6 +47,8 @@
 };
 
 }
+
+constexpr size_t BLOCK_BYTES = (std::max(sizeof(lf::FreeCtx), sizeof(lf::PersCtx)) + 63) / 64 * 64;
 
 struct lf_ctx {
     lf::KConst kc{};
@@ -122,6 +124,11 @@
     hipStream_t last_stream = nullptr;
     bool any_enqueued = false;
     int profiling = 0;
+    void* d_block = nullptr;
+    size_t block_n = 0;
+    alignas(64) unsigned char h_block[BLOCK_BYTES] = {};
+    lf::FreeCtx blk_free{};
+    lf::PersCtx blk_pers{};
     lf::ZCells zcells{};
     int64_t opt_profile_every = 1;
     int64_t prof_tick = 0;
@@ -599,17 +606,32 @@
     return LF_OK;
 }
 
+int ensure_block(lf_ctx* c, const void* blk, size_t n) {
+    if (n == c->block_n && std::memcmp(c->h_block, blk, n) == 0) return LF_OK;
+    if (n > BLOCK_BYTES || !c->d_block) {
+        c->err = "ensure_block: no constant block";
+        return LF_ERR_HIP;
+    }
+    if (c->any_enqueued) LF_HIP(c, hipDeviceSynchronize());
+    c->block_n = 0;
+    LF_HIP(c, hipMemcpy(c->d_block, blk, n, hipMemcpyHostToDevice));
+    std::memcpy(c->h_block, blk, n);
+    c->block_n = n;
+    return LF_OK;
+}
+
 template <int ST>
-void launch_free(lf_ctx* c, int slot, int B, int ntiles, const lf::SrcArrays& sa, const lf::NodeArrays& na, lf::FreeArgs fa, hipStream_t s,
+void launch_free(lf_ctx* c, int slot, int B, int nchA, int nchB, const lf::LaunchArgs& la, hipStream_t s,
                  bool fused, const lf::StepArgs* sp = nullptr, const lf::AcceptArgs* ap = nullptr) {
     using namespace lf;
-    const dim3 grid((unsigned)(8 * fa.tile_stride));
-    const int info[8] = {ST, PTW, PTW, fused ? 3 : 2, (int)grid.x, fa.nchA, fa.nchB, B};
+    const dim3 grid((unsigned)(8 * la.tile_stride));
+    const int info[8] = {ST, PTW, PTW, fused ? 3 : 2, (int)grid.x, nchA, nchB, B};
     std::memcpy(c->last_launch, info, sizeof(info));
-    if (fused && sp) hipLaunchKernelGGL((lf_free_step<ST>), grid, dim3(PB), 0, s, c->kc, sa, na, fa, *sp, *ap);
-    else if (fused) hipLaunchKernelGGL((lf_free<ST, false, true>), grid, dim3(PB), 0, s, c->kc, sa, na, c->d_wrec, c->d_wmode, fa);
-    else if (c->kc.forms) hipLaunchKernelGGL((lf_free<ST, true>), grid, dim3(PB), 0, s, c->kc, sa, na, c->d_wrec, c->d_wmode, fa);
-    else hipLaunchKernelGGL((lf_free<ST, false>), grid, dim3(PB), 0, s, c->kc, sa, na, c->d_wrec, c->d_wmode, fa);
+    const FreeCtx* cb = static_cast<const FreeCtx*>(c->d_block);
+    if (fused && sp) hipLaunchKernelGGL((lf_free_step<ST>), grid, dim3(PB), 0, s, cb, la, *sp, *ap);
+    else if (fused) hipLaunchKernelGGL((lf_free<ST, false, true>), grid, dim3(PB), 0, s, cb, c->d_wrec, c->d_wmode, la);
+    else if (c->kc.forms) hipLaunchKernelGGL((lf_free<ST, true>), grid, dim3(PB), 0, s, cb, c->d_wrec, c->d_wmode, la);
+    else hipLaunchKernelGGL((lf_free<ST, false>), grid, dim3(PB), 0, s, cb, c->d_wrec, c->d_wmode, la);
 }
 
 int enqueue_free(lf_ctx* c, const double* d_theta, int B, double* d_out, double* d_outA, double* d_outB, hipStream_t s,
@@ -671,20 +693,32 @@
         hipLaunchKernelGGL(lf_prepare, dim3((B + 7) / 8), dim3(64), 0, s, c->kc, sp, d_theta, B, c->d_wrec,
                            c->d_wstat, c->d_wmode, c->d_wbase, (int*)nullptr, c->d_queue, ntiles * QSTRIDE);
     }
-    const SrcArrays sa{c->d_lum, c->d_a1, c->d_P, c->d_U, nullptr, ct->d_start, ct->d_len, ct->d_field, ct->d_keys, nullptr};
-    const NodeArrays na{c->d_G, c->d_PG, c->d_W, c->d_a3, c->d_a4, c->d_a4min, c->nnodes};
-    FreeArgs fa{B, ntiles, nchA, nchB, nslot, g8, (int)c->opt_skip_grid, c->d_queue, c->d_partA, c->d_partB,
-                c->d_cells, c->d_nodes8, c->deal_key > 0 ? c->d_deal : nullptr, c->d_cc_len, c->d_cc_field, nchC, c->d_partR, c->d_wstat,
-                d_theta, d_out, c->d_wrec, c->d_wmode, c->d_wstat, c->d_wbase,
-                gq ? c->gridq.d_rec : nullptr, gq ? c->gridq.d_omega : nullptr, gq ? c->gridq.d_rows : nullptr, gq ? c->gridq.nb : 0,
-                poll ? 1 : 0, c->d_err};
+    {
+        FreeCtx& b = c->blk_free;
+        b.kc = c->kc;
+        b.sa = SrcArrays{c->d_lum, c->d_a1, c->d_P, c->d_U, nullptr, ct->d_start, ct->d_len, ct->d_field, ct->d_keys, nullptr};
+        NodeArrays& na = b.na;
+        na.G = c->d_G; na.PG = c->d_PG; na.W = c->d_W; na.a3 = c->d_a3; na.a4 = c->d_a4; na.a4min = c->d_a4min;
+        na.nnodes = c->nnodes;
+        FreeArgs& fa = b.fa;
+        fa.nchA = nchA; fa.nchB = nchB; fa.skip_grid = (int)c->opt_skip_grid;
+        fa.queues = c->d_queue; fa.partA = c->d_partA; fa.partB = c->d_partB;
+        fa.cells = c->d_cells; fa.nodes8 = c->d_nodes8; fa.deal = c->deal_key > 0 ? c->d_deal : nullptr;
+        fa.cc_len = c->d_cc_len; fa.cc_field = c->d_cc_field; fa.nchC = nchC; fa.partC = c->d_partR; fa.wstat = c->d_wstat;
+        fa.wrec_w = c->d_wrec; fa.wmode_w = c->d_wmode; fa.wstat_w = c->d_wstat; fa.wbase_w = c->d_wbase;
+        fa.gq_rec = gq ? c->gridq.d_rec : nullptr; fa.gq_omega = gq ? c->gridq.d_omega : nullptr;
+        fa.gq_rows = gq ? c->gridq.d_rows : nullptr; fa.nbq = gq ? c->gridq.nb : 0;
+        fa.err = c->d_err;
+        if ((rc = ensure_block(c, &b, sizeof(b))) != LF_OK) return rc;
+    }
+    const LaunchArgs la{d_theta, d_out, B, ntiles, g8, nslot, poll ? 1 : 0};
     {
         Prof p(c, s, 1);
         if (nchA + nchB > 0) {
             const StepArgs* psp = fused && stepf ? &sp : nullptr;
-            if (st == 8) launch_free<8>(c, slot, B, ntiles, sa, na, fa, s, fused, psp, &ap);
-            else if (st == 4) launch_free<4>(c, slot, B, ntiles, sa, na, fa, s, fused, psp, &ap);
-            else launch_free<2>(c, slot, B, ntiles, sa, na, fa, s, fused, psp, &ap);
+            if (st == 8) launch_free<8>(c, slot, B, nchA, nchB, la, s, fused, psp, &ap);
+            else if (st == 4) launch_free<4>(c, slot, B, nchA, nchB, la, s, fused, psp, &ap);
+            else launch_free<2>(c, slot, B, nchA, nchB, la, s, fused, psp, &ap);
         }
     }
     if (!fused) {
@@ -752,16 +786,27 @@
         hipLaunchKernelGGL(lf_prepare, dim3((B + 7) / 8), dim3(64), 0, s, c->kc, sp, d_theta, B, c->d_wrec,
                            c->d_wstat, c->d_wmode, c->d_wbase, (int*)nullptr, c->d_queue, 0);
     }
-    const PersArgs pa{B, ntiles, nchB, nchC, c->ncell, nslot, g8, c->d_queue, c->d_partA, c->d_partB, c->d_partR, c->d_nodes4, c->d_zcol,
-                      c->d_cells, c->d_lum, c->d_a1, c->d_P, c->d_U, d_theta, d_out, c->d_wrec, c->d_wmode, c->d_wstat, poll ? 1 : 0, c->d_err};
+    {
+        PersCtx& b = c->blk_pers;
+        b.kc = c->kc;
+        PersArgs& pa = b.pa;
+        pa.nchB = nchB; pa.nchC = nchC; pa.ncell = c->ncell;
+        pa.queues = c->d_queue; pa.partA = c->d_partA; pa.partB = c->d_partB; pa.partC = c->d_partR;
+        pa.nodes4 = c->d_nodes4; pa.zcol = c->d_zcol; pa.cells = c->d_cells;
+        pa.lum = c->d_lum; pa.a1 = c->d_a1; pa.P = c->d_P; pa.U = c->d_U;
+        pa.wrec = c->d_wrec; pa.wmode = c->d_wmode; pa.wstat = c->d_wstat; pa.err = c->d_err;
+        if ((rc = ensure_block(c, &b, sizeof(b))) != LF_OK) return rc;
+    }
+    const LaunchArgs la{d_theta, d_out, B, ntiles, g8, nslot, poll ? 1 : 0};
+    const PersCtx* cb = static_cast<const PersCtx*>(c->d_block);
     {
         Prof p(c, s, 1);
         const dim3 grid((unsigned)(8 * g8));
         const int info[8] = {0, PTW, PTW, fused ? 5 : 4, (int)grid.x, nchC, nchB, B};
         std::memcpy(c->last_launch, info, sizeof(info));
-        if (fused && stepf) hipLaunchKernelGGL((lf_pers_step<VARIANT>), grid, dim3(PB), 0, s, c->kc, pa, sp, ap);
-        else if (fused) hipLaunchKernelGGL((lf_pers<VARIANT, true>), grid, dim3(PB), 0, s, c->kc, pa);
-        else hipLaunchKernelGGL((lf_pers<VARIANT, false>), grid, dim3(PB), 0, s, c->kc, pa);
+        if (fused && stepf) hipLaunchKernelGGL((lf_pers_step<VARIANT>), grid, dim3(PB), 0, s, c->blk_pers.kc, c->blk_pers.pa, la, sp, ap);
+        else if (fused) hipLaunchKernelGGL((lf_pers<VARIANT, true>), grid, dim3(PB), 0, s, cb, la);
+        else hipLaunchKernelGGL((lf_pers<VARIANT, false>), grid, dim3(PB), 0, s, cb, la);
     }
     if (!fused) {
         Prof p(c, s, 3);
@@ -1106,6 +1151,7 @@
     if (c->d_cc_start) hipFree(c->d_cc_start);
     if (c->d_deal) hipFree(c->d_deal);
     if (c->d_err) hipFree(c->d_err);
+    if (c->d_block) hipFree(c->d_block);
     if (c->d_cc_len) hipFree(c->d_cc_len);
     if (c->d_cc_field) hipFree(c->d_cc_field);
     {
@@ -1521,6 +1567,10 @@
     int rc = LF_OK;
     try {
         rc = build(c, d);
+        if (rc == LF_OK && hipMalloc(&c->d_block, BLOCK_BYTES) != hipSuccess) {
+            c->err = "hipMalloc of the constant block failed";
+            rc = LF_ERR_HIP;
+        }
     } catch (const std::bad_alloc&) {
         c->err = "out of host memory";
         rc = LF_ERR_NOMEM;
```

Result: faster. 9.975 million walker-lnprob evals/s, median of 6 (+4.8%).
